# aurelienwaite/SparkNet

Hardware: AMD Instinct MI355X
Metric: images/sec AlexNet training (227x227) at 1/2/4/8 MI355X; scaling efficiency (higher is better)
Workload: dtype bf16; 1 GPU; model=caffenet (bvlc_reference_caffenet / AlexNet), global_batch=256, per_gpu_batch=256, parallelism=dp1, algorithm=local SGD, tau=50, RCCL all-reduce weight averaging, hipgraph=True, streams=3, feed_group=2, fused_input_fold=True, fp8_layers=0, fp8_wgrad=False

## Files before the change

### csrc/kernels/reduce.hip

```cpp
#include "common.h"

struct ReduceOut {
  void* out;
  long long ldo, out_gstride;
  int cols, mode, relu;
  const float* bias;
  const bf16_t* gate;
  float* extra;
  long long extra_gstride;
  int extra_col, extra_acc;
  const long long* drop_rng;
  int drop_stream;
  unsigned drop_thr;
  float drop_scale, gate_scale;
};

SN_DEV void reduce_store(const ReduceOut& o, int g, int r, int c, float4 a) {
  const float acc[4] = {a.x, a.y, a.z, a.w};
  if (o.extra && c <= o.extra_col && o.extra_col < c + 4) {
    float* e = o.extra + g * o.extra_gstride + r;
    const int q = o.extra_col - c;
    const float v = q == 0 ? a.x : (q == 1 ? a.y : (q == 2 ? a.z : a.w));
    *e = o.extra_acc ? *e + v : v;
  }
  if (o.mode == 0) {
    const long long base = g * o.out_gstride + (long long)r * o.ldo + c;
    bf16_t* p = reinterpret_cast<bf16_t*>(o.out) + base;
    float v[4];
#pragma unroll
    for (int k = 0; k < 4; ++k) {
      v[k] = acc[k] + ((o.bias && c + k < o.cols) ? o.bias[(long long)g * o.cols + c + k] : 0.f);
      if (o.relu) v[k] = fmaxf(v[k], 0.f);
      if (o.gate && c + k < o.cols) v[k] = bf2f(o.gate[base + k]) > 0.f ? v[k] * o.gate_scale : 0.f;
    }
    if (o.drop_rng) {
      if ((base & 3) == 0) {
        const uint4 u = dropout_bits4(o.drop_rng, o.drop_stream, (unsigned long long)base >> 2);
        const uint32_t b[4] = {u.x, u.y, u.z, u.w};
#pragma unroll
        for (int k = 0; k < 4; ++k) v[k] = b[k] > o.drop_thr ? v[k] * o.drop_scale : 0.f;
      } else {
#pragma unroll
        for (int k = 0; k < 4; ++k)
          v[k] = dropout_keep(o.drop_rng, o.drop_stream, o.drop_thr, base + k) ? v[k] * o.drop_scale : 0.f;
      }
    }
    if (c + 3 < o.cols && (base & 3) == 0) {
      *reinterpret_cast<uint2*>(p) = make_uint2(pack2(v[0], v[1]), pack2(v[2], v[3]));
    } else {
#pragma unroll
      for (int k = 0; k < 4; ++k)
        if (c + k < o.cols) p[k] = f2bf(v[k]);
    }
  } else {
    float* p = reinterpret_cast<float*>(o.out) + g * o.out_gstride + (long long)r * o.ldo + c;
    const int cols = o.extra ? o.extra_col : o.cols;
#pragma unroll
    for (int k = 0; k < 4; ++k)
      if (c + k < cols) p[k] = (o.mode == 2 ? p[k] : 0.f) + acc[k];
  }
}

__global__ void splitk_reduce_kernel(const float* __restrict__ ws, int splits, long long sstride, int rows,
                                     long long ldw, long long ws_gstride, ReduceOut o) {
  const int cols = o.cols, cols4 = (cols + 3) >> 2;
  const long long total = (long long)rows * cols4;
  const int g = blockIdx.y;
  const float* wsg = ws + g * ws_gstride;
  for (long long i = blockIdx.x * (long long)blockDim.x + threadIdx.x; i < total;
       i += (long long)gridDim.x * blockDim.x) {
    const int r = (int)(i / cols4), c = (int)(i - (long long)r * cols4) * 4;
    float acc[4] = {0.f, 0.f, 0.f, 0.f};
    const bool vec = (c + 3 < cols) && ((ldw & 3) == 0);
    const float* p0 = wsg + (long long)r * ldw + c;
    if (vec) {
      int s = 0;
      for (; s + 3 < splits; s += 4) {
        float4 v[4];
#pragma unroll
        for (int u = 0; u < 4; ++u) v[u] = *reinterpret_cast<const float4*>(p0 + (s + u) * sstride);
#pragma unroll
        for (int u = 0; u < 4; ++u) {
          acc[0] += v[u].x; acc[1] += v[u].y; acc[2] += v[u].z; acc[3] += v[u].w;
        }
      }
      for (; s < splits; ++s) {
        const float4 v = *reinterpret_cast<const float4*>(p0 + s * sstride);
        acc[0] += v.x; acc[1] += v.y; acc[2] += v.z; acc[3] += v.w;
      }
    } else {
      for (int s = 0; s < splits; ++s)
#pragma unroll
        for (int k = 0; k < 4; ++k)
          if (c + k < cols) acc[k] += p0[s * sstride + k];
    }
    reduce_store(o, g, r, c, make_float4(acc[0], acc[1], acc[2], acc[3]));
  }
}

__global__ void __launch_bounds__(256) splitk_reduce_wide(const float* __restrict__ ws, int splits,
                                                          long long sstride, int rows, long long ldw,
                                                          long long ws_gstride, ReduceOut o) {
  __shared__ float4 red[16][16];
  const int it = threadIdx.x & 15, sl = threadIdx.x >> 4;
  const int cols4 = (o.cols + 3) >> 2;
  const long long total = (long long)rows * cols4;
  const long long i = blockIdx.x * 16LL + it;
  const int g = blockIdx.y;
  float4 acc = make_float4(0.f, 0.f, 0.f, 0.f);
  int r = 0, c = 0;
  if (i < total) {
    r = (int)(i / cols4);
    c = (int)(i - (long long)r * cols4) * 4;
    const float* p = ws + g * ws_gstride + (long long)r * ldw + c;
    int s = sl;
    for (; s + 48 < splits; s += 64) {
      float4 v[4];
#pragma unroll
      for (int u = 0; u < 4; ++u) v[u] = *reinterpret_cast<const float4*>(p + (s + 16 * u) * sstride);
#pragma unroll
      for (int u = 0; u < 4; ++u) {
        acc.x += v[u].x; acc.y += v[u].y; acc.z += v[u].z; acc.w += v[u].w;
      }
    }
    for (; s < splits; s += 16) {
      float4 v = *reinterpret_cast<const float4*>(p + s * sstride);
      acc.x += v.x; acc.y += v.y; acc.z += v.z; acc.w += v.w;
    }
  }
  red[sl][it] = acc;
  __syncthreads();
  if (sl == 0 && i < total) {
    float a[4] = {0.f, 0.f, 0.f, 0.f};
#pragma unroll
    for (int q = 0; q < 16; ++q) {
      float4 v = red[q][it];
      a[0] += v.x; a[1] += v.y; a[2] += v.z; a[3] += v.w;
    }
    reduce_store(o, g, r, c, make_float4(a[0], a[1], a[2], a[3]));
  }
}

extern "C" int sn_splitk_reduce(const float* ws, long long splits, long long sstride, long long rows,
                                long long cols, long long ldw, void* out, long long ldo, long long mode,
                                const float* bias, long long relu, long long groups,
                                long long ws_gstride, long long out_gstride, const bf16_t* gate,
                                float* extra, long long extra_col, long long extra_acc, long long extra_gstride,
                                const long long* drop_rng, long long drop_stream, float drop_ratio,
                                float gate_scale, hipStream_t st) {
  ReduceOut o;
  o.drop_rng = drop_rng;
  o.drop_stream = (int)drop_stream;
  o.drop_thr = (uint32_t)((double)4294967295u * (double)drop_ratio);
  o.drop_scale = 1.f / (1.f - drop_ratio);
  o.gate_scale = gate_scale;
  o.out = out; o.ldo = ldo; o.out_gstride = out_gstride; o.cols = (int)cols; o.mode = (int)mode;
  o.relu = (int)relu; o.bias = bias; o.gate = gate;
  o.extra = extra; o.extra_col = (int)extra_col; o.extra_acc = (int)extra_acc; o.extra_gstride = extra_gstride;
  if (extra && (mode == 0 || extra_col != cols - 1)) return 5;
  long long total = rows * ((cols + 3) / 4);
  if (splits >= 16 && ((cols & 3) == 0 || ldw >= ((cols + 3) & ~3LL)) && (ldw & 3) == 0) {
    dim3 grid((unsigned)((total + 15) / 16), (unsigned)groups);
    hipLaunchKernelGGL(splitk_reduce_wide, grid, dim3(256), 0, st, ws, (int)splits, sstride, (int)rows, ldw,
                       ws_gstride, o);
  } else {
    dim3 grid(sn_blocks(total, 256, 4096), (unsigned)groups);
    hipLaunchKernelGGL(splitk_reduce_kernel, grid, dim3(256), 0, st, ws, (int)splits, sstride, (int)rows, ldw,
                       ws_gstride, o);
  }
  return SN_CHECK_LAUNCH();
}

__global__ void __launch_bounds__(256) colsum_pass1(const bf16_t* __restrict__ x, long long rows, int cols,
                                                    long long ld, long long rpb, int CL, float* __restrict__ part) {
  __shared__ float red[256 * 8];
  const int RL = 256 / CL;
  const int t = threadIdx.x;
  const int cc = t % CL, rr = t / CL;
  const int c = (blockIdx.y * CL + cc) * 8;
  float acc[8] = {0, 0, 0, 0, 0, 0, 0, 0};
  const long long r0 = blockIdx.x * rpb, r1 = min(rows, r0 + rpb);
  if (c < cols) {
    const bool vec = (c + 7 < cols) && ((ld & 7) == 0);
    long long r = r0 + rr;
    if (vec) {
      for (; r + 3 * RL < r1; r += 4 * RL) {
        uint4 v[4];
#pragma unroll
        for (int u = 0; u < 4; ++u) v[u] = *reinterpret_cast<const uint4*>(x + (r + u * RL) * ld + c);
#pragma unroll
        for (int u = 0; u < 4; ++u) {
          float f[8];
          unpack8(v[u], f);
#pragma unroll
          for (int k = 0; k < 8; ++k) acc[k] += f[k];
        }
      }
    }
    for (; r < r1; r += RL) {
      const bf16_t* p = x + r * ld + c;
      if (vec) {
        float f[8];
        unpack8(*reinterpret_cast<const uint4*>(p), f);
#pragma unroll
        for (int k = 0; k < 8; ++k) acc[k] += f[k];
      } else {
        for (int k = 0; k < 8; ++k)
          if (c + k < cols) acc[k] += bf2f(p[k]);
      }
    }
  }
#pragma unroll
  for (int k = 0; k < 8; ++k) red[t * 8 + k] = acc[k];
  __syncthreads();
  if (rr == 0 && c < cols) {
    for (int q = 1; q < RL; ++q)
#pragma unroll
      for (int k = 0; k < 8; ++k) acc[k] += red[(q * CL + cc) * 8 + k];
    for (int k = 0; k < 8; ++k)
      if (c + k < cols) part[blockIdx.x * (long long)cols + c + k] = acc[k];
  }
}

__global__ void __launch_bounds__(1024) colsum_pass2(const float* __restrict__ part, int nparts, int cols, float* out,
                                                     int accumulate) {
  __shared__ float red[16][64];
  const int lane = threadIdx.x & 63, w = threadIdx.x >> 6;
  const int c = blockIdx.x * 64 + lane;
  float s[8] = {0, 0, 0, 0, 0, 0, 0, 0};
  if (c < cols) {
    int p = w;
    for (; p + 7 * 16 < nparts; p += 8 * 16) {
#pragma unroll
      for (int u = 0; u < 8; ++u) s[u] += part[(long long)(p + u * 16) * cols + c];
    }
    for (; p < nparts; p += 16) s[0] += part[(long long)p * cols + c];
  }
  red[w][lane] = ((s[0] + s[1]) + (s[2] + s[3])) + ((s[4] + s[5]) + (s[6] + s[7]));
  __syncthreads();
  if (w == 0 && c < cols) {
    float tot = 0.f;
#pragma unroll
    for (int k = 0; k < 16; ++k) tot += red[k][lane];
    out[c] = (accumulate ? out[c] : 0.f) + tot;
  }
}

extern "C" int sn_colsum_bf16(const bf16_t* x, long long rows, long long cols, long long ld, float* part,
                              long long nparts, float* out, long long accumulate, hipStream_t st) {
  const int c8 = (int)((cols + 7) / 8);
  int CL = 1;
  while (CL < c8 && CL < 64) CL *= 2;
  const int cblocks = (c8 + CL - 1) / CL;
  long long rpb = (rows + nparts - 1) / nparts;
  hipLaunchKernelGGL(colsum_pass1, dim3((unsigned)nparts, (unsigned)cblocks), dim3(256), 0, st, x, rows,
                     (int)cols, ld, rpb, CL, part);
  hipLaunchKernelGGL(colsum_pass2, dim3((unsigned)((cols + 63) / 64)), dim3(1024), 0, st, part, (int)nparts,
                     (int)cols, out, (int)accumulate);
  return SN_CHECK_LAUNCH();
}

__global__ void vsum_kernel(const float* __restrict__ x, long long n, float* out, float scale, int accumulate) {
  __shared__ float red[16];
  float s = 0.f;
  for (long long i = threadIdx.x; i < n; i += blockDim.x) s += x[i];
  s = wave_sum(s);
  if ((threadIdx.x & 63) == 0) red[threadIdx.x >> 6] = s;
  __syncthreads();
  if (threadIdx.x == 0) {
    float t = 0.f;
    for (int w = 0; w < (int)(blockDim.x >> 6); ++w) t += red[w];
    out[0] = (accumulate ? out[0] : 0.f) + t * scale;
  }
}

extern "C" int sn_vsum(const float* x, long long n, float* out, float scale, long long accumulate, hipStream_t st) {
  hipLaunchKernelGGL(vsum_kernel, dim3(1), dim3(1024), 0, st, x, n, out, scale, (int)accumulate);
  return SN_CHECK_LAUNCH();
}

namespace {
__global__ void probe_tr8_kernel(unsigned* out) {
  __shared__ __attribute__((aligned(16))) unsigned char img[256];
  const int l = threadIdx.x;
  for (int e = l; e < 256; e += 64) img[e] = (unsigned char)e;
  __syncthreads();
  typedef int v2i __attribute__((ext_vector_type(2)));
  const int g = l >> 4, i = l & 15;
  const int row = 8 * (g & 1) + (i >> 1);
  typedef __attribute__((address_space(3))) v2i lds_v2i;
  const v2i v = __builtin_amdgcn_ds_read_tr8_b64_v2i32(
      (lds_v2i*)((__attribute__((address_space(3))) unsigned char*)img + row * 16 + 8 * (i & 1)));
  out[2 * l] = (unsigned)v[0];
  out[2 * l + 1] = (unsigned)v[1];
}
}

extern "C" int sn_probe_tr8(unsigned* out, hipStream_t st) {
  hipLaunchKernelGGL(probe_tr8_kernel, dim3(1), dim3(64), 0, st, out);
  return SN_CHECK_LAUNCH();
}
```

### csrc/kernels/softmax.hip

```cpp
#include "common.h"

#define FLT_MIN_ 1.175494351e-38f

__global__ void softmax_xent_fwd(const bf16_t* __restrict__ x, const float* __restrict__ labels,
                                 float* __restrict__ prob, float* __restrict__ row_loss, float* __restrict__ row_valid,
                                 int M, int C, int has_ignore, int ignore_label) {
  const int lane = threadIdx.x & 63;
  const int row = blockIdx.x * (blockDim.x >> 6) + (threadIdx.x >> 6);
  if (row >= M) return;
  const bf16_t* xr = x + (long long)row * C;
  float m = -INFINITY;
  for (int c = lane; c < C; c += 64) m = fmaxf(m, bf2f(xr[c]));
  m = wave_max(m);
  float s = 0.f;
  for (int c = lane; c < C; c += 64) s += __expf(bf2f(xr[c]) - m);
  s = wave_sum(s);
  const float inv = 1.f / s;
  float* pr = prob + (long long)row * C;
  for (int c = lane; c < C; c += 64) pr[c] = __expf(bf2f(xr[c]) - m) * inv;
  if (lane == 0) {
    int lab = (int)labels[row];
    bool valid = !(has_ignore && lab == ignore_label);
    float nll = 0.f;
    if (valid) {
      float p = __expf(bf2f(xr[min(max(lab, 0), C - 1)]) - m) * inv;
      nll = -__logf(fmaxf(p, FLT_MIN_));
    }
    row_loss[row] = nll;
    row_valid[row] = valid ? 1.f : 0.f;
  }
}

__global__ void xent_reduce(const float* __restrict__ row_loss, const float* __restrict__ row_valid, int M,
                            int normalize, float outer_num, float* __restrict__ out_loss, float* __restrict__ out_norm) {
  __shared__ float ls[16], vs[16];
  float l = 0.f, v = 0.f;
  for (int i = threadIdx.x; i < M; i += blockDim.x) {
    l += row_loss[i];
    v += row_valid[i];
  }
  l = wave_sum(l);
  v = wave_sum(v);
  if ((threadIdx.x & 63) == 0) {
    ls[threadIdx.x >> 6] = l;
    vs[threadIdx.x >> 6] = v;
  }
  __syncthreads();
  if (threadIdx.x == 0) {
    float L = 0.f, V = 0.f;
    for (int w = 0; w < (int)(blockDim.x >> 6); ++w) { L += ls[w]; V += vs[w]; }
    float norm = normalize ? V : outer_num;
    norm = fmaxf(norm, 1.f);
    out_loss[0] = L / norm;
    out_norm[0] = norm;
  }
}

extern "C" int sn_softmax_xent_fwd(const bf16_t* x, const float* labels, float* prob, float* row_loss,
                                   float* row_valid, float* out_loss, float* out_norm, long long M, long long C,
                                   long long has_ignore, long long ignore_label, long long normalize,
                                   long long outer_num, hipStream_t st) {
  const int rows_per_block = 4;
  hipLaunchKernelGGL(softmax_xent_fwd, dim3((unsigned)((M + rows_per_block - 1) / rows_per_block)), dim3(256), 0, st, x,
                     labels, prob, row_loss, row_valid, (int)M, (int)C, (int)has_ignore, (int)ignore_label);
  hipLaunchKernelGGL(xent_reduce, dim3(1), dim3(1024), 0, st, row_loss, row_valid, (int)M, (int)normalize,
                     (float)outer_num, out_loss, out_norm);
  return SN_CHECK_LAUNCH();
}

__global__ void softmax_xent_bwd(const float* __restrict__ prob, const float* __restrict__ labels,
                                 const float* __restrict__ loss_weight, const float* __restrict__ norm,
                                 bf16_t* __restrict__ dx, int M, int C, int has_ignore, int ignore_label) {
  const long long total = (long long)M * C;
  const float scale = loss_weight[0] / norm[0];
  for (long long i = blockIdx.x * (long long)blockDim.x + threadIdx.x; i < total; i += (long long)gridDim.x * blockDim.x) {
    const int row = (int)(i / C), c = (int)(i - (long long)row * C);
    const int lab = (int)labels[row];
    float g = 0.f;
    if (!(has_ignore && lab == ignore_label)) g = (prob[i] - (c == lab ? 1.f : 0.f)) * scale;
    dx[i] = f2bf(g);
  }
}

extern "C" int sn_softmax_xent_bwd(const float* prob, const float* labels, const float* loss_weight, const float* norm,
                                   bf16_t* dx, long long M, long long C, long long has_ignore, long long ignore_label,
                                   hipStream_t st) {
  hipLaunchKernelGGL(softmax_xent_bwd, dim3(sn_blocks(M * C, 256, 16384)), dim3(256), 0, st, prob, labels, loss_weight,
                     norm, dx, (int)M, (int)C, (int)has_ignore, (int)ignore_label);
  return SN_CHECK_LAUNCH();
}

__global__ void softmax_fwd(const bf16_t* __restrict__ x, bf16_t* __restrict__ y, int M, int C) {
  const int lane = threadIdx.x & 63;
  const int row = blockIdx.x * (blockDim.x >> 6) + (threadIdx.x >> 6);
  if (row >= M) return;
  const bf16_t* xr = x + (long long)row * C;
  float m = -INFINITY;
  for (int c = lane; c < C; c += 64) m = fmaxf(m, bf2f(xr[c]));
  m = wave_max(m);
  float s = 0.f;
  for (int c = lane; c < C; c += 64) s += __expf(bf2f(xr[c]) - m);
  s = wave_sum(s);
  const float inv = 1.f / s;
  for (int c = lane; c < C; c += 64) y[(long long)row * C + c] = f2bf(__expf(bf2f(xr[c]) - m) * inv);
}

__global__ void softmax_bwd(const bf16_t* __restrict__ dy, const bf16_t* __restrict__ y, bf16_t* __restrict__ dx,
                            int M, int C) {
  const int lane = threadIdx.x & 63;
  const int row = blockIdx.x * (blockDim.x >> 6) + (threadIdx.x >> 6);
  if (row >= M) return;
  const long long b = (long long)row * C;
  float d = 0.f;
  for (int c = lane; c < C; c += 64) d += bf2f(dy[b + c]) * bf2f(y[b + c]);
  d = wave_sum(d);
  for (int c = lane; c < C; c += 64) dx[b + c] = f2bf(bf2f(y[b + c]) * (bf2f(dy[b + c]) - d));
}

extern "C" int sn_softmax_fwd(const bf16_t* x, bf16_t* y, long long M, long long C, hipStream_t st) {
  hipLaunchKernelGGL(softmax_fwd, dim3((unsigned)((M + 3) / 4)), dim3(256), 0, st, x, y, (int)M, (int)C);
  return SN_CHECK_LAUNCH();
}

extern "C" int sn_softmax_bwd(const bf16_t* dy, const bf16_t* y, bf16_t* dx, long long M, long long C, hipStream_t st) {
  hipLaunchKernelGGL(softmax_bwd, dim3((unsigned)((M + 3) / 4)), dim3(256), 0, st, dy, y, dx, (int)M, (int)C);
  return SN_CHECK_LAUNCH();
}

__global__ void accuracy_rows(const bf16_t* __restrict__ x, const float* __restrict__ labels, float* __restrict__ hit,
                              float* __restrict__ valid, int M, int C, int k, int has_ignore, int ignore_label) {
  const int lane = threadIdx.x & 63;
  const int row = blockIdx.x * (blockDim.x >> 6) + (threadIdx.x >> 6);
  if (row >= M) return;
  const int lab = (int)labels[row];
  const bf16_t* xr = x + (long long)row * C;
  const int lc = min(max(lab, 0), C - 1);
  const float ls = bf2f(xr[lc]);
  float cnt = 0.f;
  for (int c = lane; c < C; c += 64) {
    const float v = bf2f(xr[c]);
    cnt += (v > ls || (!(ls > v) && c > lc)) ? 1.f : 0.f;
  }
  cnt = wave_sum(cnt);
  if (lane == 0) {
    bool v = !(has_ignore && lab == ignore_label);
    hit[row] = (v && cnt < (float)k) ? 1.f : 0.f;
    valid[row] = v ? 1.f : 0.f;
  }
}

extern "C" int sn_accuracy(const bf16_t* x, const float* labels, float* hit, float* valid, float* out_acc,
                           float* out_norm, long long M, long long C, long long k, long long has_ignore,
                           long long ignore_label, hipStream_t st) {
  hipLaunchKernelGGL(accuracy_rows, dim3((unsigned)((M + 3) / 4)), dim3(256), 0, st, x, labels, hit, valid, (int)M,
                     (int)C, (int)k, (int)has_ignore, (int)ignore_label);
  hipLaunchKernelGGL(xent_reduce, dim3(1), dim3(1024), 0, st, hit, valid, (int)M, 1, (float)M, out_acc, out_norm);
  return SN_CHECK_LAUNCH();
}
```

### csrc/kernels/solver.hip

```cpp
#include "common.h"

enum { H_LR = 0, H_MOM, H_WD, H_CLIP, H_NORM, H_DELTA, H_MOM2, H_RMS, H_CORR, H_T, H_SUMSQ = 15 };

SN_DEV void chunk_grad(const float* __restrict__ g, long long o, const long long* __restrict__ src, int cid, int i,
                       float* G) {
  const long long sp = src ? src[4 * cid] : 0;
  if (sp == 0) {
    const float4 gv = *reinterpret_cast<const float4*>(g + o);
    G[0] = gv.x; G[1] = gv.y; G[2] = gv.z; G[3] = gv.w;
    return;
  }
  const float* sl = reinterpret_cast<const float*>(sp);
  const long long ss = src[4 * cid + 1], es = src[4 * cid + 3];
  const int splits = (int)src[4 * cid + 2];
  G[0] = G[1] = G[2] = G[3] = 0.f;
  if (splits >= 16) {
    if (es == 1) {
      const float* p = sl + i;
      for (int l = 0; l < 16; ++l) {
        float P[4] = {0.f, 0.f, 0.f, 0.f};
        int s = l;
        for (; s + 48 < splits; s += 64) {
          float4 v[4];
#pragma unroll
          for (int u = 0; u < 4; ++u) v[u] = *reinterpret_cast<const float4*>(p + (s + 16 * u) * ss);
#pragma unroll
          for (int u = 0; u < 4; ++u) {
            P[0] += v[u].x; P[1] += v[u].y; P[2] += v[u].z; P[3] += v[u].w;
          }
        }
        for (; s < splits; s += 16) {
          const float4 v = *reinterpret_cast<const float4*>(p + s * ss);
          P[0] += v.x; P[1] += v.y; P[2] += v.z; P[3] += v.w;
        }
#pragma unroll
        for (int k = 0; k < 4; ++k) G[k] += P[k];
      }
    } else {
      for (int l = 0; l < 16; ++l) {
        float P[4] = {0.f, 0.f, 0.f, 0.f};
        for (int s = l; s < splits; s += 16) {
          float v[4];
#pragma unroll
          for (int k = 0; k < 4; ++k) v[k] = sl[(long long)(i + k) * es + s * ss];
#pragma unroll
          for (int k = 0; k < 4; ++k) P[k] += v[k];
        }
#pragma unroll
        for (int k = 0; k < 4; ++k) G[k] += P[k];
      }
    }
    return;
  }
  if (es == 1) {
    const float* p = sl + i;
    int s = 0;
    for (; s + 3 < splits; s += 4) {
      float4 v[4];
#pragma unroll
      for (int u = 0; u < 4; ++u) v[u] = *reinterpret_cast<const float4*>(p + (s + u) * ss);
#pragma unroll
      for (int u = 0; u < 4; ++u) {
        G[0] += v[u].x; G[1] += v[u].y; G[2] += v[u].z; G[3] += v[u].w;
      }
    }
    for (; s < splits; ++s) {
      const float4 v = *reinterpret_cast<const float4*>(p + s * ss);
      G[0] += v.x; G[1] += v.y; G[2] += v.z; G[3] += v.w;
    }
  } else {
    for (int s = 0; s < splits; ++s)
#pragma unroll
      for (int k = 0; k < 4; ++k) G[k] += sl[(long long)(i + k) * es + s * ss];
  }
}

template <int KIND, bool L1, bool CLIP, bool SHADOW>
__global__ void __launch_bounds__(256) solver_update_kernel(float* __restrict__ w, const float* __restrict__ g,
                                                            float* __restrict__ h0, float* __restrict__ h1,
                                                            bf16_t* __restrict__ shadow,
                                                            const long long* __restrict__ chunk_pos,
                                                            const float* __restrict__ chunk_mult,
                                                            const float* __restrict__ hyper, int nchunks,
                                                            const long long* __restrict__ chunk_src) {
  for (int cid = blockIdx.x; cid < nchunks; cid += gridDim.x) {
  const long long start = chunk_pos[2 * cid];
  const int count = (int)chunk_pos[2 * cid + 1];
  const float lr_mult = chunk_mult[2 * cid], decay_mult = chunk_mult[2 * cid + 1];
  const float rate = hyper[H_LR] * lr_mult;
  const float mom = hyper[H_MOM];
  const float decay = hyper[H_WD] * decay_mult;
  float gscale = hyper[H_NORM];
  if (CLIP) {
    const float clip = hyper[H_CLIP];
    const float l2 = sqrtf(hyper[H_SUMSQ]);
    if (clip > 0.f && l2 > clip) gscale *= clip / l2;
  }
  const float delta = hyper[H_DELTA], mom2 = hyper[H_MOM2], rms = hyper[H_RMS], corr = hyper[H_CORR];
  for (int i = threadIdx.x * 4; i < count; i += blockDim.x * 4) {
    const long long o = start + i;
    float4 wv = *reinterpret_cast<float4*>(w + o);
    float G[4];
    chunk_grad(g, o, chunk_src, cid, i, G);
    float4 a = *reinterpret_cast<float4*>(h0 + o);
    float4 b = make_float4(0.f, 0.f, 0.f, 0.f);
    if (KIND >= 4) b = *reinterpret_cast<float4*>(h1 + o);
    float W[4] = {wv.x, wv.y, wv.z, wv.w};
    float A[4] = {a.x, a.y, a.z, a.w}, B[4] = {b.x, b.y, b.z, b.w};
#pragma unroll
    for (int k = 0; k < 4; ++k) {
      float gg = G[k] * gscale;
      gg += decay * (L1 ? ((W[k] > 0.f) - (W[k] < 0.f)) : W[k]);
      float upd;
      if (KIND == 0) {
        A[k] = mom * A[k] + rate * gg;
        upd = A[k];
      } else if (KIND == 1) {
        float prev = A[k];
        A[k] = mom * A[k] + rate * gg;
        upd = (1.f + mom) * A[k] - mom * prev;
      } else if (KIND == 2) {
        A[k] += gg * gg;
        upd = rate * gg / (sqrtf(A[k]) + delta);
      } else if (KIND == 3) {
        A[k] = rms * A[k] + (1.f - rms) * gg * gg;
        upd = rate * gg / (sqrtf(A[k]) + delta);
      } else if (KIND == 4) {
        A[k] = mom * A[k] + (1.f - mom) * gg * gg;
        float u = gg * sqrtf((B[k] + delta) / (A[k] + delta));
        B[k] = mom * B[k] + (1.f - mom) * u * u;
        upd = rate * u;
      } else {
        A[k] = mom * A[k] + (1.f - mom) * gg;
        B[k] = mom2 * B[k] + (1.f - mom2) * gg * gg;
        upd = rate * corr * A[k] / (sqrtf(B[k]) + delta);
      }
      W[k] -= upd;
    }
    *reinterpret_cast<float4*>(w + o) = make_float4(W[0], W[1], W[2], W[3]);
    *reinterpret_cast<float4*>(h0 + o) = make_float4(A[0], A[1], A[2], A[3]);
    if (KIND >= 4) *reinterpret_cast<float4*>(h1 + o) = make_float4(B[0], B[1], B[2], B[3]);
    if (SHADOW) *reinterpret_cast<uint2*>(shadow + o) = make_uint2(pack2(W[0], W[1]), pack2(W[2], W[3]));
  }
  }
}

__global__ void sumsq_pass1(const float* __restrict__ g, long long n, float* __restrict__ part) {
  __shared__ float red[16];
  float s = 0.f;
  for (long long i = blockIdx.x * (long long)blockDim.x + threadIdx.x; i < n; i += (long long)gridDim.x * blockDim.x) {
    float v = g[i];
    s += v * v;
  }
  s = wave_sum(s);
  if ((threadIdx.x & 63) == 0) red[threadIdx.x >> 6] = s;
  __syncthreads();
  if (threadIdx.x == 0) {
    float t = 0.f;
    for (int w = 0; w < (int)(blockDim.x >> 6); ++w) t += red[w];
    part[blockIdx.x] = t;
  }
}

__global__ void sumsq_pass2(const float* __restrict__ part, int nparts, float* __restrict__ hyper) {
  __shared__ float red[16];
  float s = 0.f;
  for (int i = threadIdx.x; i < nparts; i += blockDim.x) s += part[i];
  s = wave_sum(s);
  if ((threadIdx.x & 63) == 0) red[threadIdx.x >> 6] = s;
  __syncthreads();
  if (threadIdx.x == 0) {
    float t = 0.f;
    for (int w = 0; w < (int)(blockDim.x >> 6); ++w) t += red[w];
    hyper[H_SUMSQ] = t;
  }
}

template <int KIND, bool L1, bool CLIP>
static void launch3(bool shadow, dim3 grid, hipStream_t st, float* w, const float* g, float* h0, float* h1,
                    bf16_t* sh, const long long* cp, const float* cm, const float* hyper, int n, const long long* src) {
  if (shadow)
    hipLaunchKernelGGL((solver_update_kernel<KIND, L1, CLIP, true>), grid, dim3(256), 0, st, w, g, h0, h1, sh, cp, cm,
                       hyper, n, src);
  else
    hipLaunchKernelGGL((solver_update_kernel<KIND, L1, CLIP, false>), grid, dim3(256), 0, st, w, g, h0, h1, sh, cp,
                       cm, hyper, n, src);
}

template <int KIND>
static void launch_kind(bool l1, bool clip, bool shadow, dim3 grid, hipStream_t st, float* w, const float* g,
                        float* h0, float* h1, bf16_t* sh, const long long* cp, const float* cm, const float* hyper,
                        int n, const long long* src) {
  if (l1) {
    if (clip) launch3<KIND, true, true>(shadow, grid, st, w, g, h0, h1, sh, cp, cm, hyper, n, src);
    else launch3<KIND, true, false>(shadow, grid, st, w, g, h0, h1, sh, cp, cm, hyper, n, src);
  } else {
    if (clip) launch3<KIND, false, true>(shadow, grid, st, w, g, h0, h1, sh, cp, cm, hyper, n, src);
    else launch3<KIND, false, false>(shadow, grid, st, w, g, h0, h1, sh, cp, cm, hyper, n, src);
  }
}

extern "C" int sn_solver_update(long long kind, float* w, const float* g, float* h0, float* h1, bf16_t* shadow,
                                const long long* chunk_pos, const float* chunk_mult, long long nchunks,
                                float* hyper, long long l1, long long clip, float* part, long long nparts,
                                long long total, long long grid_limit, const long long* chunk_src, hipStream_t st) {
  if (nchunks <= 0) return 0;
  if (clip && chunk_src) return 9;
  if (clip) {
    hipLaunchKernelGGL(sumsq_pass1, dim3((unsigned)nparts), dim3(256), 0, st, g, total, part);
    hipLaunchKernelGGL(sumsq_pass2, dim3(1), dim3(1024), 0, st, part, (int)nparts, hyper);
  }
  dim3 grid((unsigned)(grid_limit > 0 && grid_limit < nchunks ? grid_limit : nchunks));
  bool sh = shadow != nullptr;
  const int n = (int)nchunks;
  switch (kind) {
    case 0: launch_kind<0>(l1, clip, sh, grid, st, w, g, h0, h1, shadow, chunk_pos, chunk_mult, hyper, n, chunk_src); break;
    case 1: launch_kind<1>(l1, clip, sh, grid, st, w, g, h0, h1, shadow, chunk_pos, chunk_mult, hyper, n, chunk_src); break;
    case 2: launch_kind<2>(l1, clip, sh, grid, st, w, g, h0, h1, shadow, chunk_pos, chunk_mult, hyper, n, chunk_src); break;
    case 3: launch_kind<3>(l1, clip, sh, grid, st, w, g, h0, h1, shadow, chunk_pos, chunk_mult, hyper, n, chunk_src); break;
    case 4: launch_kind<4>(l1, clip, sh, grid, st, w, g, h0, h1, shadow, chunk_pos, chunk_mult, hyper, n, chunk_src); break;
    case 5: launch_kind<5>(l1, clip, sh, grid, st, w, g, h0, h1, shadow, chunk_pos, chunk_mult, hyper, n, chunk_src); break;
    default: return 8;
  }
  return SN_CHECK_LAUNCH();
}

__global__ void scale_shadow(float* __restrict__ w, bf16_t* __restrict__ shadow, long long n, long long n4,
                             float scale) {
  const long long stride = (long long)gridDim.x * blockDim.x;
  for (long long i = blockIdx.x * (long long)blockDim.x + threadIdx.x; i < n4; i += stride) {
    float4 v = reinterpret_cast<float4*>(w)[i];
    v.x *= scale; v.y *= scale; v.z *= scale; v.w *= scale;
    reinterpret_cast<float4*>(w)[i] = v;
    if (shadow) reinterpret_cast<uint2*>(shadow)[i] = make_uint2(pack2(v.x, v.y), pack2(v.z, v.w));
  }
  for (long long i = 4 * n4 + blockIdx.x * (long long)blockDim.x + threadIdx.x; i < n; i += stride) {
    const float v = w[i] * scale;
    w[i] = v;
    if (shadow) shadow[i] = f2bf(v);
  }
}

extern "C" int sn_scale_shadow(float* w, bf16_t* shadow, long long n, float scale, hipStream_t st) {
  if (n <= 0) return 0;
  const bool vec = (reinterpret_cast<uintptr_t>(w) & 15) == 0 && (reinterpret_cast<uintptr_t>(shadow) & 7) == 0;
  const long long n4 = vec ? n / 4 : 0;
  hipLaunchKernelGGL(scale_shadow, dim3(sn_blocks(n4 > 0 ? n4 : n, 256, 16384)), dim3(256), 0, st, w, shadow, n, n4,
                     scale);
  return SN_CHECK_LAUNCH();
}
```

### sparknet_amd/core/solver.py

```python
from __future__ import annotations

import logging
import math
import os
import time
from typing import Callable

import numpy as np
import torch

from .. import proto
from .net import Net, blob_proto_to_tensor

log = logging.getLogger("sparknet_amd.solver")

SOLVER_KINDS = {"SGD": 0, "Nesterov": 1, "AdaGrad": 2, "RMSProp": 3, "AdaDelta": 4, "Adam": 5}
_LEGACY_TYPES = {0: "SGD", 1: "Nesterov", 2: "AdaGrad", 3: "RMSProp", 4: "AdaDelta", 5: "Adam"}
N_HISTORY = {"SGD": 1, "Nesterov": 1, "AdaGrad": 1, "RMSProp": 1, "AdaDelta": 2, "Adam": 2}

H_LR, H_MOM, H_WD, H_CLIP, H_NORM, H_DELTA, H_MOM2, H_RMS, H_CORR, H_T = range(10)
N_HYPER = 16


class Solver:
    def __init__(self, param, *, device="cpu", dtype=None, seed: int | None = None,
                 train_net: Net | None = None, build_test_nets: bool = True):
        if isinstance(param, str):
            param = proto.read_solver(param)
        self.param = proto.copy(param)
        p = self.param
        self.type = p.type if p.HasField("type") else (
            _LEGACY_TYPES[int(p.solver_type)] if p.HasField("solver_type") else "SGD")
        if self.type not in SOLVER_KINDS:
            raise ValueError(f"Unknown solver type {self.type!r}")
        self.device = torch.device(device)
        if seed is None:
            seed = int(p.random_seed) if p.random_seed >= 0 else 1701
        self.seed = seed
        self.iter = 0
        self.current_step = 0
        self.callbacks: list = []
        self.action_request: Callable[[], str] | None = None
        self.requested_early_exit = False
        self.losses: list[torch.Tensor] = []
        self.smoothed_loss = 0.0
        self.net = train_net if train_net is not None else self._init_train_net(dtype)
        self.test_nets: list[Net] = []
        if build_test_nets:
            self._init_test_nets(dtype)
        self.history: list[torch.Tensor] = []
        self._init_state()

    def _net_param_source(self):
        p = self.param
        n = int(p.HasField("train_net_param")) + int(p.HasField("train_net")) + \
            int(p.HasField("net_param")) + int(p.HasField("net"))
        if n != 1:
            raise ValueError("SolverParameter must specify exactly one of train_net_param, train_net, "
                             "net_param, net")
        if p.HasField("train_net_param"):
            return proto.copy(p.train_net_param)
        if p.HasField("train_net"):
            return proto.read_net(p.train_net)
        if p.HasField("net_param"):
            return proto.copy(p.net_param)
        return proto.read_net(p.net)

    def _init_train_net(self, dtype) -> Net:
        netp = self._net_param_source()
        state = proto.NetState(phase=proto.TRAIN)
        state.MergeFrom(netp.state)
        state.MergeFrom(self.param.train_state)
        netp.state.CopyFrom(state)
        return Net(netp, device=self.device, dtype=dtype, seed=self.seed)

    def _init_test_nets(self, dtype) -> None:
        p = self.param
        sources = []
        for tp in p.test_net_param:
            sources.append(proto.copy(tp))
        for tf in p.test_net:
            sources.append(proto.read_net(tf))
        remaining = len(p.test_iter) - len(sources)
        if remaining > 0:
            if p.HasField("net_param"):
                sources += [proto.copy(p.net_param)] * remaining
            elif p.HasField("net"):
                base = proto.read_net(p.net)
                sources += [base] * remaining
        if len(p.test_state) and len(p.test_state) != len(sources):
            raise ValueError("test_state must be unspecified or specified once per test net")
        for i, netp in enumerate(sources):
            netp = proto.copy(netp)
            state = proto.NetState(phase=proto.TEST)
            state.MergeFrom(netp.state)
            if len(p.test_state):
                state.MergeFrom(p.test_state[i])
            netp.state.CopyFrom(state)
            tn = Net(netp, device=self.device, dtype=self.net.dtype, seed=self.seed, allocate=True)
            tn.share_trained_layers_with(self.net)
            self.test_nets.append(tn)

    def _init_state(self) -> None:
        n = self.net.num_param_elems
        self.history = [torch.zeros(max(n, 1), dtype=torch.float32, device=self.device)
                        for _ in range(N_HISTORY[self.type])]
        self.hyper = torch.zeros(N_HYPER, dtype=torch.float32, device=self.device)
        self._hyper_staged: list | None = None
        self._build_tables()

    def _build_tables(self) -> None:
        from .. import ops
        segs = self.net.param_segments()
        self.segments = segs
        fused = set(getattr(self, "fused_offsets", set()))
        for sink in getattr(self, "slab_sinks", ()):
            if sink.desc is not None:
                fused.update(p.offset for p in sink.params())
        self._tables = ops.solver_tables([s for s in segs if s[0] not in fused], self.net.num_param_elems,
                                         self.device)
        self.slab_tables_dirty = False

    def set_slab_sinks(self, sinks) -> None:
        self.slab_sinks = list(sinks)
        self.slab_tables_dirty = True
        if not getattr(self, "fused_offsets", None):
            self.fused_offsets = set()

    def set_fused_update(self, offsets) -> None:
        self.fused_offsets = set(offsets)
        self._build_tables()

    def get_learning_rate(self) -> float:
        p = self.param
        pol = p.lr_policy
        it = self.iter
        if pol == "fixed":
            return p.base_lr
        if pol == "step":
            self.current_step = it // p.stepsize
            return p.base_lr * math.pow(p.gamma, self.current_step)
        if pol == "exp":
            return p.base_lr * math.pow(p.gamma, it)
        if pol == "inv":
            return p.base_lr * math.pow(1.0 + p.gamma * it, -p.power)
        if pol == "multistep":
            if self.current_step < len(p.stepvalue) and it >= p.stepvalue[self.current_step]:
                self.current_step += 1
            return p.base_lr * math.pow(p.gamma, self.current_step)
        if pol == "poly":
            return p.base_lr * math.pow(1.0 - float(it) / float(p.max_iter), p.power)
        if pol == "sigmoid":
            return p.base_lr * (1.0 / (1.0 + math.exp(-p.gamma * (float(it) - float(p.stepsize)))))
        raise ValueError(f"Unknown learning rate policy: {pol!r}")

    def hyper_values(self, rate: float) -> list[float]:
        p = self.param
        h = [0.0] * N_HYPER
        h[H_LR] = rate
        h[H_MOM] = p.momentum
        h[H_WD] = p.weight_decay
        h[H_CLIP] = p.clip_gradients
        h[H_NORM] = 1.0 / max(1, p.iter_size)
        h[H_DELTA] = p.delta
        h[H_MOM2] = p.momentum2
        h[H_RMS] = p.rms_decay
        t = self.iter + 1
        if self.type == "Adam":
            h[H_CORR] = math.sqrt(1.0 - math.pow(p.momentum2, t)) / (1.0 - math.pow(p.momentum, t))
        h[H_T] = float(t)
        return h

    def stage_hyper(self, rate: float | None = None) -> float:
        rate = self.get_learning_rate() if rate is None else rate
        vals = self.hyper_values(rate)
        vals[H_T] = 0.0
        if vals == self._hyper_staged:
            return rate
        self._hyper_staged = vals
        host = torch.tensor(vals, dtype=torch.float32)
        if self.device.type == "cuda":
            host = host.pin_memory()
        self.hyper.copy_(host, non_blocking=True)
        return rate

    def apply_update(self) -> float:
        rate = self.stage_hyper()
        if self.param.display and self.iter % self.param.display == 0:
            log.info("Iteration %d, lr = %g", self.iter, rate)
        self.update_params()
        return rate

    def overlap_eligible(self) -> bool:
        return (self.device.type == "cuda" and self.param.clip_gradients <= 0 and self.param.iter_size <= 1
                and not self.callbacks)

    def overlap_plan(self, min_group: int = 1) -> tuple[dict, list]:
        net = self.net
        seg_of = {seg[0]: seg for seg in self.segments}
        final, late = {}, set()
        for li, layer in enumerate(net.layers):
            writer = getattr(layer, "fused_into", None) if layer.params else None
            wl = net.layers.index(writer) if writer is not None else li
            for i, p in enumerate(layer.params):
                if p.offset not in seg_of:
                    continue
                if not net.layer_need_backward[li] or not layer.param_grads_needed(i):
                    late.add(p.offset)
                final[p.offset] = min(final.get(p.offset, wl), wl)
        groups: dict = {}
        for off, li in final.items():
            if off not in late:
                groups.setdefault(li, []).append(seg_of[off])
        big = {li: segs for li, segs in groups.items() if sum(sg[1] for sg in segs) >= min_group}
        rest = [seg_of[o] for o in seg_of if not any(o == sg[0] for segs in big.values() for sg in segs)]
        return big, rest

    def update_params_segments(self, tables, grid_limit: int = 0) -> None:
        from .. import ops
        net = self.net
        ops.solver_update(SOLVER_KINDS[self.type], net.flat_data, net.flat_diff, self.history,
                          net.flat_compute if net.flat_compute is not net.flat_data else None,
                          tables, self.hyper, self.param.regularization_type == "L1", False, grid_limit)

    def update_params(self) -> None:
        from .. import ops
        l1 = self.param.regularization_type == "L1"
        if self.param.regularization_type not in ("L1", "L2"):
            raise ValueError(f"Unknown regularization type: {self.param.regularization_type}")
        net = self.net
        if getattr(self, "slab_tables_dirty", False):
            assert not torch.cuda.is_current_stream_capturing(), "split-K slab layout changed during capture"
            self._build_tables()
        ops.solver_update(SOLVER_KINDS[self.type], net.flat_data, net.flat_diff, self.history,
                          net.flat_compute if net.flat_compute is not net.flat_data else None,
                          self._tables, self.hyper, l1, self.param.clip_gradients > 0)

    def iteration(self):
        net = self.net
        if getattr(self, "fused_offsets", None) or getattr(self, "slab_sinks", None):
            self.stage_hyper()
        net.clear_param_diffs(lazy=True)
        for cb in self.callbacks:
            getattr(cb, "on_start", lambda: None)()
        loss = None
        for _ in range(max(1, self.param.iter_size)):
            l = net.forward_backward()
            loss = l if loss is None else loss + l
            from .. import ops
            ops.advance_rng(net.ctx.rng_state)
        net.finish_param_diffs()
        if getattr(net.ctx, "fp8", None) is not None:
            net.ctx.fp8.update()
        if self.param.iter_size > 1:
            loss = loss / self.param.iter_size
        for cb in self.callbacks:
            getattr(cb, "on_gradients_ready", lambda: None)()
        self.apply_update()
        return loss

    def step(self, iters: int) -> None:
        start_iter = self.iter
        stop_iter = self.iter + iters
        avg = max(1, self.param.average_loss)
        while self.iter < stop_iter:
            loss = self.iteration()
            self.losses.append(loss.detach())
            if len(self.losses) > avg:
                self.losses.pop(0)
            display = self.param.display and self.iter % self.param.display == 0
            self.iter += 1
            if display:
                self.smoothed_loss = float(torch.stack(self.losses).mean())
                log.info("Iteration %d, loss = %g", self.iter - 1, self.smoothed_loss)
            if self.param.snapshot and self.iter % self.param.snapshot == 0:
                self.snapshot()
            req = self.action_request() if self.action_request else "none"
            if req == "snapshot":
                self.snapshot()
            elif req == "stop":
                self.requested_early_exit = True
                break
        del start_iter

    def solve(self, resume_file: str | None = None) -> None:
        if resume_file:
            self.restore(resume_file)
        p = self.param
        self.requested_early_exit = False
        while self.iter < p.max_iter and not self.requested_early_exit:
            if p.test_interval and self.iter % p.test_interval == 0 and (self.iter > 0 or p.test_initialization):
                self.test_all()
            n = p.max_iter - self.iter
            if p.test_interval:
                n = min(n, p.test_interval - self.iter % p.test_interval)
            self.step(n)
        if p.snapshot_after_train and (not p.snapshot or self.iter % p.snapshot != 0):
            self.snapshot()
        if self.requested_early_exit:
            log.info("Optimization stopped early.")
            return
        if p.display and self.iter % p.display == 0:
            loss = self.net.forward()
            log.info("Iteration %d, loss = %g", self.iter, float(loss))
        if p.test_interval and self.iter % p.test_interval == 0:
            self.test_all()

    def test(self, test_net_id: int = 0, iters: int | None = None) -> list[float]:
        scores = self.test_and_store_result(test_net_id, iters)
        n = iters if iters is not None else self.param.test_iter[test_net_id]
        res = [s / max(n, 1) for s in scores]
        tn = self.test_nets[test_net_id]
        names = [b.name for b in tn.output_blobs]
        for name, v in zip(names, res):
            log.info("    Test net output #%s: %s = %g", test_net_id, name, v)
        return res

    def test_and_store_result(self, test_net_id: int = 0, iters: int | None = None) -> list[float]:
        tn = self.test_nets[test_net_id]
        n = iters if iters is not None else self.param.test_iter[test_net_id]
        acc = None
        for _ in range(n):
            tn.forward()
            vals = torch.stack([b.data.float().sum() for b in tn.output_blobs])
            acc = vals if acc is None else acc + vals
        return [] if acc is None else acc.cpu().tolist()

    def test_all(self) -> list[list[float]]:
        return [self.test(i) for i in range(len(self.test_nets))]

    def _prefix(self) -> str:
        return self.param.snapshot_prefix or "snapshot"

    def snapshot(self, prefix: str | None = None) -> tuple[str, str]:
        prefix = prefix or self._prefix()
        h5 = self.param.HasField("snapshot_format") and self.param.snapshot_format == 0
        ext = ".h5" if h5 else ""
        model = f"{prefix}_iter_{self.iter}.caffemodel{ext}"
        state = f"{prefix}_iter_{self.iter}.solverstate{ext}"
        d = os.path.dirname(model)
        if d:
            os.makedirs(d, exist_ok=True)
        if h5:
            self.net.to_hdf5(model, write_diff=self.param.snapshot_diff)
            self._state_to_hdf5(state, model)
        else:
            from ..utils.checkpoint import save_caffemodel
            save_caffemodel(self.net, model, write_diff=self.param.snapshot_diff)
            proto.write_binary(state, self.solver_state(model))
        log.info("Snapshotting to %s / %s", model, state)
        return model, state

    def _history_blobs(self):
        for h in self.history:
            for prm in self.net.learnable_params:
                yield prm, h[prm.offset:prm.offset + prm.count].view(prm.shape)

    def _state_to_hdf5(self, path: str, learned_net: str) -> None:
        from ..utils import hdf5
        hist = {str(i): prm.to_caffe(seg).float().cpu().numpy()
                for i, (prm, seg) in enumerate(self._history_blobs())}
        hdf5.write(path, {"iter": np.array([self.iter], np.int32), "learned_net": learned_net,
                          "current_step": np.array([self.current_step], np.int32), "history": hist})

    def solver_state(self, learned_net: str = ""):
        st = proto.SolverState(iter=self.iter, learned_net=learned_net, current_step=self.current_step)
        for prm, seg in self._history_blobs():
            bp = st.history.add()
            bp.shape.dim.extend(prm.caffe_shape)
            bp.data.extend(prm.to_caffe(seg).cpu().reshape(-1).tolist())
        return st

    def restore(self, state_file: str) -> None:
        if state_file.endswith(".h5"):
            from ..utils import hdf5
            f = hdf5.File(state_file)
            self.iter = hdf5.read_int(f["iter"])
            learned = hdf5.read_string(f["learned_net"]) if "learned_net" in f else ""
            self.current_step = hdf5.read_int(f["current_step"])
            hist = f["history"]
            blobs = [torch.from_numpy(hist[str(i)].read().astype(np.float32)) for i in range(len(hist))]
        else:
            st = proto.read_binary(state_file, proto.SolverState)
            self.iter, self.current_step, learned = st.iter, st.current_step, st.learned_net
            blobs = [blob_proto_to_tensor(b) for b in st.history]
        if learned:
            self.net.copy_trained_layers_from(learned)
        slots = list(self._history_blobs())
        if len(blobs) != len(slots):
            raise ValueError("Incorrect length of history blobs.")
        for (prm, seg), t in zip(slots, blobs):
            seg.copy_(prm.from_caffe(t).to(seg.device))
        log.info("Restored solver state from %s (iter %d)", state_file, self.iter)

    def add_callback(self, cb) -> None:
        self.callbacks.append(cb)


def create_solver(param, **kw) -> Solver:
    return Solver(param, **kw)


def timed(fn):
    def wrap(*a, **k):
        t = time.perf_counter()
        r = fn(*a, **k)
        return r, time.perf_counter() - t
    return wrap
```

### sparknet_amd/engine.py

```python
from __future__ import annotations

import gc
import logging
import os
import time

import torch

from . import ops
from .core.solver import Solver
from .utils import features
from .utils.trace import trace_range

from .ops.spec import ConvSpec

log = logging.getLogger("sparknet_amd.engine")


def fuse_relu(net) -> int:
    if net.device.type == "cuda" and net.dtype == torch.float32:
        return 0
    n = 0
    for li in range(1, len(net.layers)):
        relu = net.layers[li]
# ... 31 lines not shown
        blob = net.top_ids[li][0]
        if len(net.bottom_vecs[li][0].shape) not in (2, 4):
            continue
        if net.bottom_ids[li + 1] != [blob] or net.top_ids[li + 1] != [blob]:
            continue
        if sc.scale is None or (sc.axis, sc.k) != (1, 1) or sc.fused_into is not None:
            continue
        need = net.layer_need_backward[li]
        if net.layer_need_backward[li + 1] != need or (need and not net.bottom_need_backward[li + 1][0]):
            continue
        relu = net.layers[li + 2] if li + 2 < len(net.layers) else None
        if (relu is not None and relu.type_name == "ReLU" and getattr(relu, "slope", 1.0) == 0.0
                and net.bottom_ids[li + 2] == [blob] and net.top_ids[li + 2] == [blob] and not relu.fused
                and not relu.bwd_fused):
            if net.layer_need_backward[li + 2] != need or (need and not net.bottom_need_backward[li + 2][0]):
                continue
            relu.fused = True
            relu.bwd_fused = True
            relu.bn_fused = True
            bn.fused_relu = True
        bn.fused_scale = sc
        sc.fused_into = bn
        ex = dict(getattr(bn, "sched_extra", None) or {})
        ex["bwd_w"] = set(ex.get("bwd_w", ())) | {("p", p.offset) for p in sc.params}
        bn.sched_extra = ex
        n += 1
    net.bn_scale_fused += n
    return n


def fuse_pool_lrn(net) -> int:
    from .ops import hip
    if net.device.type != "cuda" or net.debug_info or not features.enabled("fuse_pool_lrn"):
        return 0
    outputs = set(getattr(net, "output_blob_ids", ()))
    n = 0
    for li, pool in enumerate(net.layers):
        if pool.type_name != "Pooling" or len(net.top_ids[li]) != 1 or pool.global_pooling:
            continue
        blob = net.top_ids[li][0]
        readers = [lj for lj in range(li + 1, len(net.layers)) if blob in net.bottom_ids[lj]]
        if blob in outputs or len(readers) != 1:
            continue
        lj = readers[0]
        lrn = net.layers[lj]
        if lrn.type_name != "LRN" or lrn.relu_gate or net.top_ids[lj][0] == blob:
            continue
        if net.layer_need_backward[li] != net.layer_need_backward[lj]:
            continue
        s = pool.spec(net.bottom_vecs[li][0])
        if not hip.pool_lrn_eligible(s, lrn.size, lrn.within):
            continue
        lrn.pool_fused = True
        lrn.top = net.top_vecs[lj][0]
        pool.fused_lrn = lrn
        n += 1
    return n


def fuse_lrn_pool_backward(net) -> int:
    from .ops import hip
    if net.device.type != "cuda" or net.debug_info or not features.enabled("fuse_lrn_pool_bwd"):
        return 0
    outputs = set(getattr(net, "output_blob_ids", ()))
    n = 0
    for lj, lrn in enumerate(net.layers):
        if lrn.type_name != "LRN" or lrn.pool_fused or lrn.within or len(net.top_ids[lj]) != 1:
            continue
        blob = net.top_ids[lj][0]
        if blob in outputs or blob == net.bottom_ids[lj][0]:
            continue
        readers = [li for li in range(lj + 1, len(net.layers)) if blob in net.bottom_ids[li]]
        if len(readers) != 1:
            continue
        li = readers[0]
        pool = net.layers[li]
        if (pool.type_name != "Pooling" or len(net.top_ids[li]) != 1 or pool.global_pooling
                or pool.fused_lrn is not None or pool.relu_gate or net.top_ids[li][0] == blob):
            continue
        if not (net.layer_need_backward[li] and net.layer_need_backward[lj] and net.bottom_need_backward[li][0]
                and net.bottom_need_backward[lj][0]):
            continue
        s = pool.spec(net.bottom_vecs[li][0])
        if not hip.pool_lrn_rev_eligible(s, lrn.size, lrn.within):
            continue
        pool.bwd_lrn = lrn
        lrn.bottom = net.bottom_vecs[lj][0]
        bid = net.bottom_ids[lj][0]
        ex = dict(getattr(pool, "sched_extra", None) or {})
        ex["bwd_r"] = set(ex.get("bwd_r", ())) | {("v", bid)}
        ex["bwd_w"] = set(ex.get("bwd_w", ())) | {("d", bid)}
        pool.sched_extra = ex
        n += 1
    return n


def _gating_consumers(net, blob: int, after: int):
    if blob in getattr(net, "output_blob_ids", ()):
        return None
    out = []
    for lj in range(after + 1, len(net.layers)):
        if blob not in net.bottom_ids[lj]:
            continue
        lay = net.layers[lj]
        if blob in net.top_ids[lj] or not net.layer_need_backward[lj]:
            return None
        if lay.type_name == "Split":
            for t in net.top_ids[lj]:
                sub = _gating_consumers(net, t, lj)
                if sub is None:
                    return None
                out += sub
            continue
        if lay.type_name not in _GATE_CONSUMERS or len(net.bottom_ids[lj]) != 1 or getattr(lay, "relu_gate", False):
            return None
        if lay.type_name == "Pooling" and (lay.method not in (0, 1) or len(net.top_ids[lj]) != 1):
            return None
        if lay.type_name in ("InnerProduct", "Dropout"):
            return None
        out.append(lj)
    return out


def fuse_concat(net) -> int:
    if net.device.type != "cuda" or not features.enabled("zero_copy_concat"):
        return 0
    from .layers.common import ConcatSlots
    from .ops import hip
    n = 0
    outputs = set(getattr(net, "output_blob_ids", ()))
    for lc, cat in enumerate(net.layers):
        if cat.type_name != "Concat" or len(net.bottom_ids[lc]) < 2 or cat.zero_copy is not None:
            continue
        bots = net.bottom_ids[lc]
        if len(set(bots)) != len(bots) or len(net.bottom_vecs[lc][0].shape) != 4:
            continue
        if cat.axis != 1:
            continue
        prods = []
        for bid in bots:
            writers = [lj for lj in range(lc) if bid in net.top_ids[lj]]
            readers = [lj for lj in range(len(net.layers)) if bid in net.bottom_ids[lj] and lj != lc]
            if not writers or bid in outputs:
                break
            prod = net.layers[writers[0]]
            inplace_ok = all(net.layers[lj].type_name == "ReLU" and getattr(net.layers[lj], "fused", False)
                             and net.top_ids[lj] == [bid] and net.bottom_ids[lj] == [bid] for lj in readers)
            if (not inplace_ok or set(writers[1:]) != set(readers) or prod.type_name != "Convolution"
                    or len(net.top_ids[writers[0]]) != 1 or prod.concat_slot is not None
                    or prod.fp8_slots is not None or prod.folded_input is not None):
                break
            s = prod.spec(net.bottom_vecs[writers[0]][0])
            if not hip._slice_ok(s) or hip._s2d_plan(s) is not None:
                break
            prods.append((prod, s.K))
        if len(prods) != len(bots):
            continue
        slots = ConcatSlots([k for _, k in prods])
        for part, (prod, _) in enumerate(prods):
            prod.concat_slot = (slots, part)
        cat.zero_copy = slots
        gated = _gating_consumers(net, net.top_ids[lc][0], lc)
        if gated is not None and cat.relu_gate_parts == frozenset(range(len(bots))):
            for lj in gated:
                net.layers[lj].relu_gate = True
            cat.relu_gate_parts = frozenset()
            cat.zero_copy_bwd = True
        n += 1
    return n


def fuse_dropout(net) -> int:
    if net.device.type != "cuda" or not features.enabled("fuse_dropout"):
        return 0
    n = 0
    for li in range(1, len(net.layers)):
        d = net.layers[li]
        if d.type_name != "Dropout" or d.phase != 0 or not (d.ratio > 0) or d.fused_into is not None:
            continue
        if net.bottom_ids[li] != net.top_ids[li] or not getattr(d, "relu_gate", False):
            continue
        blob = net.top_ids[li][0]
        prods = [lj for lj in range(li) if blob in net.top_ids[lj]]
        lp = next((lj for lj in reversed(prods) if net.layers[lj].type_name == "InnerProduct"), None)
        if lp is None or not getattr(net.layers[lp], "fuse_relu", False):
            continue
        between = [net.layers[lj] for lj in prods if lj > lp]
        if any(not (l.type_name == "ReLU" and getattr(l, "fused", False)) for l in between):
            continue
        consumers = [lj for lj in range(li + 1, len(net.layers)) if blob in net.bottom_ids[lj]]
        if len(consumers) != 1 or blob in getattr(net, "output_blob_ids", ()):
            continue
        lc = consumers[0]
        cons = net.layers[lc]
        if cons.type_name != "InnerProduct" or len(net.bottom_ids[lc]) != 1 or blob in net.top_ids[lc]:
            continue
        prod = net.layers[lp]
        if prod.fused_dropout is not None:
            continue
        prod.fused_dropout = d
        d.fused_into = prod
        cons.relu_gate = True
        cons.gate_scale = 1.0 / (1.0 - d.ratio)
        n += 1
    return n


def batch_weight_flips(net) -> int:
    if net.device.type != "cuda" or getattr(net, "_flip_batch", None) is not None:
        return 0
    from .ops import hip
    items = []
    for li, layer in enumerate(net.layers):
        if layer.type_name != "Convolution" or not net.layer_need_backward[li]:
            continue
        if not any(net.bottom_need_backward[li]):
            continue
        specs = [layer.spec(b) for b in net.bottom_vecs[li]]
        if not all(hip.dgrad_uses_flip(s) for s in specs):
            continue
        s = specs[0]
        wt = torch.empty((s.groups, s.Cg, s.R, s.S, s.Kg), dtype=torch.bfloat16, device=net.device)
        items.append((layer.weight.compute, wt, s.groups, s.Kg, s.R, s.S, s.Cg))
        layer.flipped_weights = wt
    if not items:
        return 0
    net._flip_batch = hip.FlipBatch(items, net.device)
    net.pre_backward_hooks.append(net._flip_batch.run)
    return len(items)


_GATE_CONSUMERS = ("Convolution", "InnerProduct", "Dropout", "Pooling", "LRN")


def fuse_relu_backward(net) -> int:
    n = 0
    for li, relu in enumerate(net.layers):
        if relu.type_name != "ReLU" or getattr(relu, "slope", 1.0) != 0.0:
            continue
        if net.bottom_ids[li] != net.top_ids[li] or getattr(relu, "bn_fused", False):
            continue
        blob = net.top_ids[li][0]
        consumers = [lj for lj in range(li + 1, len(net.layers)) if blob in net.bottom_ids[lj]]
        if not consumers:
            continue
        lc = consumers[0]
        if len(consumers) > 1 and blob not in net.top_ids[lc]:
            continue
        cons = net.layers[lc]
        if cons.type_name == "Concat" and len(net.bottom_ids[lc]) > 1 and blob not in net.top_ids[lc] \
                and blob not in getattr(net, "output_blob_ids", ()):
            pos = {i for i, b in enumerate(net.bottom_ids[lc]) if b == blob}
            cons.relu_gate_parts = frozenset(cons.relu_gate_parts | pos)
            relu.bwd_fused = True
            n += 1
            continue
        if cons.type_name not in _GATE_CONSUMERS or len(net.bottom_ids[lc]) != 1:
            continue
        if cons.type_name == "Pooling" and (cons.method != 0 or len(net.top_ids[lc]) != 1):
            continue
        if blob in getattr(net, "output_blob_ids", ()):
            continue
        cons.relu_gate = True
        relu.bwd_fused = True
        n += 1
    return n


class _FusedFCUpdate:

    def __init__(self, solver, param, flags: int):
        self.solver, self.p, self.flags = solver, param, flags

    def sgd(self) -> dict:
        p = self.p
        h = self.solver.history[0][p.offset:p.offset + p.count].view(p.data.shape)
        return {"w": p.data, "h": h, "shadow": p.compute, "hyper": self.solver.hyper, "lr_mult": p.lr_mult,
                "decay_mult": p.decay_mult, "flags": self.flags}


def fuse_fc_updates(solver) -> int:
    net = solver.net
    if net.device.type != "cuda" or not solver.overlap_eligible() or solver.type not in ("SGD", "Nesterov"):
        return 0
    if net.flat_compute is net.flat_data or solver.param.regularization_type not in ("L1", "L2"):
        return 0
    users: dict = {}
    for layer in net.layers:
        for p in layer.params:
            users[p.offset] = users.get(p.offset, 0) + 1
    flags = (1 if solver.type == "Nesterov" else 0) | (2 if solver.param.regularization_type == "L1" else 0)
    offsets = []
    for li, layer in enumerate(net.layers):
        if layer.type_name != "InnerProduct" or not net.layer_need_backward[li] or not layer.param_grads_needed(0):
            continue
        p = layer.weight
        if p.owner is not None or users.get(p.offset, 0) != 1 or layer.N % 8 or layer.Kdim % 8:
            continue
        layer.fused_update = _FusedFCUpdate(solver, p, flags)
        offsets.append(p.offset)
    if offsets:
        solver.set_fused_update(offsets)
    return len(offsets)


class _SlabGrad:

    def __init__(self, solver, layer):
        self.solver, self.layer = solver, layer
        self.buf = None
        self.desc = None
        self.got = False
        self.table = None

    def begin(self):
        self.got = False

    def end(self):
        if not self.got:
            self._set(None)

    def accepts(self, out, bias_grad) -> bool:
        ok = out.data_ptr() == self.layer.weight.diff.data_ptr()
        if ok and bias_grad is not None:
            ok = self.layer.bias is not None and bias_grad.data_ptr() == self.layer.bias.diff.data_ptr()
        return ok

    def slab(self, numel: int, device):
        if self.buf is None or self.buf.numel() < numel:
            assert not torch.cuda.is_current_stream_capturing(), "split-K slab buffer grown during capture"
            self.buf = torch.empty(numel, dtype=torch.float32, device=device)
        return self.buf[:numel]

    def record(self, d):
        self.got = True
        self._set(d)

    def _set(self, d):
        if d != self.desc:
            assert not torch.cuda.is_current_stream_capturing(), "split-K slab layout changed during capture"
            self.desc = d
            self.solver.slab_tables_dirty = True
            self.table = None
            if d is not None:
                from . import ops
                mine = {p.offset for p in self.params()}
                segs = [sg for sg in self.solver.net.param_segments() if sg[0] in mine]
                self.table = ops.solver_tables(segs, self.solver.net.num_param_elems, self.solver.device,
                                               self.chunks())

    def params(self):
        return [self.layer.weight] + ([self.layer.bias] if self.layer.bias is not None else [])

    def apply(self) -> None:
        if self.table is not None:
            self.solver.update_params_segments(self.table)

    def chunks(self) -> dict:
        d = self.desc
        if d is None:
            return {}
        M, N, ldw, G, S = d.M, d.N, d.ldw, d.groups, d.splits
        assert d.ldc == N and d.c_gstride == M * N, "weight gradient must be the dense [K][RS*Cg] layout"
        base, ss, gs = d.base, M * ldw, S * M * ldw
        wp = self.layer.weight
        out = {wp.offset: [(wp.offset + (g * M + m) * N, N, base + 4 * (g * gs + m * ldw), ss, S, 1)
                           for g in range(G) for m in range(M)]}
        bp = self.layer.bias
        if d.ones >= 0 and bp is not None:
            out[bp.offset] = [(bp.offset + g * M, M, base + 4 * (g * gs + d.ones), ss, S, ldw) for g in range(G)]
        return out


def fuse_splitk_updates(solver) -> int:
    net = solver.net
    if (net.device.type != "cuda" or not solver.overlap_eligible() or net.debug_info
            or not features.enabled("fuse_splitk")):
        return 0
    from .ops import hip
    users: dict = {}
    for layer in net.layers:
        for p in layer.params:
            users[p.offset] = users.get(p.offset, 0) + 1
    sinks = []
    for li, layer in enumerate(net.layers):
        if layer.type_name != "Convolution" or not net.layer_need_backward[li] or not layer.param_grads_needed(0):
            continue
        if len(net.bottom_vecs[li]) != 1 or getattr(layer, "folded_input", None) is not None:
            continue
        ps = [layer.weight] + ([layer.bias] if layer.bias is not None else [])
        if any(p.owner is not None or users.get(p.offset, 0) != 1 for p in ps):
            continue
        s = layer.spec(net.bottom_vecs[li][0])
        if hip.s2d_plan(s) is not None or hip._image_chunk(s) < s.N or not hip._implicit_ok(s) or s.Kg % 8:
            continue
        layer.slab_grad = _SlabGrad(solver, layer)
        sinks.append(layer.slab_grad)
    if sinks:
        solver.set_slab_sinks(sinks)
    return len(sinks)


def fuse_input_fold(net, feeder) -> bool:
    if feeder is None or feeder.device.type != "cuda" or net.dtype == torch.float32:
        return False
    from .ops import hip
    try:
        bid = net.blob_names.index(feeder.data_blob.name)
    except (AttributeError, ValueError):
        return False
    consumers = [li for li, b in enumerate(net.bottom_ids) if bid in b]
    if len(consumers) != 1:
        return False
    conv = net.layers[consumers[0]]
    if conv.type_name != "Convolution" or net.bottom_ids[consumers[0]].index(bid) != 0:
        return False
    spec = conv.spec(feeder.data_blob)
    plan = hip.s2d_plan(spec)
    if plan is None or spec.H != feeder.crop or spec.C != feeder.shape[1]:
        return False
    s2 = plan[4]
    x2 = torch.empty((spec.N, s2.H, s2.W, s2.C), dtype=torch.bfloat16, device=feeder.device)
    feeder.fold = (x2, plan, spec)
    conv.folded_input = x2
    return True


def fp8_macs_per_input(layer, bottom) -> float:
    if layer.type_name == "Convolution":
        s = layer.spec(bottom)
        return (s.K // s.groups) * s.R * s.S / float(s.sh * s.sw)
    return float(layer.N)


def fp8_dgrad_macs_per_grad(layer, bottom) -> float:
    s = layer.spec(bottom)
    return float(s.Cg * s.R * s.S)


def enable_fp8(net, min_macs_per_input: float = 1000.0, dgrad: bool = False, dgrad_format: str = "e4m3",
               wgrad: bool = False) -> int:
    if net.device.type != "cuda":
        return 0
    from .ops import hip
    chosen, chosen_dg = [], []
    for li, layer in enumerate(net.layers):
        if layer.type_name in ("Convolution", "InnerProduct") and len(net.bottom_vecs[li]) == 1:
            b = net.bottom_vecs[li][0]
            direct = layer.type_name == "Convolution" and hip.direct_fp8_ok(layer.spec(b))
            if layer.fp8_eligible(b) and (direct or fp8_macs_per_input(layer, b) >= min_macs_per_input):
                chosen.append(layer)
            if (dgrad and layer.type_name == "Convolution" and layer.fp8_dgrad_eligible(b)
                    and net.bottom_need_backward[li][0]
                    and ((direct and dgrad_format == "e4m3")
                         or fp8_dgrad_macs_per_grad(layer, b) >= min_macs_per_input)):
                chosen_dg.append(layer)
    sc = hip.Fp8Scales(2 * (len(chosen) + len(chosen_dg)), net.device)
    for i, layer in enumerate(chosen):
        layer.fp8_slots = (2 * i, 2 * i + 1)
    assert dgrad_format in ("e4m3", "e5m2"), dgrad_format
    for i, layer in enumerate(chosen_dg, start=len(chosen)):
        layer.fp8_dgrad_slots = (2 * i, 2 * i + 1)
        if dgrad_format == "e5m2":
            sc.set_e5m2(2 * i)
    n_wg = 0
    if wgrad:
        both = set(map(id, chosen)) & set(map(id, chosen_dg))
        for li, layer in enumerate(net.layers):
            if id(layer) in both and hip.fp8_wgrad_ok(layer.spec(net.bottom_vecs[li][0])):
                layer.fp8_wgrad = True
                n_wg += 1
    net.ctx.fp8 = sc if (chosen or chosen_dg) else None
    fuse_fp8_quant(net)
    return len(chosen) + len(chosen_dg) + n_wg


def fuse_fp8_quant(net) -> int:
    if getattr(net.ctx, "fp8", None) is None or not features.enabled("fuse_fp8_quant"):
        return 0
    from .ops import hip
    outputs = set(getattr(net, "output_blob_ids", ()))
    n = 0

    def sole_reader(pi):
        blob = net.top_ids[pi][0]
        readers = [lj for lj in range(pi + 1, len(net.layers))
                   if blob in net.bottom_ids[lj] and not getattr(net.layers[lj], "fused", False)]
        return readers[0] if (blob not in outputs and len(readers) == 1) else None

    for oi, pool in enumerate(net.layers):
        if (pool.type_name != "Pooling" or len(net.top_ids[oi]) != 1 or pool.fused_lrn is not None
                or pool.global_pooling):
            continue
        s = pool.spec(net.bottom_vecs[oi][0])
        lq = sole_reader(oi)
        if lq is not None and net.layers[lq].type_name == "Convolution" and net.layers[lq].fp8_slots is not None \
                and hip.pool_side_ok(s, False):
            cons = net.layers[lq]
            pool.fp8_out = (cons, cons.fp8_slots[0])
            n += 1
        bid = net.bottom_ids[oi][0]
        prods = [pj for pj in range(oi) if bid in net.top_ids[pj] and not getattr(net.layers[pj], "fused", False)]
        if prods and hip.pool_side_ok(s, True) and net.bottom_need_backward[oi][0]:
            prod = net.layers[prods[-1]]
            if (prod.type_name == "Convolution" and prod.fp8_dgrad_slots is not None
                    and net.bottom_need_backward[prods[-1]][0] and sole_reader(prods[-1]) == oi):
                pool.fp8_dx_out = (prod, prod.fp8_dgrad_slots[0])
                pool.fp8_dx_only = (features.enabled("fp8_dx_only") and not net.debug_info
                                    and hip.conv_dy_fp8_only_ok(prod, prod.spec(net.bottom_vecs[prods[-1]][0])))
                n += 1
    for pi, prod in enumerate(net.layers):
        if prod.type_name != "Convolution" or not prod.fuse_relu or len(net.top_ids[pi]) != 1:
            continue
        if prod.concat_slot is not None:
            continue
        blob = net.top_ids[pi][0]
        readers = [lj for lj in range(pi + 1, len(net.layers))
                   if blob in net.bottom_ids[lj] and not getattr(net.layers[lj], "fused", False)]
        if blob in outputs or len(readers) != 1:
            continue
        lq = readers[0]
        cons = net.layers[lq]
        if cons.type_name != "Convolution" or len(net.bottom_ids[lq]) != 1:
            continue
        if cons.fp8_slots is not None:
            prod.fp8_out = (cons, cons.fp8_slots[0])
            n += 1
        if prod.fp8_dgrad_slots is not None and net.bottom_need_backward[pi][0]:
            cons.fp8_dx_out = (prod, prod.fp8_dgrad_slots[0])
            n += 1
    return n


def fp8_step(net) -> None:
    if getattr(net.ctx, "fp8", None) is not None:
        net.ctx.fp8.update()


_DEPFREE_LRU = features.enabled("branch_depfree")


class BranchStreams:

    def __init__(self, net, n_streams: int = 4, star: bool = False):
        self.net = net
        self.n = max(1, n_streams)
        self.star = star
        self.side = None
        L = len(net.layers)
        ex = [getattr(net.layers[li], "sched_extra", None) or {} for li in range(L)]
        fwd = [(li, {("v", b) for b in net.bottom_ids[li]} | set(ex[li].get("fwd_r", ())),
                {("v", b) for b in net.top_ids[li]} | set(ex[li].get("fwd_w", ()))) for li in range(L)]
        bwd = []
        for li in range(L - 1, -1, -1):
            if not net.layer_need_backward[li]:
                continue
            reads = {("v", b) for b in list(net.bottom_ids[li]) + list(net.top_ids[li])}
            reads |= {("d", b) for b in net.top_ids[li]}
            reads |= set(ex[li].get("bwd_r", ()))
            writes = {("d", b) for b, need in zip(net.bottom_ids[li], net.bottom_need_backward[li]) if need}
            writes |= {("p", p.offset) for p in net.layers[li].params}
            writes |= set(ex[li].get("bwd_w", ()))
            bwd.append((li, reads, writes))
        self.fwd_plan = self._plan(fwd)
        self.bwd_plan = self._plan(bwd)

    def _plan(self, nodes):
        last_w, readers = {}, {}
        tail = [-1] * self.n
        seen = [[-1] * self.n for _ in range(self.n)]
        stream_of, plan = [], []
        for pos, (li, reads, writes) in enumerate(nodes):
            deps = {last_w[r] for r in reads if r in last_w}
            for w in writes:
                if w in last_w:
                    deps.add(last_w[w])
                deps |= readers.get(w, set())
            deps.discard(pos)
            follow = [stream_of[d] for d in sorted(deps, reverse=True) if tail[stream_of[d]] == d]
            if follow:
                sid = follow[0]
            elif not deps and (pos == 0 or not _DEPFREE_LRU):
                sid = 0
            else:
                sid = min(range(self.n), key=lambda s: tail[s])
            if self.star and sid != 0 and any(stream_of[d] not in (0, sid) for d in deps):
                sid = 0
            waits = [d for d in sorted(deps) if stream_of[d] != sid and d > seen[sid][stream_of[d]]]
            for d in waits:
                seen[sid][stream_of[d]] = max(seen[sid][stream_of[d]], d)
            stream_of.append(sid)
            tail[sid] = pos
            plan.append([li, sid, waits, False])
            for r in reads:
                readers.setdefault(r, set()).add(pos)
            for w in writes:
                last_w[w] = pos
                readers[w] = set()
        for _, _, waits, _ in list(plan):
            for d in waits:
                plan[d][3] = True
        return plan

    def streams_used(self, backward: bool = False) -> int:
        return len({sid for _, sid, _, _ in (self.bwd_plan if backward else self.fwd_plan)})

    def _run(self, plan, fn) -> None:
        if self.side is None:
            self.side = [torch.cuda.Stream(self.net.device) for _ in range(self.n - 1)]
            self._events = {}
            self._fork_join = (torch.cuda.Event(), [torch.cuda.Event() for _ in self.side])
        main = torch.cuda.current_stream(self.net.device)
        streams = [main] + self.side
        evs = self._events.setdefault(id(plan), {})
        fork, join = self._fork_join
        fork.record(main)
        for s in self.side:
            s.wait_event(fork)
        for pos, (li, sid, waits, record) in enumerate(plan):
            st = streams[sid]
            for d in waits:
                st.wait_event(evs[d])
            with torch.cuda.stream(st):
                fn(li)
            if record:
                if pos not in evs:
                    evs[pos] = torch.cuda.Event()
                evs[pos].record(st)
        for s, ev in zip(self.side, join):
            ev.record(s)
            main.wait_event(ev)

    def forward(self):
        net = self.net
        self._run(self.fwd_plan, lambda li: net.layers[li].forward(net.bottom_vecs[li], net.top_vecs[li]))
        return net.loss_value()

    def backward(self) -> None:
        net = self.net
        if net.backward_hooks:
            net.backward()
            return
        net.prefill_loss_diffs()
        for hook in net.pre_backward_hooks:
            hook()
        self._run(self.bwd_plan, lambda li: net.layers[li].backward(
            net.top_vecs[li], net.bottom_need_backward[li], net.bottom_vecs[li]))

    def forward_backward(self):
        loss = self.forward()
        self.backward()
        return loss


def branch_streams(net, n_streams: int = 4):
    if net.device.type != "cuda" or n_streams <= 1:
        return None
    bs = BranchStreams(net, n_streams, star=n_streams > 2)
    if bs.streams_used() <= 1 and bs.streams_used(backward=True) <= 1:
        return None
    return bs


class OverlappedUpdate:

    MIN_GROUP = 1 << 22
    GRID = 128

    def __init__(self, solver: Solver, min_group: int | None = None):
        self.solver = solver
        groups, rest = solver.overlap_plan(self.MIN_GROUP if min_group is None else min_group)
        dev = solver.device
        self.tables = {li: ops.solver_tables(segs, solver.net.num_param_elems, dev) for li, segs in groups.items()}
        self.rest = ops.solver_tables(rest, solver.net.num_param_elems, dev) if rest else None
        self.side = torch.cuda.Stream(dev)
        self.active = False

    def hook(self, li: int) -> None:
        t = self.tables.get(li)
        if t is None or not self.active:
            return
        main = torch.cuda.current_stream(self.solver.device)
        self.side.wait_stream(main)
        with torch.cuda.stream(self.side):
            self.solver.update_params_segments(t, grid_limit=self.GRID)

    def begin(self) -> None:
        self.active = True

    def end(self) -> None:
        self.active = False
        if self.rest is not None:
            self.solver.update_params_segments(self.rest)
        torch.cuda.current_stream(self.solver.device).wait_stream(self.side)


def release_activations(net) -> int:
    keep = set()
    for li in range(len(net.layers)):
        if not net.bottom_ids[li]:
            keep.update(net.top_ids[li])
    n = 0
    for bi, blob in enumerate(net.blobs):
        if bi in keep:
            continue
        blob._data = None
        blob._diff = None
        n += 1
    from .ops.hip import ConvScratch
    for layer in net.layers:
        ws = getattr(layer, "_ws", None)
        for d in ws if isinstance(ws, list) else ():
            if isinstance(d, ConvScratch):
                d.release()
    gc.collect()
    torch.cuda.empty_cache()
    return n


GRAPH_RELEASE = None


def _release_before_capture(dev) -> bool:
    if GRAPH_RELEASE is not None:
        return bool(GRAPH_RELEASE)
    if dev.type != "cuda":
        return False
    total = torch.cuda.get_device_properties(dev).total_memory
    return torch.cuda.memory_reserved(dev) > 0.45 * total


class GraphStep:

    def __init__(self, solver: Solver, warmup: int = 2, pre=None, overlap: bool = True, fuse_fc: bool = True,
                 streams: int = 2, comm=None):
        self.solver = solver
        self.pre = pre
        self.comm = comm
        self.graph = None
        self.loss = None
        self.warmup = warmup
        self.overlap = None
        if overlap and solver.overlap_eligible():
            self.overlap = OverlappedUpdate(solver)
            solver.net.backward_hooks.append(self.overlap.hook)
        elif fuse_fc:
            fuse_fc_updates(solver)
            fuse_splitk_updates(solver)
        self.n_streams = streams if not solver.net.debug_info else 1
        self.branches = None
        self._use_branches = False

    def _body(self):
        s = self.solver
        net = s.net
        net.clear_param_diffs(lazy=True)
        for cb in s.callbacks:
            getattr(cb, "on_start", lambda: None)()
        if self.overlap is not None:
            self.overlap.begin()
        if self._use_branches and self.branches is None:
            self.branches = branch_streams(net, self.n_streams) or False
        loss = (self.branches.forward_backward() if self._use_branches and self.branches
                else net.forward_backward())
        net.finish_param_diffs()
        fp8_step(net)
        for cb in s.callbacks:
            getattr(cb, "on_gradients_ready", lambda: None)()
        ops.advance_rng(net.ctx.rng_state)
        if self.overlap is not None:
            self.overlap.end()
        else:
            s.update_params()
        return loss

    def capture(self) -> None:
        s = self.solver
        dev = s.device
        side = torch.cuda.Stream(dev)
        side.wait_stream(torch.cuda.current_stream(dev))
        with torch.cuda.stream(side):
            for w in range(self.warmup):
                self._use_branches = w > 0
                if self.pre:
                    self.pre()
                s.stage_hyper()
                self._body()
                s.iter += 1
        torch.cuda.current_stream(dev).wait_stream(side)
        torch.cuda.synchronize(dev)
        if self.comm is not None:
            from .ops import gemm as _gemm
            _gemm.sync_tuned(self.comm)
        if _release_before_capture(dev):
            release_activations(s.net)
        self.graph = torch.cuda.CUDAGraph()
        self._use_branches = True
        if self.pre:
            self.pre()
        s.stage_hyper()
        with torch.cuda.graph(self.graph):
            self.loss = self._body()
        self.graph.replay()
        s.iter += 1
        gc.collect()
        gc.freeze()

    max_ahead = int(os.environ.get("SN_MAX_AHEAD", "2"))

    def step(self):
        s = self.solver
        if self.graph is None:
            self.capture()
            return self.loss
        d = self.max_ahead
        if d > 0:
            ring = self.__dict__.setdefault("_ahead", [None] * d)
            k = self.__dict__.get("_ahead_k", 0)
            if ring[k % d] is not None:
                ring[k % d].synchronize()
        if self.pre:
            self.pre()
        s.stage_hyper()
        self.graph.replay()
        s.iter += 1
        if d > 0:
            ev = ring[k % d] or torch.cuda.Event()
            ev.record()
            ring[k % d] = ev
            self._ahead_k = k + 1
        return self.loss


class LocalSGDTrainer:

    def __init__(self, solver: Solver, comm=None, tau: int = 50, feeder=None, use_graph: bool = True,
                 log_every: int = 0, overlap_update: bool = False, fuse_fc: bool = True, streams: int = 2):
        self.solver = solver
        self.comm = comm
        self.tau = tau
        self.feeder = feeder
        self.round = 0
        self.use_graph = use_graph and solver.device.type == "cuda"
        self.step_fn = (GraphStep(solver, pre=self._pre, overlap=overlap_update, fuse_fc=fuse_fc, streams=streams,
                                  comm=comm)
                        if self.use_graph else None)
        self.log_every = log_every
        self.times = {"compute": 0.0, "allreduce": 0.0}

    def _pre(self):
        if self.feeder is not None:
            with trace_range("data"):
                self.feeder.stage()
                self.feeder.prefetch()

    def broadcast_initial(self) -> None:
        if self.comm is not None and getattr(self.comm, "active", self.comm.world_size > 1):
            self.comm.broadcast_params(self.solver.net)

    def local_step(self):
        with trace_range("compute"):
            if self.use_graph:
                return self.step_fn.step()
            self._pre()
            loss = self.solver.iteration()
            self.solver.iter += 1
            return loss

    def average(self) -> None:
        if self.comm is not None and getattr(self.comm, "active", self.comm.world_size > 1):
            with trace_range("allreduce"):
                self.comm.average_params(self.solver.net)

    def run_round(self):
        loss = None
        for _ in range(self.tau):
            loss = self.local_step()
        self.average()
        self.round += 1
        return loss

    def train(self, rounds: int, on_round=None):
        for r in range(rounds):
            t = time.perf_counter()
            loss = self.run_round()
            if on_round:
                on_round(r, loss, time.perf_counter() - t)
        return self.round
```

### sparknet_amd/layers/loss.py

```python
from __future__ import annotations

import torch

from .. import ops
from ..core.layer import Layer, register


def _prod(dims) -> int:
    n = 1
    for d in dims:
        n *= int(d)
    return n


def rows_view(blob, axis, diff=False):
    t = blob.diff if diff else blob.data
    axis = blob.canonical_axis(axis)
    if blob.is_image:
        if axis == 1:
            return t.reshape(-1, blob.shape[1])
        t = _lh().nhwc_to_nchw(t) if t.is_cuda else t.permute(0, 3, 1, 2)
    elif axis == len(blob.shape) - 1 or blob.count_range(axis + 1) == 1:
        return t.reshape(-1, blob.shape[axis])
    outer, A, inner = _prod(blob.shape[:axis]), blob.shape[axis], _prod(blob.shape[axis + 1:])
    if inner == 1:
        return t.reshape(-1, A)
    if t.is_cuda:
        return _lh().transpose(t.contiguous(), outer, A, inner).reshape(-1, A)
    return t.reshape(outer, A, inner).permute(0, 2, 1).reshape(-1, A)


def rows_view_back(rows, blob, axis):
    axis = blob.canonical_axis(axis)
    if (blob.is_image and axis == 1) or (not blob.is_image and (
            axis == len(blob.shape) - 1 or blob.count_range(axis + 1) == 1)):
        return rows.reshape(blob.data.shape)
    outer, A, inner = _prod(blob.shape[:axis]), blob.shape[axis], _prod(blob.shape[axis + 1:])
    if inner == 1:
        t = rows
    elif rows.is_cuda:
        t = _lh().transpose(rows.contiguous().reshape(outer, inner, A), outer, inner, A)
    else:
        t = rows.reshape(outer, inner, A).permute(0, 2, 1)
    if not blob.is_image:
        return t.reshape(blob.data.shape)
    N, C_, H, W = blob.shape
    if rows.is_cuda:
        return _lh().nchw_to_nhwc(t.contiguous().reshape(N, C_, H * W), N, C_, H, W)
    return t.reshape(N, C_, H, W).permute(0, 2, 3, 1).contiguous()


def _lh():
    from ..ops import layers_hip
    return layers_hip


def _sample_rows(blob, diff=False):
    t = blob.diff if diff else blob.data
    N = blob.shape[0] if blob.shape else 1
    if blob.is_image and blob.shape[2] * blob.shape[3] > 1:
        t = _lh().nhwc_to_nchw(t)
    return t.reshape(N, -1)


def _sample_rows_back(g, blob):
    if blob.is_image and blob.shape[2] * blob.shape[3] > 1:
        N, C_, H, W = blob.shape
        return _lh().nchw_to_nhwc(g.reshape(N, C_, H * W), N, C_, H, W)
    return g.reshape(blob.data.shape)


class _RowLossGPU:

    kind = ""

    def _gpu_label(self, bottoms):
        return bottoms[1].data.reshape(-1).float() if len(bottoms) > 1 else None

    def gpu_forward(self, x, t, label, H=None, margin=0.0, legacy=False):
        lh = _lh()
        M = x.shape[0]
        self._ws = lh.loss_rows_fwd(self.kind, x, t, label, H, M, x.shape[1], margin, legacy)
        return lh.loss_sum(self._ws, M, 1.0 / M)

    def gpu_backward(self, x, t, label, lw, H=None, margin=0.0, legacy=False):
        M = x.shape[0]
        return _lh().loss_rows_bwd(self.kind, x, t, label, H, M, x.shape[1], lw, 1.0 / M, 1.0, self._ws, margin,
                                   legacy)


class LossLayer(Layer):
    is_loss = True
    auto_top_blobs = True
    min_bottoms = 2
    exact_tops = -1
    min_tops = 1

    def reshape(self, bottoms, tops):
        tops[0].reshape((), torch.float32)

    def allow_force_backward(self, bottom_id: int) -> bool:
        return bottom_id != 1


@register("SoftmaxWithLoss")
class SoftmaxWithLossLayer(LossLayer):
    exact_bottoms = 2
    max_tops = 2

    def layer_setup(self, bottoms, tops):
        lp = self.lp.loss_param
        self.ignore_label = lp.ignore_label if lp.HasField("ignore_label") else None
        self.normalize = lp.normalize
        self.axis = bottoms[0].canonical_axis(self.lp.softmax_param.axis)

    def reshape(self, bottoms, tops):
        tops[0].reshape((), torch.float32)
        b = bottoms[0]
        outer = b.count_range(0, self.axis)
        inner = b.count_range(self.axis + 1)
        if outer * inner != bottoms[1].count:
            raise ValueError("Number of labels must match number of predictions")
        self.outer = outer
        if len(tops) > 1:
            tops[1].reshape(b.shape, self.dtype)

    def forward(self, bottoms, tops):
        x2 = rows_view(bottoms[0], self.axis)
        loss, prob, norm = ops.softmax_loss_forward(x2, bottoms[1].data, self.ignore_label,
                                                    self.normalize, self.outer)
        self.prob, self.norm = prob, norm
        tops[0].data = loss.reshape(())
        if len(tops) > 1:
            tops[1].data = rows_view_back(prob, bottoms[0], self.axis).to(self.dtype)

    def backward(self, tops, propagate_down, bottoms):
        if len(propagate_down) > 1 and propagate_down[1]:
            raise ValueError("SoftmaxWithLoss cannot backpropagate to label inputs")
        if propagate_down[0]:
            g = ops.softmax_loss_backward(self.prob, bottoms[1].data, tops[0].diff, self.norm,
                                          self.ignore_label, bottoms[0].dtype)
            bottoms[0].diff = rows_view_back(g, bottoms[0], self.axis).to(bottoms[0].dtype)


@register("Softmax")
class SoftmaxLayer(Layer):
    exact_bottoms = 1
    exact_tops = 1

    def layer_setup(self, bottoms, tops):
        self.axis = bottoms[0].canonical_axis(self.lp.softmax_param.axis)

    def reshape(self, bottoms, tops):
        tops[0].reshape(bottoms[0].shape, self.dtype)

    def forward(self, bottoms, tops):
        b = bottoms[0]
        tops[0].data = rows_view_back(ops.softmax_forward(rows_view(b, self.axis)), b, self.axis).to(self.dtype)

    def backward(self, tops, propagate_down, bottoms):
        if not propagate_down[0]:
            return
        t, b = tops[0], bottoms[0]
        g = ops.softmax_backward(rows_view(t, self.axis, diff=True), rows_view(t, self.axis))
        b.diff = rows_view_back(g, b, self.axis).to(b.dtype)


@register("Accuracy")
class AccuracyLayer(Layer):
    exact_bottoms = 2
    exact_tops = 1

    def layer_setup(self, bottoms, tops):
        p = self.lp.accuracy_param
        self.top_k = int(p.top_k)
        self.axis = bottoms[0].canonical_axis(p.axis)
        self.ignore_label = p.ignore_label if p.HasField("ignore_label") else None

    def reshape(self, bottoms, tops):
        tops[0].reshape((), torch.float32)

    def forward(self, bottoms, tops):
        x2 = rows_view(bottoms[0], self.axis)
        tops[0].data = ops.accuracy(x2, bottoms[1].data, self.top_k, self.ignore_label).reshape(())

    def backward(self, tops, propagate_down, bottoms):
        if any(propagate_down):
            raise NotImplementedError("Accuracy has no backward")


@register("EuclideanLoss")
class EuclideanLossLayer(LossLayer, _RowLossGPU):
    exact_bottoms = 2
    kind = "Euclidean"

    def forward(self, bottoms, tops):
        if bottoms[0].data.is_cuda:
            a, b = bottoms[0].data.reshape(bottoms[0].shape[0], -1), bottoms[1].data.reshape(bottoms[0].shape[0], -1)
            tops[0].data = self.gpu_forward(a, b, None).reshape(())
            return
        self.d = bottoms[0].data.float() - bottoms[1].data.float()
        n = bottoms[0].shape[0]
        tops[0].data = ((self.d * self.d).sum() / n / 2.0).reshape(())

    def backward(self, tops, propagate_down, bottoms):
        n = bottoms[0].shape[0]
        if tops[0].diff.is_cuda:
            rows = [bottoms[i].data.reshape(n, -1) for i in range(2)]
            for i in range(2):
                if propagate_down[i]:
                    g = self.gpu_backward(rows[i], rows[1 - i], None, tops[0].diff)
                    bottoms[i].diff = g.reshape(bottoms[i].data.shape)
            return
        lw = tops[0].diff.float()
        for i in range(2):
            if propagate_down[i]:
                sign = 1.0 if i == 0 else -1.0
                bottoms[i].diff = (self.d * (sign * lw / n)).to(bottoms[i].dtype)


@register("SigmoidCrossEntropyLoss")
class SigmoidCrossEntropyLossLayer(LossLayer, _RowLossGPU):
    exact_bottoms = 2
    kind = "SigmoidXent"

    def forward(self, bottoms, tops):
        if bottoms[0].data.is_cuda:
            x, t = _sample_rows(bottoms[0]), _sample_rows(bottoms[1])
            tops[0].data = self.gpu_forward(x, t.reshape(x.shape), None).reshape(())
            return
        x = bottoms[0].data.float()
        t = bottoms[1].data.float().reshape(x.shape)
        self.sig = torch.sigmoid(x)
        loss = -(x * (t - (x >= 0).float()) - torch.log1p(torch.exp(x - 2 * x * (x >= 0).float())))
        tops[0].data = (loss.sum() / bottoms[0].shape[0]).reshape(())

    def backward(self, tops, propagate_down, bottoms):
        if len(propagate_down) > 1 and propagate_down[1]:
            raise ValueError("SigmoidCrossEntropyLoss cannot backpropagate to label inputs")
        if propagate_down[0] and tops[0].diff.is_cuda:
            x, t = _sample_rows(bottoms[0]), _sample_rows(bottoms[1])
            g = self.gpu_backward(x, t.reshape(x.shape), None, tops[0].diff)
            bottoms[0].diff = _sample_rows_back(g, bottoms[0])
            return
        if propagate_down[0]:
            t = bottoms[1].data.float().reshape(self.sig.shape)
            g = (self.sig - t) * (tops[0].diff.float() / bottoms[0].shape[0])
            bottoms[0].diff = g.to(bottoms[0].dtype)


@register("HingeLoss")
class HingeLossLayer(LossLayer, _RowLossGPU):
    exact_bottoms = 2

    def forward(self, bottoms, tops):
        if bottoms[0].data.is_cuda:
            self.kind = "HingeL2" if int(self.lp.hinge_loss_param.norm) == 2 else "HingeL1"
            tops[0].data = self.gpu_forward(_sample_rows(bottoms[0]), None, self._gpu_label(bottoms)).reshape(())
            return
        x = rows_view(bottoms[0], 1).float()
        lab = bottoms[1].data.reshape(-1).long()
        sign = -torch.ones_like(x)
        sign.scatter_(1, lab[:, None], 1.0)
        self.m = torch.clamp(1 - sign * x, min=0)
        self.sign = sign
        l2 = int(self.lp.hinge_loss_param.norm) == 2
        self.l2 = l2
        v = (self.m * self.m).sum() if l2 else self.m.sum()
        tops[0].data = (v / x.shape[0]).reshape(())

    def backward(self, tops, propagate_down, bottoms):
        if propagate_down[0] and tops[0].diff.is_cuda:
            g = self.gpu_backward(_sample_rows(bottoms[0]), None, self._gpu_label(bottoms), tops[0].diff)
            bottoms[0].diff = _sample_rows_back(g, bottoms[0])
            return
        if propagate_down[0]:
            n = self.m.shape[0]
            g = -self.sign * ((2 * self.m) if self.l2 else (self.m > 0).float())
            g = g * (tops[0].diff.float() / n)
            bottoms[0].diff = g.reshape(bottoms[0].data.shape).to(bottoms[0].dtype)


@register("MultinomialLogisticLoss")
class MultinomialLogisticLossLayer(LossLayer, _RowLossGPU):
    exact_bottoms = 2
    kind = "Multinomial"

    def forward(self, bottoms, tops):
        if bottoms[0].data.is_cuda:
            tops[0].data = self.gpu_forward(_sample_rows(bottoms[0]), None, self._gpu_label(bottoms)).reshape(())
            return
        p = rows_view(bottoms[0], 1).float()
        lab = bottoms[1].data.reshape(-1).long()
        self.pl = p.gather(1, lab[:, None]).clamp_min(1e-20)
        tops[0].data = (-torch.log(self.pl).sum() / p.shape[0]).reshape(())

    def backward(self, tops, propagate_down, bottoms):
        if propagate_down[0] and tops[0].diff.is_cuda:
            g = self.gpu_backward(_sample_rows(bottoms[0]), None, self._gpu_label(bottoms), tops[0].diff)
            bottoms[0].diff = _sample_rows_back(g, bottoms[0])
            return
        if propagate_down[0]:
            p = rows_view(bottoms[0], 1).float()
            lab = bottoms[1].data.reshape(-1).long()
            g = torch.zeros_like(p)
            g.scatter_(1, lab[:, None], -1.0 / self.pl)
            g = g * (tops[0].diff.float() / p.shape[0])
            bottoms[0].diff = g.reshape(bottoms[0].data.shape).to(bottoms[0].dtype)


@register("InfogainLoss")
class InfogainLossLayer(LossLayer, _RowLossGPU):
    min_bottoms = 2
    max_bottoms = 3
    kind = "Infogain"

    def _gpu_H(self, bottoms, dim):
        H = self.H if self.H is not None else bottoms[2].data
        return H.reshape(dim, -1).float().contiguous()

    def layer_setup(self, bottoms, tops):
        self.H = None
        if len(bottoms) < 3:
            from ..core.net import blob_proto_to_tensor
            from .. import proto
            src = self.lp.infogain_loss_param.source
            self.H = blob_proto_to_tensor(proto.read_binary(src, proto.BlobProto)).reshape(
                bottoms[0].shape[1], -1).to(self.device)

    def forward(self, bottoms, tops):
        if bottoms[0].data.is_cuda:
            x = _sample_rows(bottoms[0])
            self._Hg = self._gpu_H(bottoms, x.shape[1])
            tops[0].data = self.gpu_forward(x, None, self._gpu_label(bottoms), self._Hg).reshape(())
            return
        p = rows_view(bottoms[0], 1).float()
        H = self.H if self.H is not None else bottoms[2].data.float().reshape(p.shape[1], -1)
        lab = bottoms[1].data.reshape(-1).long()
        self.Hl = H[lab]
        self.p = p.clamp_min(1e-20)
        tops[0].data = (-(self.Hl * torch.log(self.p)).sum() / p.shape[0]).reshape(())

    def backward(self, tops, propagate_down, bottoms):
        if propagate_down[0] and tops[0].diff.is_cuda:
            g = self.gpu_backward(_sample_rows(bottoms[0]), None, self._gpu_label(bottoms), tops[0].diff, self._Hg)
            bottoms[0].diff = _sample_rows_back(g, bottoms[0])
            return
        if propagate_down[0]:
            g = -self.Hl / self.p * (tops[0].diff.float() / self.p.shape[0])
            bottoms[0].diff = g.reshape(bottoms[0].data.shape).to(bottoms[0].dtype)


@register("ContrastiveLoss")
class ContrastiveLossLayer(LossLayer, _RowLossGPU):
    exact_bottoms = 3
    kind = "Contrastive"

    def forward(self, bottoms, tops):
        p = self.lp.contrastive_loss_param
        if bottoms[0].data.is_cuda:
            n = bottoms[0].shape[0]
            a, b = bottoms[0].data.reshape(n, -1), bottoms[1].data.reshape(n, -1)
            self._y = bottoms[2].data.reshape(-1).float()
            tops[0].data = self.gpu_forward(a, b, self._y, None, p.margin, p.legacy_version).reshape(())
            return
        a = bottoms[0].data.float().reshape(bottoms[0].shape[0], -1)
        b = bottoms[1].data.float().reshape(a.shape)
        y = bottoms[2].data.float().reshape(-1)
        self.diff = a - b
        self.d2 = (self.diff * self.diff).sum(1)
        self.margin, self.legacy = p.margin, p.legacy_version
        if self.legacy:
            neg = torch.clamp(self.margin - self.d2, min=0)
        else:
            neg = torch.clamp(self.margin - torch.sqrt(self.d2), min=0) ** 2
        self.y = y
        loss = torch.where(y > 0, self.d2, neg).sum() / a.shape[0] / 2.0
        tops[0].data = loss.reshape(())

    def backward(self, tops, propagate_down, bottoms):
        if tops[0].diff.is_cuda:
            p = self.lp.contrastive_loss_param
            n = bottoms[0].shape[0]
            rows = [bottoms[i].data.reshape(n, -1) for i in range(2)]
            for i in range(2):
                if propagate_down[i]:
                    g = self.gpu_backward(rows[i], rows[1 - i], self._y, tops[0].diff, None, p.margin,
                                          p.legacy_version)
                    bottoms[i].diff = g.reshape(bottoms[i].data.shape)
            return
        n = self.diff.shape[0]
        lw = tops[0].diff.float() / n
        if self.legacy:
            negc = -(self.margin - self.d2 > 0).float()
        else:
            dist = torch.sqrt(self.d2)
            mdist = self.margin - dist
            negc = -(mdist > 0).float() * mdist / (dist + 1e-4)
        coef = torch.where(self.y > 0, torch.ones_like(self.d2), negc)[:, None]
        for i, sign in ((0, 1.0), (1, -1.0)):
            if propagate_down[i]:
                g = sign * lw * coef * self.diff
                bottoms[i].diff = g.reshape(bottoms[i].data.shape).to(bottoms[i].dtype)
```

### sparknet_amd/layers/vision.py

```python
from __future__ import annotations

import torch

from .. import ops, proto
from ..core.layer import Layer, register
from ..ops.spec import POOL_AVE, POOL_MAX, POOL_STOCHASTIC, ConvSpec, PoolSpec


def _conv_hw(cp, name, rep_name, h_name, w_name, default):
    if cp.HasField(h_name) or cp.HasField(w_name):
        return int(getattr(cp, h_name)), int(getattr(cp, w_name))
    rep = list(getattr(cp, rep_name))
    if len(rep) == 0:
        return default, default
    if len(rep) == 1:
        return int(rep[0]), int(rep[0])
    return int(rep[0]), int(rep[1])


def conv_geometry(cp):
    if cp.HasField("kernel_h") or cp.HasField("kernel_w"):
        kh, kw = cp.kernel_h, cp.kernel_w
    else:
        ks = list(cp.kernel_size)
# ... 344 lines not shown
                dx = ops.conv_backward(t.diff, b.data, w, s, bool(propagate_down[i]), dw, db, gate, ws,
                                       dw_acc=dw_acc, db_acc=db_acc)
            side, ws.fp8_dx_side_out = ws.fp8_dx_side_out, None
            if side is not None:
                self.fp8_dx_out[0]._fp8_dy_side = side
            if propagate_down[i]:
                b.diff = dx


@register("Deconvolution")
class DeconvolutionLayer(Layer):
    min_bottoms = 1
    min_tops = 1

    def layer_setup(self, bottoms, tops):
        cp = self.lp.convolution_param
        if conv_nd_mode(cp, bottoms[0]):
            self.__class__ = DeconvolutionNdLayer
            return self.layer_setup(bottoms, tops)
        self.R, self.S, self.sh, self.sw, self.ph, self.pw = conv_geometry(cp)
        self.K = int(cp.num_output)
        self.groups = int(cp.group)
        C = bottoms[0].shape[1]
        self.C = C
        Kg = self.K // self.groups
        self.weight = self.add_param((C, Kg, self.R, self.S), (C, self.R, self.S, Kg),
                                     to_caffe=lambda t: t.permute(0, 3, 1, 2),
                                     from_caffe=lambda t: t.permute(0, 2, 3, 1),
                                     filler=cp.weight_filler if cp.HasField("weight_filler") else None)
        self.bias = None
        if cp.bias_term:
            self.bias = self.add_param((self.K,), filler=cp.bias_filler if cp.HasField("bias_filler") else None)

    def out_hw(self, H, W):
        return ((H - 1) * self.sh + self.R - 2 * self.ph, (W - 1) * self.sw + self.S - 2 * self.pw)

    def fwd_spec(self, b):
        N, C, H, W = b.shape
        Ho, Wo = self.out_hw(H, W)
        return ConvSpec(N, Ho, Wo, self.K, C, self.R, self.S, self.sh, self.sw, self.ph, self.pw,
                        1, 1, self.groups)

    def reshape(self, bottoms, tops):
        for b, t in zip(bottoms, tops):
            N, C, H, W = b.shape
            Ho, Wo = self.out_hw(H, W)
            t.reshape((N, self.K, Ho, Wo), self.dtype)

    def _w_as_conv(self):
        return self.weight.compute

    def forward(self, bottoms, tops):
        for b, t in zip(bottoms, tops):
            s = self.fwd_spec(b)
            zeros = torch.zeros(t.data.shape, dtype=t.dtype, device=t.device)
            y = ops.conv_backward(b.data, zeros, self._w_as_conv(), s, True, None, None)
            if self.bias is not None:
                y = (y.float() + self.bias.data.float()).to(t.dtype)
            t.data = y

    def backward(self, tops, propagate_down, bottoms):
        dw = self.weight.diff if self.param_grads_needed(0) else None
        for i, (t, b) in enumerate(zip(tops, bottoms)):
            s = self.fwd_spec(b)
            if self.bias is not None and self.param_grads_needed(1):
                self.bias.diff += t.diff.float().reshape(-1, self.K).sum(0)
            if dw is not None:
                ops.conv_backward(b.data, t.diff, self._w_as_conv(), s, False, dw, None)
            if propagate_down[i]:
                b.diff = ops.conv_forward(t.diff, self._w_as_conv(), None, s)


@register("Pooling")
class PoolingLayer(Layer):
    exact_bottoms = 1
    min_tops = 1
    max_tops = 2

    def layer_setup(self, bottoms, tops):
        pp = self.lp.pooling_param
        self.global_pooling = pp.global_pooling
        if pp.HasField("kernel_h") or pp.HasField("kernel_w"):
            self.kh, self.kw = pp.kernel_h, pp.kernel_w
        else:
            self.kh = self.kw = pp.kernel_size
        if pp.HasField("pad_h") or pp.HasField("pad_w"):
            self.ph, self.pw = pp.pad_h, pp.pad_w
        else:
            self.ph = self.pw = pp.pad
        if pp.HasField("stride_h") or pp.HasField("stride_w"):
            self.sh, self.sw = pp.stride_h, pp.stride_w
        else:
            self.sh = self.sw = pp.stride
        self.method = int(pp.pool)
        if self.global_pooling:
            self.ph = self.pw = 0
            self.sh = self.sw = 1
        elif not self.kh or not self.kw:
            raise ValueError("Pooling: kernel size is required")
        self.aux = None

    relu_gate = False
    fused_lrn = None
    bwd_lrn = None
    fp8_out = None
    fp8_dx_out = None

    def _fp8_side(self, pair, shape, key, dev):
        sc = getattr(self.ctx, "fp8", None)
        if pair is None or sc is None or sc.updates == 0:
            return None
        from ..ops import gemm as _gemm
        parts = self.__dict__.setdefault("_fp8_parts", {})
        if key not in parts:
            parts[key] = _gemm.new_side_part(dev)
        i = pair[1]
        return _gemm.Fp8Side(torch.empty(shape, dtype=torch.bfloat16, device=dev), sc.slot(i), sc.is_e5m2(i),
                             parts[key])

    def spec(self, b) -> PoolSpec:
        N, C, H, W = b.shape
        kh, kw = (H, W) if self.global_pooling else (self.kh, self.kw)
        return PoolSpec(N, H, W, C, kh, kw, self.sh, self.sw, self.ph, self.pw, self.method)

    def reshape(self, bottoms, tops):
        s = self.spec(bottoms[0])
        tops[0].reshape((s.N, s.C, s.P, s.Q), self.dtype)
        if len(tops) > 1:
            tops[1].reshape((s.N, s.C, s.P, s.Q), self.dtype)

    def forward(self, bottoms, tops):
        s = self.spec(bottoms[0])
        x = bottoms[0].data
        if self.method == POOL_STOCHASTIC and x.is_cuda:
            from ..ops import layers_hip
            if getattr(self, "stream", None) is None:
                self.stream = self.ctx.next_stream_id()
            train = self.phase == proto.TRAIN
            tops[0].data, self.aux = layers_hip.stopool(x, s, self.ctx.rng_state, self.stream, train)
            return
        if self.method == POOL_STOCHASTIC:
            if self.phase == proto.TRAIN:
                wins = ops.ref._pool_windows(x.float(), s, 0.0)
                u = torch.rand(wins.shape[:4], generator=self.ctx.gen).to(wins.device)
                csum = wins.cumsum(-1)
                self.aux = (csum >= (u * csum[..., -1])[..., None]).to(torch.uint8).argmax(-1, keepdim=True)
                tops[0].data = ops.ref.nhwc(wins.gather(-1, self.aux).squeeze(-1)).to(x.dtype)
            else:
                tops[0].data = _stochastic_test(x.float().clamp_min(0), s).to(x.dtype)
            return
        f = self.fused_lrn
        if f is not None and x.is_cuda:
            from ..ops import hip
            tops[0].data, self.aux, f.top.data = hip.pool_lrn_forward(x, s, self.relu_gate, f.size, f.alpha, f.beta,
                                                                      f.k)
            return
        side = self._fp8_side(self.fp8_out, (s.N, s.P, s.Q, s.C), "fwd", x.device) if x.is_cuda else None
        if side is not None:
            from ..ops import hip
            y, self.aux = hip.pool_forward_mask(x, s, self.relu_gate, side=side)
            self.fp8_out[0]._fp8_x_side = side
        else:
            y, self.aux = ops.pool_forward_aux(x, s, self.relu_gate)
        tops[0].data = y
        if len(tops) > 1:
            tops[1].data = (self.aux.to(tops[1].dtype) if self.aux is not None
                            else torch.zeros_like(y))

    def backward(self, tops, propagate_down, bottoms):
        if not propagate_down[0]:
            return
        s = self.spec(bottoms[0])
        if self.method == POOL_STOCHASTIC and tops[0].diff.is_cuda:
            import dataclasses
            sm = dataclasses.replace(s, method=0)
            bottoms[0].diff = ops.pool_backward(tops[0].diff, bottoms[0].data, sm, self.aux)
            return
        if self.method == POOL_STOCHASTIC:
            xl = bottoms[0].data.float().requires_grad_(True)
            with torch.enable_grad():
                y = ops.ref._pool_windows(xl, s, 0.0).gather(-1, self.aux).squeeze(-1)
                g, = torch.autograd.grad(y, xl, ops.ref.nchw(tops[0].diff.float()))
            bottoms[0].diff = g.to(bottoms[0].dtype)
            return
        f = self.fused_lrn
        if f is not None and bottoms[0].data.is_cuda:
            from ..ops import hip
            bottoms[0].diff = hip.lrn_pool_backward(f.top.diff, tops[0].data, self.aux, s, f.size, f.alpha, f.beta,
                                                    f.k)
            return
        f = self.bwd_lrn
        if f is not None and self.aux is not None and self.fp8_dx_out is None and bottoms[0].data.is_cuda:
            from ..ops import hip
            f.bottom.diff = hip.pool_lrn_backward_rev(tops[0].diff, self.aux, f.bottom.data, s, f.size, f.alpha,
                                                      f.beta, f.k, f.relu_gate)
            f.bwd_done = True
            return
        side = (self._fp8_side(self.fp8_dx_out, (s.N, s.H, s.W, s.C), "bwd", bottoms[0].data.device)
                if bottoms[0].data.is_cuda else None)
        if side is not None:
            from ..ops import hip
            bottoms[0].diff = hip.pool_backward(tops[0].diff, bottoms[0].data, s, self.aux, tops[0].data,
                                                self.relu_gate, side=side, side_only=self.fp8_dx_only)
            self.fp8_dx_out[0]._fp8_dy_side = side
            return
        bottoms[0].diff = ops.pool_backward(tops[0].diff, bottoms[0].data, s, self.aux, tops[0].data,
                                            self.relu_gate)


def _stochastic_test(xf, s: PoolSpec):
    sq = ops.ref._pool_windows(xf * xf, s, 0.0).sum(-1)
    lin = ops.ref._pool_windows(xf, s, 0.0).sum(-1)
    out = torch.where(lin > 0, sq / lin.clamp_min(1e-30), torch.zeros_like(lin))
    return ops.ref.nhwc(out)


@register("LRN")
class LRNLayer(Layer):
    exact_bottoms = 1
    exact_tops = 1

    def layer_setup(self, bottoms, tops):
        p = self.lp.lrn_param
        self.size = int(p.local_size)
        if self.size % 2 == 0:
            raise ValueError("LRN only supports odd values for local_size")
        self.alpha, self.beta, self.k = float(p.alpha), float(p.beta), float(p.k)
        self.within = int(p.norm_region) == 1

    def reshape(self, bottoms, tops):
        tops[0].reshape(bottoms[0].shape, self.dtype)

    def forward(self, bottoms, tops):
        if self.pool_fused and bottoms[0].data.is_cuda:
            return
        tops[0].data = ops.lrn_forward(bottoms[0].data, self.size, self.alpha, self.beta, self.k, self.within)

    relu_gate = False
    pool_fused = False
    top = None
    bottom = None
    bwd_done = False

    def backward(self, tops, propagate_down, bottoms):
        if self.bwd_done:
            self.bwd_done = False
            return
        if not propagate_down[0] or (self.pool_fused and bottoms[0].data.is_cuda):
            return
        x = bottoms[0].data
        if self.relu_gate and x.is_cuda:
            from ..ops import hip
            bottoms[0].diff = hip.lrn_backward(tops[0].diff, x, self.size, self.alpha, self.beta, self.k,
                                               self.within, gate=True)
            return
        dx = ops.lrn_backward(tops[0].diff, x, self.size, self.alpha, self.beta, self.k, self.within, tops[0].data)
        bottoms[0].diff = ops.relu_backward(dx, x) if self.relu_gate else dx


@register("InnerProduct")
class InnerProductLayer(Layer):
    exact_bottoms = 1
    exact_tops = 1
    fuse_relu = False
    relu_gate = False
    supports_grad_overwrite = True

    def layer_setup(self, bottoms, tops):
        p = self.lp.inner_product_param
        self.N = int(p.num_output)
        b = bottoms[0]
        self.axis = b.canonical_axis(p.axis)
        self.Kdim = b.count_range(self.axis)
        self.perm = None
        if b.is_image and self.axis == 1 and b.shape[2] * b.shape[3] > 1:
            _, C, H, W = b.shape
            self.perm = (C, H, W)
        N, K = self.N, self.Kdim
        if self.perm is not None:
            C, H, W = self.perm
            to_caffe = lambda t: t.reshape(N, H, W, C).permute(0, 3, 1, 2).reshape(N, K)
            from_caffe = lambda t: t.reshape(N, C, H, W).permute(0, 2, 3, 1).reshape(N, K)
        else:
            to_caffe = from_caffe = None
        self.weight = self.add_param((N, K), (N, K), to_caffe, from_caffe,
                                     filler=p.weight_filler if p.HasField("weight_filler") else None)
        self.bias = None
        if p.bias_term:
            self.bias = self.add_param((N,), filler=p.bias_filler if p.HasField("bias_filler") else None)

    def reshape(self, bottoms, tops):
        b = bottoms[0]
        if b.count_range(self.axis) != self.Kdim:
            raise ValueError(f"{self.name}: input size incompatible with inner product parameters")
        tops[0].reshape(tuple(b.shape[:self.axis]) + (self.N,), self.dtype)

    def forward(self, bottoms, tops):
        b = bottoms[0]
        M = b.count_range(0, self.axis)
        x2 = b.data.reshape(M, self.Kdim)
        bias = self.bias.data if self.bias is not None else None
        d = self.fused_dropout
        drop = (d.ctx.rng_state, d.stream, d.ratio) if d is not None and x2.is_cuda and d.phase == 0 else None
        if self.fp8_slots is not None and x2.is_cuda:
            from ..ops import hip
            sc = self.ctx.fp8
            ix, iw = self.fp8_slots
            xq = hip.quant_fp8(x2, sc.slot(ix))
            wq = hip.quant_fp8(self.weight.compute, sc.slot(iw))
            y = hip.linear_forward_fp8(xq, wq, bias, sc.deq(ix), sc.deq(iw), relu=self.fuse_relu, dropout=drop)
        else:
            if drop is not None:
                from ..ops import hip
                y = hip.linear_forward(x2, self.weight.compute, bias, self.fuse_relu, dropout=drop)
            else:
                y = ops.linear_forward(x2, self.weight.compute, bias, self.fuse_relu)
        tops[0].data = y.reshape(tops[0].data.shape)

    fp8_slots = None
    fused_update = None
    fused_dropout = None
    gate_scale = 1.0

    def fp8_eligible(self, b) -> bool:
        return self.Kdim % 16 == 0

    def backward(self, tops, propagate_down, bottoms):
        b = bottoms[0]
        M = b.count_range(0, self.axis)
        dy2 = tops[0].diff.reshape(M, self.N)
        x2 = b.data.reshape(M, self.Kdim)
        dw = self.weight.diff if self.param_grads_needed(0) else None
        db = self.bias.diff if (self.bias is not None and self.param_grads_needed(1)) else None
        gate = b.data if self.relu_gate else None
        dw_acc = not (dw is not None and self.grad_overwrite(0))
        db_acc = not (db is not None and self.grad_overwrite(1))
        if self.fused_update is not None and dw is not None and x2.is_cuda:
            from ..ops import hip
            dx = hip.linear_backward_sgd(dy2, x2, self.weight.compute, bool(propagate_down[0]),
                                         self.fused_update.sgd(), db, gate, db_acc=db_acc, gate_scale=self.gate_scale)
        elif self.gate_scale != 1.0:
            from ..ops import hip
            dx = hip.linear_backward(dy2, x2, self.weight.compute, bool(propagate_down[0]), dw, db, gate,
                                     dw_acc=dw_acc, db_acc=db_acc, gate_scale=self.gate_scale)
        else:
            dx = ops.linear_backward(dy2, x2, self.weight.compute, bool(propagate_down[0]), dw, db, gate,
                                     dw_acc=dw_acc, db_acc=db_acc)
        if propagate_down[0]:
            b.diff = dx.reshape(b.data.shape)


@register("Im2col")
class Im2colLayer(Layer):
    exact_bottoms = 1
    exact_tops = 1

    def layer_setup(self, bottoms, tops):
        cp = self.lp.convolution_param
        if conv_nd_mode(cp, bottoms[0]):
            self.__class__ = Im2colNdLayer
            return self.layer_setup(bottoms, tops)
        self.R, self.S, self.sh, self.sw, self.ph, self.pw = conv_geometry(cp)

    def reshape(self, bottoms, tops):
        N, C, H, W = bottoms[0].shape
        P = (H + 2 * self.ph - self.R) // self.sh + 1
        Q = (W + 2 * self.pw - self.S) // self.sw + 1
        tops[0].reshape((N, C * self.R * self.S, P, Q), self.dtype)

    def _geom(self, b, t):
        N, C_, H, W = b.shape
        return (N, H, W, C_, t.shape[2], t.shape[3], self.R, self.S, self.sh, self.sw, self.ph, self.pw, 1, 1)

    def forward(self, bottoms, tops):
        if bottoms[0].data.is_cuda:
            from ..ops import layers_hip
            b, t = bottoms[0], tops[0]
            t.data = layers_hip.im2col_caffe(b.data, self._geom(b, t), t.data.shape)
            return
        xn = bottoms[0].nchw().float()
        cols = torch.nn.functional.unfold(xn, (self.R, self.S), padding=(self.ph, self.pw),
                                          stride=(self.sh, self.sw))
        N, CK, L = cols.shape
        t = tops[0]
        t.data = cols.reshape(N, CK, t.shape[2], t.shape[3]).permute(0, 2, 3, 1).contiguous().to(t.dtype)

    def backward(self, tops, propagate_down, bottoms):
        if not propagate_down[0]:
            return
        t, b = tops[0], bottoms[0]
        if t.diff.is_cuda:
            from ..ops import layers_hip
            b.diff = layers_hip.col2im_caffe(t.diff, self._geom(b, t), b.data.shape)
            return
        d = t.nchw(diff=True).float().reshape(t.shape[0], t.shape[1], -1)
        x = torch.nn.functional.fold(d, b.shape[2:], (self.R, self.S), padding=(self.ph, self.pw),
                                     stride=(self.sh, self.sw))
        b.diff = x.permute(0, 2, 3, 1).contiguous().to(b.dtype)


class Im2colNdLayer(_NdGeometry, Layer):
    type_name = "Im2colND"
    exact_bottoms = 1
    exact_tops = 1

    def layer_setup(self, bottoms, tops):
        self.nd_setup(self.lp.convolution_param, bottoms[0])

    def spec(self, b) -> ops.ConvNdSpec:
        num, C, ins = self.nd_split(b.shape)
        return ops.ConvNdSpec(num, C, 1, ins, self.ks, self.st, self.pd, 1)

    def reshape(self, bottoms, tops):
        b = bottoms[0]
        s = self.spec(b)
        tops[0].reshape(tuple(b.shape[:self.axis]) + (s.C * s.T,) + s.outs, self.dtype)

    def forward(self, bottoms, tops):
        b = bottoms[0]
        s = self.spec(b)
        x = _logical(b).reshape((s.num, s.C) + s.ins)
        CT = s.C * s.T
        if x.is_cuda:
            from ..ops import hip, layers_hip
            x = x.contiguous()
            col = torch.empty((s.num * s.P, CT), dtype=x.dtype, device=x.device)
            hip.call("im2col_nd", x, col, s.nd, s.num, s.C, s.C, 0, CT, hip._nd_dims(s), hip._nd_dt(x),
                     hip._nd_dt(col))
            y = layers_hip.transpose(col, s.num, s.P, CT)
        else:
            y = ops.ref.im2col_nd(x.float(), s).reshape(s.num, s.P, CT).transpose(1, 2)
        _store_logical(tops[0], y)

    def backward(self, tops, propagate_down, bottoms):
        if not propagate_down[0]:
            return
        b, t = bottoms[0], tops[0]
        s = self.spec(b)
        CT = s.C * s.T
        dy = _logical(t, diff=True).reshape(s.num, CT, s.P)
        if dy.is_cuda:
            from ..ops import hip, layers_hip
            dcol = layers_hip.transpose(dy.contiguous(), s.num, CT, s.P)
            dx = torch.empty((s.num, s.C) + s.ins, dtype=dy.dtype, device=dy.device)
            hip.call("col2im_nd", dcol, dx, s.nd, s.num, s.C, s.C, 0, CT, hip._nd_dims(s), hip._nd_dt(dcol),
                     hip._nd_dt(dx), 0)
        else:
            x = _logical(b).reshape((s.num, s.C) + s.ins).float().detach().requires_grad_(True)
            col = ops.ref.im2col_nd(x, s).reshape(s.num, s.P, CT).transpose(1, 2)
            dx, = torch.autograd.grad(col, x, dy.float())
        _store_logical(b, dx, diff=True)


__all__ = ["ConvolutionLayer", "DeconvolutionLayer", "PoolingLayer", "LRNLayer", "InnerProductLayer",
           "Im2colLayer", "POOL_MAX", "POOL_AVE"]
```

### sparknet_amd/ops/__init__.py

```python
from __future__ import annotations

import contextlib
import threading

import torch

from . import ref
from .spec import POOL_AVE, POOL_MAX, POOL_STOCHASTIC, ConvNdSpec, ConvSpec, PoolSpec

_hip = None
_state = threading.local()


def _hipmod():
    global _hip
    if _hip is None:
        from . import hip as _h
        _hip = _h
    return _hip


def f32_active() -> bool:
    return getattr(_state, "f32", False)


@contextlib.contextmanager
def precision(dtype):
    prev = f32_active()
    _state.f32 = dtype == torch.float32
    try:
        yield
    finally:
        _state.f32 = prev


def _gpu(t: torch.Tensor) -> bool:
    return t.is_cuda and not f32_active()


def _impl(t: torch.Tensor):
    if not t.is_cuda:
        return ref
    if f32_active():
        from . import f32dev
        return f32dev
    return _hipmod()


def _dispatch(name):
    def fn(first, *args, **kwargs):
        return getattr(_impl(first), name)(first, *args, **kwargs)
    fn.__name__ = name
    return fn


conv_forward = _dispatch("conv_forward")
conv_backward = _dispatch("conv_backward")
conv_nd_forward = _dispatch("conv_nd_forward")
conv_nd_backward = _dispatch("conv_nd_backward")
linear_forward = _dispatch("linear_forward")
linear_backward = _dispatch("linear_backward")
pool_forward = _dispatch("pool_forward")
lrn_forward = _dispatch("lrn_forward")
lrn_backward = _dispatch("lrn_backward")
relu_forward = _dispatch("relu_forward")
relu_backward = _dispatch("relu_backward")
softmax_forward = _dispatch("softmax_forward")
softmax_backward = _dispatch("softmax_backward")
accuracy = _dispatch("accuracy")


def pool_backward(dy, x, s, aux=None, y=None, gate=False):
    if _gpu(dy):
        return _hipmod().pool_backward(dy, x, s, aux, y, gate)
    if dy.is_cuda:
        from . import f32dev
        return f32dev.pool_backward(dy, x, s, aux, y, gate)
    return ref.pool_backward(dy, x, s, gate)


def pool_forward_aux(x, s, gate=False):
    if _gpu(x):
        return _hipmod().pool_forward_mask(x, s, gate)
    if x.is_cuda:
        from . import f32dev
        return f32dev.pool_forward_aux(x, s, gate)
    return ref.pool_forward(x, s), None


def dropout_forward(x, ratio, rng_state, stream):
    if _gpu(x):
        return _hipmod().dropout_forward(x, ratio, rng_state, stream)
    if x.is_cuda:
        from . import f32dev
        return f32dev.dropout_forward(x, ratio, rng_state, stream)
    seed, counter = (int(v) for v in rng_state.tolist())
    return ref.dropout_forward(x, ratio, seed, counter, stream)


def dropout_backward(dy, ratio, rng_state, stream, gate=None):
    if _gpu(dy):
        return _hipmod().dropout_backward(dy, ratio, rng_state, stream, gate)
    if dy.is_cuda:
        from . import f32dev
        return f32dev.dropout_backward(dy, ratio, rng_state, stream, gate)
    seed, counter = (int(v) for v in rng_state.tolist())
    return ref.dropout_backward(dy, ratio, seed, counter, stream, gate)


def softmax_loss_forward(x2, labels, ignore_label=None, normalize=True, outer_num=None):
    return _impl(x2).softmax_loss_forward(x2, labels, ignore_label, normalize, outer_num)


def softmax_loss_backward(prob, labels, loss_weight, norm, ignore_label=None, dtype=torch.float32):
    return _impl(prob).softmax_loss_backward(prob, labels, loss_weight, norm, ignore_label, dtype)


def sum_bf16(tensors):
    return _hipmod().sum_bf16([t.contiguous() for t in tensors])


def cast_f32_to_bf16(src: torch.Tensor, dst: torch.Tensor) -> None:
    if src.is_cuda:
        _hipmod().cast_f32_to_bf16(src, dst)
    else:
        dst.copy_(src)


def advance_rng(rng_state: torch.Tensor) -> None:
    if rng_state.is_cuda:
        _hipmod().advance_rng(rng_state)
    else:
        rng_state[1] += 1


def solver_tables(segments, total: int, device, slab_chunks=None) -> dict:
    device = torch.device(device)
    if device.type == "cuda":
        return _hipmod().solver_tables(segments, total, device, slab_chunks)
    assert not slab_chunks
    lr = torch.zeros(max(total, 1))
    dc = torch.zeros(max(total, 1))
    for off, cnt, lm, dm in segments:
        lr[off:off + cnt] = lm
        dc[off:off + cnt] = dm
    return {"lr": lr, "decay": dc}


def solver_update(kind, data, diff, history, compute, tables, hyper, l1: bool, clip: bool,
                  grid_limit: int = 0) -> None:
    if data.is_cuda:
        _hipmod().solver_update(kind, data, diff, history, compute, tables, hyper, l1, clip, grid_limit)
        return
    h = hyper.tolist()
    ref.solver_update_ref(kind, data, diff, history, tables["lr"], tables["decay"], h, l1, clip)
    if compute is not None and compute is not data:
        compute.copy_(data)
```

### sparknet_amd/ops/gemm.py

```python
from __future__ import annotations

import ast
import contextlib
import ctypes as C
import json
import os
from dataclasses import dataclass, field, replace

import torch

from . import _lib
from ..utils import features

OP_DENSE, OP_IM2COL, OP_FLIPW = 0, 1, 2
EPI_BF16, EPI_F32, EPI_F32_ACC, EPI_SGD, EPI_BF16_DROP = 0, 1, 2, 3, 4
BM = BN = 128
BK = 64


@dataclass
class Dense:
    t: torch.Tensor
    ld: int
    kcontig: bool
    gstride: int = 0


@dataclass
class ConvGeom:
    N: int
    H: int
    W: int
    C: int
    P: int
    Q: int
    R: int
    S: int
    sh: int = 1
    sw: int = 1
    ph: int = 0
    pw: int = 0
    dh: int = 1
    dw: int = 1
    Cg: int = 0

    def c_struct(self) -> _lib.SnConvGeom:
        return _lib.SnConvGeom(self.N, self.H, self.W, self.C, self.P, self.Q, self.R, self.S,
                               self.sh, self.sw, self.ph, self.pw, self.dh, self.dw, self.Cg)


@dataclass
class Im2col:
    x: torch.Tensor
    geom: ConvGeom
    kcontig: bool
    gstride: int = 0


@dataclass
class FlipW:
    w: torch.Tensor
    Kg: int
    R: int
    S: int
    Cg: int


FP8 = torch.uint8


@dataclass
class Operand:
    s: _lib.SnOperand
    mc: int
    mode: int


def _operand(op, fp8: bool = False) -> Operand:
    elt = FP8 if fp8 else torch.bfloat16
    if isinstance(op, FlipW):
        assert op.w.dtype == torch.bfloat16 and op.w.is_contiguous() and op.Cg % 8 == 0
        g = _lib.SnConvGeom(0, 0, 0, op.Kg, 1, 1, op.R, op.S, 1, 1, 0, 0, 1, 1, op.Cg)
        s = _lib.SnOperand(op.w.data_ptr(), 0, op.Kg * op.R * op.S * op.Cg, g)
        return Operand(s, 1, OP_FLIPW)
    if isinstance(op, Dense):
        assert op.t.dtype == elt, (op.t.dtype, elt)
        assert op.t.data_ptr() % 16 == 0 and (op.ld * op.t.element_size()) % 16 == 0, \
            "dense operand must be 16-B aligned"
        s = _lib.SnOperand(op.t.data_ptr(), op.ld, op.gstride, _lib.SnConvGeom())
        return Operand(s, 0 if op.kcontig else 1, OP_DENSE)
    g = op.geom
    assert op.x.dtype == elt and (op.x.is_contiguous() or (
        op.x.dim() == 4 and op.x.stride(-1) == 1 and op.x.stride(2) == g.C and op.x.shape[-1] <= g.C)), \
        "implicit conv operand must be NHWC (contiguous or a channel slice with pixel stride C)"
    cm = 16 if fp8 else 8
    assert g.Cg % cm == 0 and g.C % cm == 0, f"implicit conv needs channels % {cm} == 0"
    assert g.N * g.P * g.Q < (1 << 24) and g.N * g.H * g.W < (1 << 24), "conv too large for one launch"
    assert g.N * g.H * g.W * g.C < (1 << 31), "implicit conv uses 32-bit element offsets"
    assert op.x.data_ptr() % 16 == 0, "implicit conv operand must be 16-B aligned"
    s = _lib.SnOperand(op.x.data_ptr(), 0, op.gstride, g.c_struct())
    return Operand(s, 0 if op.kcontig else 1, OP_IM2COL)


TILES = {0: (128, 128), 1: (256, 64), 2: (256, 128), 3: (128, 256), 4: (128, 96), 5: (256, 48),
         6: (256, 256), 7: (256, 128), 10: (128, 64),
         11: (256, 256), 12: (256, 128), 13: (256, 128), 14: (256, 192), 15: (128, 192), 16: (192, 128),
         17: (192, 96), 18: (192, 64), 19: (128, 128), 20: (128, 64), 21: (64, 256), 22: (64, 128)}
_SLOTS = {6: 256, 7: 256, 10: 768, 11: 256, 12: 256, 13: 256, 14: 256, 19: 256, 20: 512, 21: 512, 22: 768}
_KTILE_US = {6: 2.0, 7: 1.1, 11: 2.0, 12: 1.1, 13: 1.1, 14: 1.55}
_FORCE_TILE = int(os.environ.get("SN_GEMM_TILE", "-1"))


def choose_tile(M: int, N: int, b_kcontig: bool = False) -> int:
    if N <= 64 and M >= 256:
        return 5 if N % 48 == 0 and N % 64 != 0 else 1
    if b_kcontig and N % 96 == 0 and N % 128 != 0 and M >= 128:
        return 4
    return 0


SLOTS = 512
KTILE_US = 1.25
BLOCK_OVERHEAD = 4
REDUCE_BW = 5e12


def _cost(tiles: int, ktiles: int, s: int, out_elems: int, tile: int = 0) -> float:
    kt = -(-ktiles // s)
    t = -(-tiles * s // _SLOTS.get(tile, SLOTS)) * (kt + BLOCK_OVERHEAD) * _KTILE_US.get(tile, KTILE_US)
    if s > 1:
        t += (out_elems * 4.0 * (s + 1)) / REDUCE_BW * 1e6 + 3.0
    return t


def choose_splits(M: int, N: int, K: int, groups: int = 1, tile: int = 0) -> tuple[int, int]:
    bm, bn = TILES[tile]
    tiles = -(-M // bm) * -(-N // bn) * groups
    ktiles = -(-K // BK)
    ws_cap = max(1, (256 << 20) // max(1, 4 * M * N * groups))
    smax = max(1, min(256, ktiles // 4, ws_cap))
    best, best_t = 1, _cost(tiles, ktiles, 1, M * N * groups, tile)
    for s in range(2, smax + 1):
        t = _cost(tiles, ktiles, s, M * N * groups, tile)
        if t < best_t * 0.98:
            best, best_t = s, t
    kchunk = -(-K // best)
    kchunk = -(-kchunk // BK) * BK
    splits = -(-K // kchunk)
    return splits, kchunk


@dataclass
class GemmCall:
    M: int
    N: int
    K: int
    groups: int
    a: Operand
    b: Operand
    epi: int
    out: torch.Tensor
    ldc: int
    c_gstride: int = 0
    bias: torch.Tensor | None = None
    relu: bool = False
    gate: torch.Tensor | None = None
    gate_scale: float = 1.0
    bias_grad: torch.Tensor | None = None
    bias_acc: bool = True
    ones: int = -1
    sgd: dict | None = None
    dropout: tuple | None = None
    deq_a: torch.Tensor | None = None
    deq_b: torch.Tensor | None = None
    fp8_format: int = 0

    @property
    def fp8(self) -> bool:
        return self.fp8_format != 0

    @property
    def bk(self) -> int:
        return 128 if self.fp8_format else BK

    @property
    def b_kc_dense(self) -> bool:
        return self.b.mc == 0 and self.b.mode == OP_DENSE

    @property
    def key(self) -> tuple:
        a, b, f8 = self.a, self.b, self.fp8_format
        return (self.M, self.N, self.K, self.groups, a.mc, a.mode, b.mc, b.mode, self.epi, self.gate is not None,
                self.bias_grad is not None, self.dropout is not None, _geom_key(a.s), _geom_key(b.s),
                *(("fp8",) if f8 == 1 else ("fp8", f8) if f8 else ()), self.out.dtype)


@dataclass
class SplitSlabs:
    ws: torch.Tensor = field(compare=False)
    base: int
    splits: int
    M: int
    N: int
    ldw: int
    groups: int
    ones: int
    ldc: int
    c_gstride: int


def gemm(M: int, N: int, K: int, A, B, out: torch.Tensor, ldc: int, *, epi: int,
         groups: int = 1, c_gstride: int = 0, bias: torch.Tensor | None = None, relu: bool = False,
         splits: int | None = None, gate: torch.Tensor | None = None,
         deq: tuple[torch.Tensor, torch.Tensor] | None = None,
         bias_grad: torch.Tensor | None = None, bias_acc: bool = True, sgd: dict | None = None,
         dropout: tuple | None = None, gate_scale: float = 1.0) -> None:
    if M == 0 or N == 0:
        return
    if epi == EPI_SGD:
        assert sgd is not None and groups == 1 and deq is None
        splits = 1
    deq_a, deq_b, fp8 = (*deq, 1)[:3] if deq is not None else (None, None, 0)
    a, b = _operand(A, bool(fp8)), _operand(B, bool(fp8))
    ones = -1
    if bias_grad is not None:
        assert epi in (EPI_F32, EPI_F32_ACC, EPI_SGD) and b.mc == 1 and b.mode != OP_FLIPW and N % 8 == 0
        assert not fp8 or (a.mc == 1 and N % 16 == 0)
        assert bias_grad.dtype == torch.float32 and bias_grad.is_contiguous() and bias_grad.numel() == groups * M
        ones, N = N, N + 1
    assert bias is None or (bias.dtype == torch.float32 and bias.is_contiguous())
    assert gate is None or (epi == EPI_BF16 and gate.dtype == torch.bfloat16)
    assert dropout is None or epi == EPI_BF16
    call =GemmCall(M, N, K, groups, a, b, epi, out, ldc, c_gstride, bias, relu, gate, float(gate_scale),
                    bias_grad, bias_acc, ones, sgd if epi == EPI_SGD else None, dropout, deq_a, deq_b, fp8)
    if splits is not None or _FORCE_TILE >= 0:
        tile, model_splits, kchunk = _model_config(call, _FORCE_TILE)
        if splits is None:
            splits = model_splits
        else:
            kchunk = _kchunk(K, splits, call.bk)
    else:
        tile, splits, kchunk = _tuned_config(call)
    _launch(call, tile, splits, kchunk)


def _kchunk(K: int, splits: int, bk: int) -> int:
    return -(-(-(-K // splits)) // bk) * bk


def _model_config(c: GemmCall, force: int = -1) -> tuple[int, int, int]:
    if c.fp8:
        tile = force if (force in _FP8_TILES and not (c.a.mc or c.b.mc)) else 0
    else:
        tile = force if force >= 0 else choose_tile(c.M, c.N, c.b_kc_dense)
    if c.epi == EPI_SGD and tile not in (0, 1, 2, 3):
        tile = 0
    _, kchunk = choose_splits(c.M, c.N, c.K * BK // c.bk, c.groups, tile)
    kchunk = kchunk * c.bk // BK
    return tile, -(-c.K // kchunk), kchunk


_LDS_EPI = True
_LDS_EPI_TILES = frozenset((0, 1, 4, 5, 10, 12, 13, 14, 15, 16, 17, 18, 19, 20))


def _ptr(t) -> int:
    return t.data_ptr() if t is not None else 0


def _gemm_args(c: GemmCall, tile: int, **fields) -> _lib.SnGemmArgs:
    bm, bn = TILES[tile]
    tm, tn = -(-c.M // bm), -(-c.N // bn)
    args = _lib.SnGemmArgs(M=c.M, N=c.N, K=c.K, groups=c.groups, a_mc=c.a.mc, a_mode=c.a.mode, b_mc=c.b.mc,
                           b_mode=c.b.mode, A=c.a.s, B=c.b.s, tile=tile, fp8=c.fp8_format, deq_a=_ptr(c.deq_a),
                           deq_b=_ptr(c.deq_b), raster_n=int(1 < tn <= 8 and tm >= 8 * tn), ones_col=c.ones,
                           **fields)
    if c.sgd is not None:
        s = c.sgd
        args.sgd_w, args.sgd_h, args.sgd_shadow, args.sgd_hyper = (s[k].data_ptr() for k in ("w", "h", "shadow", "hyper"))
        args.sgd_lr_mult, args.sgd_decay_mult, args.sgd_flags = float(s["lr_mult"]), float(s["decay_mult"]), int(s["flags"])
    return args


def _launch(c: GemmCall, tile: int, splits: int, kchunk: int) -> None:
    M, N, out = c.M, c.N, c.out
    splits = max(1, -(-c.K // kchunk))
    rng, dstream, ratio = c.dropout or (None, 0, 0.0)
    dstream, ratio = int(dstream), float(ratio)
    if splits == 1:
        e = EPI_BF16_DROP if rng is not None else c.epi
        lds = int(_LDS_EPI and c.epi == EPI_BF16 and tile in _LDS_EPI_TILES and c.ldc % 8 == 0 and c.c_gstride % 8 == 0
                  and out.data_ptr() % 16 == 0)
        thr, scale = (int(4294967295 * ratio) & 0xffffffff, 1.0 / (1.0 - ratio)) if rng is not None else (0, 1.0)
        args = _gemm_args(c, tile, splits=1, kchunk=max(kchunk, c.bk), epi=e, C=out.data_ptr(), ldc=c.ldc,
                          c_gstride=c.c_gstride, bias=_ptr(c.bias), relu=int(c.relu), gate=_ptr(c.gate),
                          gate_scale=c.gate_scale, bias_out=_ptr(c.bias_grad), bias_acc=int(c.bias_acc),
                          drop_rng=_ptr(rng), drop_stream=dstream, drop_thr=thr, drop_scale=scale, lds_store=lds)
        side = _SIDE
        if side is not None and side.covers(out):
            q = _side_fields(side, c, tile, e, lds)
            if q is not None:
                args.q_out, args.q_ld, args.q_gstride, args.q_slot, args.q_e5m2, args.q_part = q
        _lib.check(_lib.kernels().sn_gemm(C.byref(args), C.c_void_p(_lib.stream_ptr())), "gemm")
        if _lib.DEBUG_SYNC:
            _lib.debug_sync("gemm")
        return
    if _SIDE is not None and _SIDE.covers(out):
        _SIDE.ok = False
    ldw = -(-N // 4) * 4
    sink = _DEFER_SINK
    deferred = (sink is not None and c.epi == EPI_F32 and not c.fp8 and (c.bias_grad is None or not c.bias_acc)
                and sink.accepts(out, c.bias_grad))
    ws = (sink.slab(c.groups * splits * M * ldw, out.device).view(c.groups, splits, M, ldw) if deferred
          else torch.empty((c.groups, splits, M, ldw), dtype=torch.float32, device=out.device))
    args = _gemm_args(c, tile, splits=splits, kchunk=kchunk, epi=EPI_F32, C=ws.data_ptr(), ldc=ldw,
                      c_gstride=splits * M * ldw, c_split_stride=M * ldw, drop_scale=1.0, gate_scale=1.0)
    _lib.check(_lib.kernels().sn_gemm(C.byref(args), C.c_void_p(_lib.stream_ptr())), "gemm")
    if deferred:
        sink.record(SplitSlabs(ws, ws.data_ptr(), splits, M, N - (1 if c.ones >= 0 else 0), ldw, c.groups, c.ones,
                               c.ldc, c.c_gstride))
        return
    mode = {EPI_BF16: 0, EPI_F32: 1, EPI_F32_ACC: 2}[c.epi]
    _lib.call("splitk_reduce", ws, splits, M * ldw, M, N, ldw, out, c.ldc, mode, c.bias, int(c.relu),
              c.groups, splits * M * ldw, c.c_gstride, c.gate, c.bias_grad, c.ones, int(c.bias_acc), M,
              C.c_void_p(_ptr(rng)), dstream, ratio, c.gate_scale)




class Fp8Side:
    def __init__(self, base: torch.Tensor, slot: torch.Tensor, e5m2: bool = False, part: torch.Tensor | None = None):
        assert base.is_contiguous() and base.dtype == torch.bfloat16
        self.base = base
        self.q = torch.empty(base.shape, dtype=torch.uint8, device=base.device)
        self.slot = slot
        self.e5m2 = bool(e5m2)
        self.ok = True
        self.only = False
        self.launches = 0
        self.part = part if part is not None else new_side_part(base.device)

    def finish(self) -> None:
        if self.launches:
            _lib.call("fp8_fold_amax", self.part, self.slot)

    def covers(self, out: torch.Tensor) -> bool:
        b = self.base.data_ptr()
        return out.dtype == torch.bfloat16 and b <= out.data_ptr() < b + 2 * self.base.numel()

    @property
    def complete(self) -> bool:
        return self.ok and self.launches > 0

    def matches(self, x: torch.Tensor) -> bool:
        return self.complete and x.data_ptr() == self.base.data_ptr() and x.numel() == self.base.numel()


def new_side_part(device) -> torch.Tensor:
    return torch.zeros(256 * 32, dtype=torch.float32, device=device)


_SIDE = None
_SIDE_FRAG = features.enabled("fp8_side_frag")
SIDE_STATS = {"used": 0, "missed": 0}


def side_bytes(side, x: torch.Tensor, e5m2: bool = False):
    if side is None:
        return None
    if side.matches(x) and side.e5m2 == bool(e5m2):
        SIDE_STATS["used"] += 1
        return side.q
    SIDE_STATS["missed"] += 1
    return None


@contextlib.contextmanager
def fp8_side_output(side):
    global _SIDE
    prev, _SIDE = _SIDE, side
    try:
        yield side
    finally:
        _SIDE = prev
    side.finish()


def _side_fields(side, c, tile, epi, lds):
    off = (c.out.data_ptr() - side.base.data_ptr()) // 2
    qp = side.q.data_ptr() + off
    if ((not lds and not _SIDE_FRAG) or epi not in (EPI_BF16, EPI_BF16_DROP) or tile in (6, 7)
            or c.N % 8 or c.ldc % 8 or c.c_gstride % 8 or qp % 8):
        side.ok = False
        return None
    side.launches += 1
    return (qp, c.ldc, c.c_gstride, side.slot.data_ptr(), int(side.e5m2), side.part.data_ptr())


_DEFER_SINK = None


class defer_reduce:
    def __init__(self, sink):
        self.sink = sink

    def __enter__(self):
        global _DEFER_SINK
        self.prev, _DEFER_SINK = _DEFER_SINK, self.sink
        self.sink.begin()
        return self.sink

    def __exit__(self, *exc):
        global _DEFER_SINK
        _DEFER_SINK = self.prev
        self.sink.end()
        return False


_AUTOTUNE = os.environ.get("SN_GEMM_AUTOTUNE", "0") == "1"
_TUNED: dict = {}
_MISSES: set = set()
_TUNE_LOG = os.environ.get("SN_GEMM_TUNE_LOG", "0") == "1"
_TUNE_PASSES = 3
_THIN = True
_DB_PATH = os.environ.get("SN_GEMM_TUNE_DB", os.path.join(os.path.dirname(os.path.abspath(__file__)),
                                                          "gemm_tuned.json"))


def _key_to_str(key) -> str:
    return repr(key[:-1] + (str(key[-1]).replace("torch.", ""),))


def _key_from_str(s: str):
    k = ast.literal_eval(s)
    return k[:-1] + (getattr(torch, k[-1]),)


def load_tune_db(path: str | None = None) -> int:
    path = path or _DB_PATH
    if not path or path == "0" or not os.path.exists(path):
        return 0
    with open(path) as f:
        db = json.load(f)
    for k, v in db.items():
        _TUNED[_key_from_str(k)] = tuple(int(x) for x in v)
    return len(db)


def save_tune_db(path: str) -> int:
    db = {}
    if os.path.exists(path):
        with open(path) as f:
            db = json.load(f)
    db.update({_key_to_str(k): list(v) for k, v in _TUNED.items()})
    with open(path, "w") as f:
        json.dump(dict(sorted(db.items())), f, indent=0)
    return len(db)


load_tune_db()


def _geom_key(s) -> tuple:
    return (s.ld, s.gstride) + tuple(getattr(s.g, f) for f, _ in s.g._fields_)


def _candidates(c: GemmCall) -> list:
    M, N, K, groups, b_kc_dense, epi = c.M, c.N, c.K, c.groups, c.b_kc_dense, c.epi
    tiles = [0, 1, 2]
    if N >= 256:
        tiles.append(3)
    if epi != EPI_SGD and M >= 256:
        tiles.append(7)
        if N > 128:
            tiles.append(6)
    if epi != EPI_SGD and M >= 256 and N > 64:
        tiles += [12, 13]
        if N > 128:
            tiles.append(11)
        if N > 128 and (b_kc_dense or N % 192 == 0):
            tiles.append(14)
    if epi != EPI_SGD and N > 64:
        tiles.append(16)
        if b_kc_dense and N > 128:
            tiles.append(15)
    if epi != EPI_SGD and M >= 192:
        tiles.append(18)
        if b_kc_dense and N % 96 == 0:
            tiles.append(17)
    if epi != EPI_SGD and N >= 64:
        tiles.append(20)
    if _THIN and (M <= 64 or -(-M // 64) * 64 < -(-M // 128) * 128):
        tiles += [21, 22]
    if epi != EPI_SGD:
        tiles.append(10)
        if b_kc_dense and N % 96 == 0:
            tiles.append(4)
        if N % 48 == 0 and N <= 96 and M >= 256:
            tiles.append(5)
    out = []
    for t in tiles:
        s, kc = choose_splits(M, N, K, groups, t)
        out.append((t, s, kc))
        if epi == EPI_SGD:
            continue
        for s2 in {1, 2 * s} - {s}:
            kc2 = _kchunk(K, s2, BK)
            s2 = max(1, -(-K // kc2))
            if s2 * M * N * groups * 4 <= (256 << 20):
                out.append((t, s2, kc2))
    return list(dict.fromkeys(out))


_FP8_TILES = (0, 11, 16)


def _candidates_fp8(c: GemmCall) -> list:
    M, N, K, groups = c.M, c.N, c.K, c.groups
    out = []
    for t in ((0,) if (c.a.mc or c.b.mc) else _FP8_TILES):
        if t != 0 and (c.dropout is not None or c.epi not in (EPI_BF16, EPI_F32)):
            continue
        s, kc = choose_splits(M, N, K // 2, groups, t)
        for s2 in dict.fromkeys((s, 1)):
            kc2 = _kchunk(K, s2, 128)
            s2 = max(1, -(-K // kc2))
            if s2 == 1 or s2 * M * N * groups * 4 <= (256 << 20):
                out.append((t, s2, kc2))
    return list(dict.fromkeys(out))


def _tuned_config(c: GemmCall) -> tuple[int, int, int]:
    M, N, K, groups, epi, out = c.M, c.N, c.K, c.groups, c.epi, c.out
    key = c.key
    hit = _TUNED.get(key)
    if hit is None and not _AUTOTUNE and epi != EPI_SGD:
        _MISSES.add(key)
    if hit is not None:
        return hit
    default = tile, splits, _ = _model_config(c)
    extent = (groups - 1) * c.c_gstride + (M - 1) * c.ldc + (N - (1 if c.ones >= 0 else 0))
    if (not _AUTOTUNE or epi == EPI_SGD or not out.is_cuda or torch.cuda.is_current_stream_capturing()
            or (out.is_contiguous() and extent > out.numel())):
        return default
    scratch = torch.empty_like(out) if out.is_contiguous() else torch.empty(extent, dtype=out.dtype, device=out.device)
    trial = replace(c, out=scratch, bias_grad=torch.zeros_like(c.bias_grad) if c.bias_grad is not None else None)
    times = {}
    for cand in (_candidates_fp8(c) if c.fp8 else _candidates(c)):
        try:
            _launch(trial, *cand)
        except RuntimeError as e:
            if _TUNE_LOG:
                print(f"[gemm-tune] candidate {cand} skipped: {e}", flush=True)
            continue
        times[cand] = float("inf")
    torch.cuda.synchronize(out.device)
    est = _cost(-(-M // TILES[tile][0]) * -(-N // TILES[tile][1]) * groups, -(-K // BK), splits, M * N * groups, tile)
    reps = max(4, min(32, int(150.0 / max(est, 1.0))))
    for _ in range(_TUNE_PASSES):
        for cand in times:
            torch.cuda._sleep(1 << 19)
            e0, e1 = torch.cuda.Event(enable_timing=True), torch.cuda.Event(enable_timing=True)
            e0.record()
            for _ in range(reps):
                _launch(trial, *cand)
            e1.record()
            e1.synchronize()
            times[cand] = min(times[cand], e0.elapsed_time(e1))
    best = min(times, key=times.get) if times else default
    if default in times and times[best] > 0.97 * times[default]:
        best = default
    if _TUNE_LOG:
        print(f"[gemm-tune] M={M} N={N} K={K} g={groups} modes={(c.a.mc, c.a.mode)}/{(c.b.mc, c.b.mode)} epi={epi} "
              f"default={default} best={best} " +
              " ".join(f"{k[0]}/{k[1]}:{v * 1000 / reps:.1f}" for k, v in sorted(times.items())), flush=True)
    _TUNED[key] = best
    return best


def set_autotune(on: bool) -> None:
    global _AUTOTUNE
    _AUTOTUNE = bool(on)


def tune_misses() -> list:
    return sorted(_MISSES, key=repr)


def sync_tuned(comm) -> int:
    import torch.distributed as dist
    if (comm is None or not getattr(comm, "active", False) or comm.world_size <= 1
            or not (dist.is_available() and dist.is_initialized())):
        return 0
    payload = [{_key_to_str(k): list(v) for k, v in _TUNED.items()} if comm.rank == 0 else None]
    dist.broadcast_object_list(payload, src=0)
    for ks, v in payload[0].items():
        _TUNED[_key_from_str(ks)] = tuple(v)
    return len(payload[0])



def _pad8(t: torch.Tensor, dim: int) -> torch.Tensor:
    n = t.shape[dim]
    if n % 8 == 0 and t.is_contiguous() and t.data_ptr() % 16 == 0:
        return t
    pad = (-n) % 8
    shape = list(t.shape)
    shape[dim] = n + pad
    out = torch.zeros(shape, dtype=t.dtype, device=t.device)
    out.narrow(dim, 0, n).copy_(t)
    return out


def linear_fwd(x: torch.Tensor, w: torch.Tensor, bias: torch.Tensor | None = None,
               relu: bool = False, out: torch.Tensor | None = None, dropout: tuple | None = None) -> torch.Tensor:
    M, K = x.shape
    N = w.shape[0]
    xp, wp = _pad8(x, 1), _pad8(w, 1)
    Kp = xp.shape[1]
    if out is None:
        out = torch.empty((M, N), dtype=torch.bfloat16, device=x.device)
    if dropout is not None:
        assert out.is_contiguous()
    gemm(M, N, Kp, Dense(xp, Kp, True), Dense(wp, Kp, True), out, out.stride(0), epi=EPI_BF16,
         bias=bias, relu=relu, dropout=dropout)
    return out


def linear_dgrad(dy: torch.Tensor, w: torch.Tensor, out: torch.Tensor | None = None,
                 gate: torch.Tensor | None = None, gate_scale: float = 1.0) -> torch.Tensor:
    M, N = dy.shape
    K = w.shape[1]
    dyp = _pad8(dy, 1)
    Np = dyp.shape[1]
    wp = w
    if Np != N or K % 8 or not w.is_contiguous():
        wp = torch.zeros((Np, -(-K // 8) * 8), dtype=w.dtype, device=w.device)
        wp[:N, :K].copy_(w)
    Kp = wp.shape[1]
    o = out if out is not None and Kp == K else torch.empty((M, Kp), dtype=torch.bfloat16, device=dy.device)
    fused = gate is None or (Kp == K and gate.is_contiguous())
    gemm(M, Kp, Np, Dense(dyp, Np, True), Dense(wp, Kp, False), o, o.stride(0), epi=EPI_BF16,
         gate=gate if fused else None, gate_scale=gate_scale if fused else 1.0)
    if not fused:
        o = o[:, :K] * (gate > 0).to(o.dtype) * gate_scale
    elif o is not out:
        o = o[:, :K]
    if out is not None and o is not out:
        out.copy_(o)
        return out
    return o


def linear_wgrad(dy: torch.Tensor, x: torch.Tensor, dw: torch.Tensor, accumulate: bool = True,
                 db: torch.Tensor | None = None, db_acc: bool = True) -> bool:
    M, N = dy.shape
    K = x.shape[1]
    dyp, xp = _pad8(dy, 1), _pad8(x, 1)
    Np, Kp = dyp.shape[1], xp.shape[1]
    if Np == N and Kp == K and dw.is_contiguous():
        fuse = db is not None and db.is_contiguous() and db.dtype == torch.float32
        gemm(N, K, M, Dense(dyp, Np, False), Dense(xp, Kp, False), dw, K,
             epi=EPI_F32_ACC if accumulate else EPI_F32, bias_grad=db if fuse else None, bias_acc=db_acc)
        return fuse
    tmp = torch.zeros((Np, Kp), dtype=torch.float32, device=dw.device)
    gemm(Np, Kp, M, Dense(dyp, Np, False), Dense(xp, Kp, False), tmp, Kp, epi=EPI_F32)
    if accumulate:
        dw.add_(tmp[:N, :K])
    else:
        dw.copy_(tmp[:N, :K])
    return False


def linear_wgrad_sgd(dy: torch.Tensor, x: torch.Tensor, sgd: dict, db: torch.Tensor | None = None,
                     db_acc: bool = True) -> bool:
    M, N = dy.shape
    K = x.shape[1]
    assert N % 8 == 0 and K % 8 == 0 and dy.is_contiguous() and x.is_contiguous()
    fuse = db is not None and db.is_contiguous() and db.dtype == torch.float32
    w = sgd["w"]
    gemm(N, K, M, Dense(dy, N, False), Dense(x, K, False), w, K, epi=EPI_SGD, sgd=sgd,
         bias_grad=db if fuse else None, bias_acc=db_acc)
    return fuse


def colsum(x: torch.Tensor, out: torch.Tensor, accumulate: bool = True) -> None:
    M, N = x.shape
    c8 = -(-N // 8)
    cl = 1
    while cl < c8 and cl < 64:
        cl *= 2
    cblocks = -(-c8 // cl)
    rl = 256 // cl
    nparts = max(1, min(max(1, 1024 // cblocks), -(-M // (2 * rl))))
    part = torch.empty((nparts, N), dtype=torch.float32, device=x.device)
    _lib.call("colsum_bf16", x, M, N, x.stride(0), part, nparts, out, int(accumulate))
```

### sparknet_amd/ops/hip.py

```python
from __future__ import annotations

import contextlib
import ctypes as C
import dataclasses
import os
from typing import NamedTuple

import torch

from . import _lib
from ..utils import features
from .gemm import (EPI_BF16, EPI_F32, EPI_F32_ACC, ConvGeom, Dense, FlipW, Fp8Side, Im2col, colsum, fp8_side_output,
                   gemm, linear_dgrad, linear_fwd, linear_wgrad, side_bytes)
from .spec import POOL_MAX, ConvNdSpec, ConvSpec, PoolSpec

call = _lib.call
BF16 = torch.bfloat16
DGRAD_INPLACE_WEIGHTS = False


def _c(t: torch.Tensor) -> torch.Tensor:
    return t if t.is_contiguous() else t.contiguous()


# ... 640 lines not shown
    lh.axis_copy(t, tmp, s.num, chans, per, s.P, g * per, 0, per)
    return lh.transpose(tmp, s.num, per, s.P).view(s.num * s.P, per)


def conv_nd_forward(x, w, b, s: ConvNdSpec):
    from . import layers_hip as lh
    x = _c(x)
    CT = s.Cg * s.T
    y = torch.empty((s.num, s.K, s.P), dtype=BF16, device=x.device)
    for g in range(s.groups):
        col = _nd_col(x, s, g)
        wg = torch.zeros((s.Kg, col.shape[1]), dtype=BF16, device=x.device)
        wg[:, :CT] = w[g * s.Kg:(g + 1) * s.Kg].reshape(s.Kg, CT)
        bg = b[g * s.Kg:(g + 1) * s.Kg].float().contiguous() if b is not None else None
        yc = linear_fwd(col, wg, bg)
        if s.groups == 1:
            y = lh.transpose(yc, s.num, s.P, s.Kg, out_shape=(s.num, s.K, s.P))
        else:
            lh.axis_copy(lh.transpose(yc, s.num, s.P, s.Kg), y, s.num, s.Kg, s.K, s.P, 0, g * s.Kg, s.Kg)
    return y.view((s.num, s.K) + s.outs)


def conv_nd_backward(dy, x, w, s: ConvNdSpec, need_dx: bool, dw=None, db=None):
    dy = _c(dy).to(BF16)
    if x is not None:
        x = _c(x)
    assert x is not None or dw is None, "the weight gradient needs the input"
    CT = s.Cg * s.T
    dx = torch.empty((s.num, s.C) + s.ins, dtype=dy.dtype, device=dy.device) if need_dx else None
    for g in range(s.groups):
        dyc = _nd_chan_cl(dy, s, s.K, g, s.Kg)
        if dw is not None:
            col = _nd_col(x, s, g)
            dwg = dw.view(s.K, CT)[g * s.Kg:(g + 1) * s.Kg]
            dbg = db[g * s.Kg:(g + 1) * s.Kg] if db is not None else None
            if not linear_wgrad(dyc, col[:, :CT], dwg, accumulate=True, db=dbg, db_acc=True) and dbg is not None:
                colsum(dyc, dbg, accumulate=True)
        elif db is not None:
            colsum(dyc, db[g * s.Kg:(g + 1) * s.Kg], accumulate=True)
        if need_dx:
            wg = w[g * s.Kg:(g + 1) * s.Kg].reshape(s.Kg, CT).contiguous()
            dcol = linear_dgrad(dyc, wg)
            call("col2im_nd", dcol, dx, s.nd, s.num, s.C, s.Cg, g * s.Cg, dcol.stride(0), _nd_dims(s), 0,
                 _nd_dt(dx), 0)
    return dx



def _pool_args(s: PoolSpec):
    return (s.N, s.H, s.W, s.C, s.P, s.Q, s.kh, s.kw, s.sh, s.sw, s.ph, s.pw, s.method)


_MAX_ELEMS = 1 << 31


def _pool_images(s: PoolSpec) -> int:
    per = s.H * s.W * s.C
    return s.N if s.N * per < _MAX_ELEMS else max(1, (_MAX_ELEMS - 1) // per)


def pool_side_ok(s: PoolSpec, backward: bool) -> bool:
    if s.C % 8:
        return False
    if not backward:
        return s.method == POOL_MAX and s.kh == s.kw and s.kh in (2, 3)
    nh, nw = -(-s.kh // s.sh), -(-s.kw // s.sw)
    return not (s.kh == 3 and s.kw == 3 and s.sh == 2 and s.sw == 2) and nh == nw and 1 <= nh <= 3


def _side_args(side, t, n0, n1):
    if side is None:
        return (None, None, None, 0)
    return (side.q[n0:n1], side.slot, side.part, int(side.e5m2))


def pool_forward_mask(x, s: PoolSpec, gate: bool = False, side=None):
    x = _c(x)
    if side is not None:
        assert pool_side_ok(s, False) and tuple(side.base.shape) == (s.N, s.P, s.Q, s.C)
        y = side.base
    else:
        y = torch.empty((s.N, s.P, s.Q, s.C), dtype=BF16, device=x.device)
    mask = torch.empty((s.N, s.P, s.Q, s.C), dtype=torch.uint8, device=x.device) if s.method == POOL_MAX else None
    nb = _pool_images(s)
    for n0 in range(0, s.N, nb):
        n1 = min(s.N, n0 + nb)
        call("pool_fwd", x[n0:n1], y[n0:n1], mask[n0:n1] if mask is not None else None,
             *_pool_args(dataclasses.replace(s, N=n1 - n0)), int(gate and s.method == POOL_MAX),
             *_side_args(side, y, n0, n1))
    if side is not None:
        side.launches += 1
        side.finish()
    return y, mask


def pool_forward(x, s: PoolSpec):
    return pool_forward_mask(x, s)[0]


def pool_backward(dy, x, s: PoolSpec, mask=None, y=None, gate=False, side=None, side_only=False):
    if side_only:
        assert side is not None and s.method == POOL_MAX
        side.only = True
    if side is not None:
        assert pool_side_ok(s, True) and not (gate and s.method != POOL_MAX)
        assert tuple(side.base.shape) == (s.N, s.H, s.W, s.C)
        dx = side.base
    else:
        dx = torch.empty((s.N, s.H, s.W, s.C), dtype=BF16, device=dy.device)
    if s.method == POOL_MAX and mask is None:
        _, mask = pool_forward_mask(x, s, gate)
    dy = _c(dy)
    nb = _pool_images(s)
    for n0 in range(0, s.N, nb):
        n1 = min(s.N, n0 + nb)
        call("pool_bwd", dy[n0:n1], mask[n0:n1] if mask is not None else None, None if side_only else dx[n0:n1],
             *_pool_args(dataclasses.replace(s, N=n1 - n0)), *_side_args(side, dx, n0, n1))
    if side is not None:
        side.launches += 1
        side.finish()
    if gate and s.method != POOL_MAX:
        dx = relu_backward(dx, x)
    return dx


def pool_lrn_eligible(s: PoolSpec, size: int, within: bool) -> bool:
    if s.method != POOL_MAX or within or (s.kh, s.kw, s.sh, s.sw) != (3, 3, 2, 2) or s.C % 8 or size not in (3, 5, 7, 9):
        return False
    if s.ph >= 3 or s.pw >= 3 or s.N * s.H * s.W * s.C >= 1 << 32:
        return False
    fn = _lib.kernels().sn_pool_lrn_supported
    fn.restype = C.c_int
    return bool(fn(*(C.c_longlong(v) for v in (s.N, s.H, s.W, s.C, s.P, s.Q, s.ph, s.pw, size))))


def pool_lrn_forward(x, s: PoolSpec, gate: bool, size: int, alpha: float, beta: float, k: float):
    x = _c(x)
    pooled = torch.empty((s.N, s.P, s.Q, s.C), dtype=BF16, device=x.device)
    mask = torch.empty((s.N, s.P, s.Q, s.C), dtype=torch.uint8, device=x.device)
    y = torch.empty_like(pooled)
    call("pool_lrn_fwd", x, pooled, mask, y, s.N, s.H, s.W, s.C, s.P, s.Q, s.ph, s.pw, int(gate), int(size),
         float(alpha), float(beta), float(k))
    return pooled, mask, y


def lrn_pool_backward(dy, pooled, mask, s: PoolSpec, size: int, alpha: float, beta: float, k: float):
    dx = torch.empty((s.N, s.H, s.W, s.C), dtype=BF16, device=dy.device)
    call("lrn_pool_bwd", _c(pooled), _c(dy), mask, dx, s.N, s.H, s.W, s.C, s.P, s.Q, s.ph, s.pw, int(size),
         float(alpha), float(beta), float(k))
    return dx


def pool_lrn_rev_eligible(s: PoolSpec, size: int, within: bool) -> bool:
    if s.method != POOL_MAX or within or (s.kh, s.kw, s.sh, s.sw) != (3, 3, 2, 2) or s.C % 8 or size not in (3, 5, 7, 9):
        return False
    if s.ph >= 3 or s.pw >= 3 or s.N * s.H * s.W * s.C >= 1 << 32 or s.C > 8192:
        return False
    if 2 * (s.P - 1) - s.ph >= s.H or 2 * (s.Q - 1) - s.pw >= s.W:
        return False
    return (s.H + s.ph + 1) // 2 <= s.P + 1 and (s.W + s.pw + 1) // 2 <= s.Q + 1


def pool_lrn_backward_rev(dy, mask, x, s: PoolSpec, size: int, alpha: float, beta: float, k: float,
                          gate: bool = False):
    x = _c(x)
    assert tuple(x.shape) == (s.N, s.H, s.W, s.C) and tuple(mask.shape) == (s.N, s.P, s.Q, s.C)
    dx = torch.empty_like(x)
    call("pool_lrn_bwd_rev", _c(dy), _c(mask), x, dx, s.N, s.H, s.W, s.C, s.P, s.Q, s.ph, s.pw, int(size),
         float(alpha), float(beta), float(k), int(gate))
    return dx


def lrn_forward(x, size, alpha, beta, k, within=False):
    x = _c(x)
    N, H, W, Cc = x.shape
    y = torch.empty_like(x)
    if within:
        call("lrn_within_fwd", x, y, None, N, H, W, Cc, size, float(alpha), float(beta))
    else:
        call("lrn_across_fwd", x, y, N, H, W, Cc, size, float(alpha), float(beta), float(k))
    return y


def lrn_backward(dy, x, size, alpha, beta, k, within=False, y=None, gate=False):
    x, dy = _c(x), _c(dy)
    N, H, W, Cc = x.shape
    dx = torch.empty_like(x)
    if within:
        sbuf = torch.empty(x.shape, dtype=torch.float32, device=x.device)
        u = torch.empty(x.shape, dtype=torch.float32, device=x.device)
        call("lrn_within_bwd", x, dy, sbuf, u, dx, N, H, W, Cc, size, float(alpha), float(beta))
        if gate:
            dx = relu_backward(dx, x)
    else:
        call("lrn_across_bwd", x, dy, dx, N, H, W, Cc, size, float(alpha), float(beta), float(k), int(gate))
    return dx



def relu_forward(x, slope=0.0):
    x = as_bf16(x)
    y = torch.empty_like(x)
    call("relu_fwd", x, y, x.numel(), float(slope))
    return y


def relu_backward(dy, x, slope=0.0):
    dy, x = as_bf16(dy), as_bf16(x)
    dx = torch.empty_like(dy)
    call("relu_bwd", dy, x, dx, x.numel(), float(slope))
    return dx


def _dropout(x, ratio, rng_state, stream, gate=None):
    x = as_bf16(x)
    y = torch.empty_like(x)
    call("dropout", x, y, x.numel(), rng_state, int(stream), float(ratio), as_bf16(gate))
    return y


def dropout_forward(x, ratio, rng_state, stream):
    return _dropout(x, ratio, rng_state, stream)


def dropout_backward(dy, ratio, rng_state, stream, gate=None):
    return _dropout(dy, ratio, rng_state, stream, gate)


def cast_f32_to_bf16(src, dst):
    call("cast_f32_bf16", src, dst, src.numel())


def advance_rng(rng_state):
    call("advance_rng", rng_state)


def concat_channels(parts, out):
    pix = out.numel() // out.shape[-1]
    parts = [_c(t) for t in parts]
    assert sum(t.shape[-1] for t in parts) == out.shape[-1] and all(t.numel() // t.shape[-1] == pix for t in parts)
    _concat(parts, None, [t.shape[-1] for t in parts], out, pix, 0)
    return out


def concat_channels_bwd(dy, diffs, gates, chans):
    dy = _c(dy)
    pix = dy.numel() // dy.shape[-1]
    assert sum(chans) == dy.shape[-1]
    for d, g, c in zip(diffs, gates, chans):
        assert d is None or (d.is_contiguous() and d.shape[-1] == c and d.numel() // c == pix)
        assert g is None or (g.is_contiguous() and d is not None and g.shape == d.shape)
    _concat(diffs, gates, chans, dy, pix, 1)


def _concat(parts, gates, chans, top, pix, bwd):
    n = len(parts)
    P = (C.c_void_p * 8)(*[(t.data_ptr() if t is not None else 0) for t in parts] + [0] * (8 - n))
    G = (C.c_void_p * 8)(*[(g.data_ptr() if g is not None else 0) for g in (gates or [None] * n)] + [0] * (8 - n))
    Ch = (C.c_longlong * 8)(*list(chans) + [0] * (8 - n))
    _lib.check(_lib.kernels().sn_concat_nhwc(P, G, Ch, C.c_longlong(n), C.c_void_p(top.data_ptr()),
                                             C.c_longlong(pix), C.c_longlong(bwd), C.c_void_p(_lib.stream_ptr())),
               "concat_nhwc")
    if _lib.DEBUG_SYNC:
        _lib.debug_sync("concat_nhwc")


def sum_bf16(tensors, out=None):
    out = torch.empty_like(tensors[0]) if out is None else out
    n = out.numel()
    for i in range(0, len(tensors), 8):
        chunk = [_c(t) for t in tensors[i:i + 8]]
        if i:
            chunk = [out] + chunk[:7]
        arr = (C.c_void_p * 8)(*[t.data_ptr() for t in chunk] + [0] * (8 - len(chunk)))
        _lib.check(_lib.kernels().sn_sum_bf16(arr, C.c_longlong(len(chunk)), C.c_void_p(out.data_ptr()),
                                              C.c_longlong(n), C.c_void_p(_lib.stream_ptr())), "sum_bf16")
    return out



def softmax_loss_forward(x2, labels, ignore_label=None, normalize=True, outer_num=None):
    x2 = as_bf16(x2)
    M, Cn = x2.shape
    dev = x2.device
    prob = torch.empty((M, Cn), dtype=torch.float32, device=dev)
    rows = torch.empty((2, M), dtype=torch.float32, device=dev)
    out = torch.empty(2, dtype=torch.float32, device=dev)
    lab = _c(labels.reshape(-1).float())
    call("softmax_xent_fwd", x2, lab, prob, rows[0], rows[1], out[0:1], out[1:2], M, Cn,
         int(ignore_label is not None), int(ignore_label or 0), int(normalize),
         int(outer_num if outer_num is not None else M))
    return out[0], prob, out[1:2]


def softmax_loss_backward(prob, labels, loss_weight, norm, ignore_label=None, dtype=BF16):
    M, Cn = prob.shape
    dx = torch.empty((M, Cn), dtype=BF16, device=prob.device)
    lw = loss_weight.reshape(-1).float()
    call("softmax_xent_bwd", prob, _c(labels.reshape(-1).float()), lw, norm, dx, M, Cn,
         int(ignore_label is not None), int(ignore_label or 0))
    return dx if dtype == BF16 else dx.to(dtype)


def softmax_forward(x2):
    x2 = as_bf16(x2)
    y = torch.empty_like(x2)
    call("softmax_fwd", x2, y, x2.shape[0], x2.shape[1])
    return y


def softmax_backward(dy2, y2):
    dy2, y2 = as_bf16(dy2), as_bf16(y2)
    dx = torch.empty_like(y2)
    call("softmax_bwd", dy2, y2, dx, y2.shape[0], y2.shape[1])
    return dx


def accuracy(x2, labels, top_k=1, ignore_label=None):
    x2 = as_bf16(x2)
    M, Cn = x2.shape
    rows = torch.empty((2, M), dtype=torch.float32, device=x2.device)
    out = torch.empty(2, dtype=torch.float32, device=x2.device)
    call("accuracy", x2, _c(labels.reshape(-1).float()), rows[0], rows[1], out[0:1], out[1:2], M, Cn,
         int(top_k), int(ignore_label is not None), int(ignore_label or 0))
    return out[0]



CHUNK = 8192


def solver_tables(segments, total: int, device, slab_chunks=None) -> dict:
    pos, mult, src = [], [], []
    slab_chunks = slab_chunks or {}
    for off, cnt, lm, dm in segments:
        if off in slab_chunks:
            for start, n, ptr, ss, splits, es in slab_chunks[off]:
                for s in range(0, n, CHUNK):
                    pos.append((start + s, min(CHUNK, n - s)))
                    mult.append((lm, dm))
                    src.append((ptr + 4 * s * es, ss, splits, es))
            continue
        padded = -(-cnt // 64) * 64
        for s in range(0, padded, CHUNK):
            pos.append((off + s, min(CHUNK, padded - s)))
            mult.append((lm, dm))
            src.append((0, 0, 0, 0))
    nparts = max(1, min(1024, -(-total // (256 * 16))))
    return {
        "pos": torch.tensor(pos or [(0, 0)], dtype=torch.int64, device=device),
        "mult": torch.tensor(mult or [(0.0, 0.0)], dtype=torch.float32, device=device),
        "src": (torch.tensor(src, dtype=torch.int64, device=device) if slab_chunks and src else None),
        "n": len(pos),
        "part": torch.empty(nparts, dtype=torch.float32, device=device),
        "total": total,
    }


def solver_update(kind, data, diff, history, compute, tables, hyper, l1, clip, grid_limit=0):
    h0 = history[0]
    h1 = history[1] if len(history) > 1 else history[0]
    call("solver_update", int(kind), data, diff, h0, h1, compute, tables["pos"], tables["mult"], tables["n"],
         hyper, int(l1), int(clip), tables["part"], tables["part"].numel(), tables["total"], int(grid_limit),
         tables.get("src"))


def scale_shadow(flat, shadow, scale: float):
    call("scale_shadow", flat, shadow, flat.numel(), float(scale))



def s2d_plan(s: ConvSpec):
    return _s2d_plan(s)


def _labels(labels, label_out):
    if labels is None:
        return None, None
    assert labels.dtype == torch.int32 and label_out.dtype == torch.float32 and label_out.numel() == labels.numel()
    return _c(labels), label_out


def augment_s2d(src_u8, x2, crop, plan, s: ConvSpec, mean=None, mean_mode=0, scale=1.0, rng_state=None,
                train=True, mirror=False, labels=None, label_out=None):
    N, Cc, Hs, Ws = src_u8.shape
    f, cp, rf, sf, s2 = plan
    assert tuple(x2.shape) == (N, s2.H, s2.W, s2.C) and x2.dtype == BF16 and x2.is_contiguous()
    assert s.C == Cc and s.H == crop and s.W == crop
    assert labels is None or labels.numel() == N
    call("augment_s2d", _c(src_u8), x2, N, Cc, Hs, Ws, crop, crop, mean, int(mean_mode), float(scale), rng_state,
         int(train), int(mirror), s2.H, s2.W, f, cp, s.ph, s.pw, *_labels(labels, label_out))
    return x2


def augment(src_u8, dst, crop, mean=None, mean_mode=0, scale=1.0, rng_state=None, train=True, mirror=False,
            offs_out=None, labels=None, label_out=None):
    N, Cc, Hs, Ws = src_u8.shape
    assert labels is None or labels.numel() == N
    call("augment_f32" if dst.dtype == torch.float32 else "augment", _c(src_u8), dst, N, Cc, Hs, Ws, crop, crop,
         mean, int(mean_mode), float(scale), rng_state, int(train), int(mirror), offs_out,
         *_labels(labels, label_out))
    return dst



FP8_MARGIN = float(os.environ.get("SN_FP8_MARGIN", "1.0"))
FP8_HISTORY = int(os.environ.get("SN_FP8_HISTORY", "16"))


E4M3_MAX, E5M2_MAX = 448.0, 57344.0


class Fp8Scales:

    def __init__(self, n: int, device):
        self.updates = 0
        self.slots = torch.zeros((max(n, 1), 8), dtype=torch.float32, device=device)
        self.slots[:, 0] = 1.0
        self.slots[:, 2] = 1.0
        self.slots[:, 4] = E4M3_MAX
        self.n = n
        self._e5m2 = set()
        self.history = FP8_HISTORY
        self.hist = torch.zeros((max(n, 1), max(1, self.history)), dtype=torch.float32, device=device)

    def set_e5m2(self, i: int) -> None:
        self.slots[i, 4] = E5M2_MAX
        self._e5m2.add(i)

    def is_e5m2(self, i: int) -> bool:
        return i in self._e5m2

    def slot(self, i: int) -> torch.Tensor:
        return self.slots[i]

    def deq(self, i: int) -> torch.Tensor:
        return self.slots[i, 2:3]

    def update(self) -> None:
        call("fp8_update_scales", self.slots, self.hist, int(self.history), self.n, float(FP8_MARGIN))
        self.updates += 1


def quant_fp8(x: torch.Tensor, slot: torch.Tensor, out: torch.Tensor | None = None,
              e5m2: bool = False) -> torch.Tensor:
    x = _c(x)
    q = torch.empty(x.shape, dtype=torch.uint8, device=x.device) if out is None else out
    call("quant_fp8", x, q, x.numel(), slot, bool(e5m2))
    return q


def conv_forward_fp8(xq, wq, b, s: ConvSpec, deq_x, deq_w, relu=False, out=None):
    assert s.Cg % 16 == 0 and s.C % 16 == 0 and xq.dtype == torch.uint8 and wq.dtype == torch.uint8
    nb = _image_chunk(s)
    if nb < s.N:
        y = out if out is not None else torch.empty((s.N, s.P, s.Q, s.K), dtype=BF16, device=xq.device)
        for n0 in range(0, s.N, nb):
            n1 = min(s.N, n0 + nb)
            conv_forward_fp8(xq[n0:n1], wq, b, s.with_batch(n1 - n0), deq_x, deq_w, relu, out=y[n0:n1])
        return y
    M = s.N * s.P * s.Q
    kred = s.R * s.S * s.Cg
    y = out if out is not None else torch.empty((s.N, s.P, s.Q, s.K), dtype=BF16, device=xq.device)
    assert y.is_contiguous()
    if direct_fp8_ok(s) and not _side_covers(y):
        call("conv3x3_fp8", _c(xq), _c(wq), deq_x, deq_w, b, None, y, s.N, s.H, s.W, int(relu))
        return y
    A = Im2col(xq, _geom(s), kcontig=True, gstride=s.Cg)
    B = Dense(wq.view(s.K, kred), kred, True, gstride=s.Kg * kred)
    gemm(M, s.Kg, kred, A, B, y, s.K, epi=EPI_BF16, groups=s.groups, c_gstride=s.Kg, bias=b, relu=relu,
         deq=(deq_x, deq_w))
    return y


def linear_forward_fp8(xq, wq, b, deq_x, deq_w, relu=False, dropout=None):
    M, K = xq.shape
    N = wq.shape[0]
    assert K % 16 == 0
    y = torch.empty((M, N), dtype=BF16, device=xq.device)
    gemm(M, N, K, Dense(xq, K, True), Dense(wq, K, True), y, N, epi=EPI_BF16, bias=b, relu=relu,
         deq=(deq_x, deq_w), dropout=dropout)
    return y
```

### sparknet_amd/utils/features.py

```python
from __future__ import annotations

import os

DEFAULTS = {
    "fuse_pool_lrn": True,
    "fuse_lrn_pool_bwd": True,
    "zero_copy_concat": True,
    "fuse_dropout": True,
    "fuse_fp8_quant": True,
    "fuse_bn_scale": True,
    "branch_depfree": True,
    "fuse_splitk": False,
    "conv_direct_c64": True,
    "conv_direct_k96": True,
    "conv_direct96": True,
    "conv_packed": True,
    "conv_packed44": True,
    "conv_packed11": False,
    "conv_packed_k64": True,
    "conv_direct_fp8": True,
    "conv_depthwise": True,
    "fp8_wgrad_bias": True,
    "fp8_side_frag": True,
    "fp8_dx_only": True,
}

_cache: tuple[str, dict] = ("", {})


def _parsed() -> dict:
    global _cache
    raw = os.environ.get("SN_FEATURES", "")
    if raw != _cache[0]:
        out = {}
        for item in filter(None, (p.strip() for p in raw.split(","))):
            name, _, val = item.partition("=")
            if name not in DEFAULTS:
                raise ValueError(f"SN_FEATURES: unknown switch {name!r} (known: {', '.join(sorted(DEFAULTS))})")
            out[name] = val.strip().lower() not in ("0", "false", "off", "no")
        _cache = (raw, out)
    return _cache[1]


def enabled(name: str) -> bool:
    if name not in DEFAULTS:
        raise KeyError(name)
    return _parsed().get(name, DEFAULTS[name])
```

Measured before the change: 120,100 images/sec.

## Fuse final FC split-K reduce with softmax-xent head and fold loss reduce into solver

Adds a fused kernel that takes the last inner-product layer's split-K workspace, reduces it with bias, writes logits, and computes softmax, per-row loss and the loss gradient in one launch per row. It also folds the cross-entropy loss reduction and the RNG advance into an extra block of the solver update kernel. Both are enabled by default through new feature switches. The aim is to remove several small kernel launches and the round trips of logits and probabilities through global memory at the network head, at the cost of more complex control flow and one block per row with 1024 threads.

```diff
diff --git a/csrc/kernels/reduce.hip b/csrc/kernels/reduce.hip
--- a/csrc/kernels/reduce.hip
+++ b/csrc/kernels/reduce.hip
@@ -1,4 +1,5 @@
 #include "common.h"
+#include "reduce_order.h"
 
 struct ReduceOut {
   void* out;
@@ -70,31 +71,9 @@
   for (long long i = blockIdx.x * (long long)blockDim.x + threadIdx.x; i < total;
        i += (long long)gridDim.x * blockDim.x) {
     const int r = (int)(i / cols4), c = (int)(i - (long long)r * cols4) * 4;
-    float acc[4] = {0.f, 0.f, 0.f, 0.f};
     const bool vec = (c + 3 < cols) && ((ldw & 3) == 0);
     const float* p0 = wsg + (long long)r * ldw + c;
-    if (vec) {
-      int s = 0;
-      for (; s + 3 < splits; s += 4) {
-        float4 v[4];
-#pragma unroll
-        for (int u = 0; u < 4; ++u) v[u] = *reinterpret_cast<const float4*>(p0 + (s + u) * sstride);
-#pragma unroll
-        for (int u = 0; u < 4; ++u) {
-          acc[0] += v[u].x; acc[1] += v[u].y; acc[2] += v[u].z; acc[3] += v[u].w;
-        }
-      }
-      for (; s < splits; ++s) {
-        const float4 v = *reinterpret_cast<const float4*>(p0 + s * sstride);
-        acc[0] += v.x; acc[1] += v.y; acc[2] += v.z; acc[3] += v.w;
-      }
-    } else {
-      for (int s = 0; s < splits; ++s)
-#pragma unroll
-        for (int k = 0; k < 4; ++k)
-          if (c + k < cols) acc[k] += p0[s * sstride + k];
-    }
-    reduce_store(o, g, r, c, make_float4(acc[0], acc[1], acc[2], acc[3]));
+    reduce_store(o, g, r, c, splitk_sum_serial(p0, splits, sstride, vec, cols - c));
   }
 }
 
@@ -113,31 +92,12 @@
     r = (int)(i / cols4);
     c = (int)(i - (long long)r * cols4) * 4;
     const float* p = ws + g * ws_gstride + (long long)r * ldw + c;
-    int s = sl;
-    for (; s + 48 < splits; s += 64) {
-      float4 v[4];
-#pragma unroll
-      for (int u = 0; u < 4; ++u) v[u] = *reinterpret_cast<const float4*>(p + (s + 16 * u) * sstride);
-#pragma unroll
-      for (int u = 0; u < 4; ++u) {
-        acc.x += v[u].x; acc.y += v[u].y; acc.z += v[u].z; acc.w += v[u].w;
-      }
-    }
-    for (; s < splits; s += 16) {
-      float4 v = *reinterpret_cast<const float4*>(p + s * sstride);
-      acc.x += v.x; acc.y += v.y; acc.z += v.z; acc.w += v.w;
-    }
+    acc = splitk_lane_partial(p, acc, sl, splits, sstride);
   }
   red[sl][it] = acc;
   __syncthreads();
   if (sl == 0 && i < total) {
-    float a[4] = {0.f, 0.f, 0.f, 0.f};
-#pragma unroll
-    for (int q = 0; q < 16; ++q) {
-      float4 v = red[q][it];
-      a[0] += v.x; a[1] += v.y; a[2] += v.z; a[3] += v.w;
-    }
-    reduce_store(o, g, r, c, make_float4(a[0], a[1], a[2], a[3]));
+    reduce_store(o, g, r, c, splitk_lane_combine(&red[0][it], 16));
   }
 }
 
@@ -159,7 +119,7 @@
   o.extra = extra; o.extra_col = (int)extra_col; o.extra_acc = (int)extra_acc; o.extra_gstride = extra_gstride;
   if (extra && (mode == 0 || extra_col != cols - 1)) return 5;
   long long total = rows * ((cols + 3) / 4);
-  if (splits >= 16 && ((cols & 3) == 0 || ldw >= ((cols + 3) & ~3LL)) && (ldw & 3) == 0) {
+  if (splitk_wide_order(splits, cols, ldw)) {
     dim3 grid((unsigned)((total + 15) / 16), (unsigned)groups);
     hipLaunchKernelGGL(splitk_reduce_wide, grid, dim3(256), 0, st, ws, (int)splits, sstride, (int)rows, ldw,
                        ws_gstride, o);
diff --git a/csrc/kernels/reduce_order.h b/csrc/kernels/reduce_order.h
--- /dev/null
+++ b/csrc/kernels/reduce_order.h
@@ -0,0 +1,87 @@
+#pragma once
+#include "common.h"
+
+static inline bool splitk_wide_order(long long splits, long long cols, long long ldw) {
+  return splits >= 16 && ((cols & 3) == 0 || ldw >= ((cols + 3) & ~3LL)) && (ldw & 3) == 0;
+}
+
+SN_DEV float4 splitk_sum_serial(const float* __restrict__ p0, int splits, long long sstride, bool vec, int nvalid) {
+  float acc[4] = {0.f, 0.f, 0.f, 0.f};
+  if (vec) {
+    int s = 0;
+    for (; s + 3 < splits; s += 4) {
+      float4 v[4];
+#pragma unroll
+      for (int u = 0; u < 4; ++u) v[u] = *reinterpret_cast<const float4*>(p0 + (s + u) * sstride);
+#pragma unroll
+      for (int u = 0; u < 4; ++u) {
+        acc[0] += v[u].x; acc[1] += v[u].y; acc[2] += v[u].z; acc[3] += v[u].w;
+      }
+    }
+    for (; s < splits; ++s) {
+      const float4 v = *reinterpret_cast<const float4*>(p0 + s * sstride);
+      acc[0] += v.x; acc[1] += v.y; acc[2] += v.z; acc[3] += v.w;
+    }
+  } else {
+    for (int s = 0; s < splits; ++s)
+#pragma unroll
+      for (int k = 0; k < 4; ++k)
+        if (k < nvalid) acc[k] += p0[s * sstride + k];
+  }
+  return make_float4(acc[0], acc[1], acc[2], acc[3]);
+}
+
+SN_DEV float4 splitk_lane_partial(const float* __restrict__ p, float4 acc, int s, int splits, long long sstride) {
+  for (; s + 48 < splits; s += 64) {
+    float4 v[4];
+#pragma unroll
+    for (int u = 0; u < 4; ++u) v[u] = *reinterpret_cast<const float4*>(p + (s + 16 * u) * sstride);
+#pragma unroll
+    for (int u = 0; u < 4; ++u) {
+      acc.x += v[u].x; acc.y += v[u].y; acc.z += v[u].z; acc.w += v[u].w;
+    }
+  }
+  for (; s < splits; s += 16) {
+    float4 v = *reinterpret_cast<const float4*>(p + s * sstride);
+    acc.x += v.x; acc.y += v.y; acc.z += v.z; acc.w += v.w;
+  }
+  return acc;
+}
+
+SN_DEV float4 splitk_lane_combine(const float4* red, int stride) {
+  float a[4] = {0.f, 0.f, 0.f, 0.f};
+#pragma unroll
+  for (int q = 0; q < 16; ++q) {
+    float4 v = red[q * stride];
+    a[0] += v.x; a[1] += v.y; a[2] += v.z; a[3] += v.w;
+  }
+  return make_float4(a[0], a[1], a[2], a[3]);
+}
+
+SN_DEV void xent_reduce_block(const float* __restrict__ row_loss, const float* __restrict__ row_valid, int M,
+                              int normalize, float outer_num, float* __restrict__ out_loss,
+                              float* __restrict__ out_norm, float* ls, float* vs) {
+  const int lane = threadIdx.x & 63;
+  for (int w = threadIdx.x >> 6; w < 16; w += blockDim.x >> 6) {
+    float l = 0.f, v = 0.f;
+    for (int i = w * 64 + lane; i < M; i += 1024) {
+      l += row_loss[i];
+      v += row_valid[i];
+    }
+    l = wave_sum(l);
+    v = wave_sum(v);
+    if (lane == 0) {
+      ls[w] = l;
+      vs[w] = v;
+    }
+  }
+  __syncthreads();
+  if (threadIdx.x == 0) {
+    float L = 0.f, V = 0.f;
+    for (int w = 0; w < 16; ++w) { L += ls[w]; V += vs[w]; }
+    float norm = normalize ? V : outer_num;
+    norm = fmaxf(norm, 1.f);
+    out_loss[0] = L / norm;
+    out_norm[0] = norm;
+  }
+}
diff --git a/csrc/kernels/softmax.hip b/csrc/kernels/softmax.hip
--- a/csrc/kernels/softmax.hip
+++ b/csrc/kernels/softmax.hip
@@ -1,4 +1,5 @@
 #include "common.h"
+#include "reduce_order.h"
 
 #define FLT_MIN_ 1.175494351e-38f
 
@@ -34,26 +35,7 @@
 __global__ void xent_reduce(const float* __restrict__ row_loss, const float* __restrict__ row_valid, int M,
                             int normalize, float outer_num, float* __restrict__ out_loss, float* __restrict__ out_norm) {
   __shared__ float ls[16], vs[16];
-  float l = 0.f, v = 0.f;
-  for (int i = threadIdx.x; i < M; i += blockDim.x) {
-    l += row_loss[i];
-    v += row_valid[i];
-  }
-  l = wave_sum(l);
-  v = wave_sum(v);
-  if ((threadIdx.x & 63) == 0) {
-    ls[threadIdx.x >> 6] = l;
-    vs[threadIdx.x >> 6] = v;
-  }
-  __syncthreads();
-  if (threadIdx.x == 0) {
-    float L = 0.f, V = 0.f;
-    for (int w = 0; w < (int)(blockDim.x >> 6); ++w) { L += ls[w]; V += vs[w]; }
-    float norm = normalize ? V : outer_num;
-    norm = fmaxf(norm, 1.f);
-    out_loss[0] = L / norm;
-    out_norm[0] = norm;
-  }
+  xent_reduce_block(row_loss, row_valid, M, normalize, outer_num, out_loss, out_norm, ls, vs);
 }
 
 extern "C" int sn_softmax_xent_fwd(const bf16_t* x, const float* labels, float* prob, float* row_loss,
@@ -90,6 +72,139 @@
   return SN_CHECK_LAUNCH();
 }
 
+struct HeadArgs {
+  const float* ws;
+  long long sstride, ldw;
+  const float* bias;
+  bf16_t* x;
+  long long ldx;
+  const float* labels;
+  float *prob, *row_loss, *row_valid;
+  bf16_t* dx;
+  int splits, C, wide;
+  float loss_weight, norm;
+};
+
+#define HEAD_LDS_C 4096
+
+SN_DEV void head_store_logits(const HeadArgs& a, bf16_t* xr, bf16_t* lx, int c, float4 s) {
+  const float acc[4] = {s.x, s.y, s.z, s.w};
+  float v[4];
+#pragma unroll
+  for (int k = 0; k < 4; ++k) v[k] = acc[k] + ((a.bias && c + k < a.C) ? a.bias[c + k] : 0.f);
+  if (a.C <= HEAD_LDS_C) {
+#pragma unroll
+    for (int k = 0; k < 4; ++k)
+      if (c + k < a.C) lx[c + k] = f2bf(v[k]);
+  }
+  if (c + 3 < a.C && (reinterpret_cast<uintptr_t>(xr + c) & 7) == 0) {
+    *reinterpret_cast<uint2*>(xr + c) = make_uint2(pack2(v[0], v[1]), pack2(v[2], v[3]));
+  } else {
+#pragma unroll
+    for (int k = 0; k < 4; ++k)
+      if (c + k < a.C) xr[c + k] = f2bf(v[k]);
+  }
+}
+
+__global__ void __launch_bounds__(1024) ip_softmax_xent(HeadArgs a) {
+  __shared__ float4 red[16][128];
+  __shared__ float stat[2];
+  __shared__ bf16_t lx[HEAD_LDS_C];
+  const int t = threadIdx.x, row = blockIdx.x, C = a.C;
+  bf16_t* xr = a.x + (long long)row * a.ldx;
+  const bf16_t* xs = C <= HEAD_LDS_C ? lx : xr;
+  if (!a.ws && C <= HEAD_LDS_C) {
+    for (int c = t; c < C; c += 1024) lx[c] = xr[c];
+    __syncthreads();
+  }
+  if (a.ws) {
+    const int cols4 = (C + 3) >> 2;
+    const float* wr = a.ws + (long long)row * a.ldw;
+    if (a.wide) {
+      const int it = t & 63, sl = t >> 6;
+      for (int base = 0; base < cols4; base += 128) {
+        float4 acc[2];
+#pragma unroll
+        for (int u = 0; u < 2; ++u) {
+          const int i = base + u * 64 + it;
+          acc[u] = make_float4(0.f, 0.f, 0.f, 0.f);
+          if (i < cols4) {
+            const float4 v = *reinterpret_cast<const float4*>(wr + i * 4 + sl * a.sstride);
+            acc[u].x += v.x; acc[u].y += v.y; acc[u].z += v.z; acc[u].w += v.w;
+          }
+        }
+#pragma unroll
+        for (int u = 0; u < 2; ++u) {
+          const int i = base + u * 64 + it;
+          if (i < cols4) acc[u] = splitk_lane_partial(wr + i * 4, acc[u], sl + 16, a.splits, a.sstride);
+          red[sl][u * 64 + it] = acc[u];
+        }
+        __syncthreads();
+        if (t < 128 && base + t < cols4) head_store_logits(a, xr, lx, (base + t) * 4, splitk_lane_combine(&red[0][t], 128));
+        __syncthreads();
+      }
+    } else {
+      for (int i = t; i < cols4; i += 1024) {
+        const int c = i * 4;
+        const bool vec = (c + 3 < C) && ((a.ldw & 3) == 0);
+        head_store_logits(a, xr, lx, c, splitk_sum_serial(wr + c, a.splits, a.sstride, vec, C - c));
+      }
+    }
+    __syncthreads();
+  }
+  const int lab = (int)a.labels[row];
+  if (t < 64) {
+    const int lane = t;
+    float m = -INFINITY;
+    for (int c = lane; c < C; c += 64) m = fmaxf(m, bf2f(xs[c]));
+    m = wave_max(m);
+    float s = 0.f;
+    for (int c = lane; c < C; c += 64) s += __expf(bf2f(xs[c]) - m);
+    s = wave_sum(s);
+    const float inv = 1.f / s;
+    if (lane == 0) {
+      float p = __expf(bf2f(xs[min(max(lab, 0), C - 1)]) - m) * inv;
+      a.row_loss[row] = -__logf(fmaxf(p, FLT_MIN_));
+      a.row_valid[row] = 1.f;
+      stat[0] = m;
+      stat[1] = inv;
+    }
+  }
+  __syncthreads();
+  const float m = stat[0], inv = stat[1];
+  const float scale = a.loss_weight / a.norm;
+  float* pr = a.prob + (long long)row * C;
+  bf16_t* dr = a.dx + (long long)row * C;
+  for (int c = t; c < C; c += 1024) {
+    const float p = __fmul_rn(__expf(bf2f(xs[c]) - m), inv);
+    pr[c] = p;
+    dr[c] = f2bf((p - (c == lab ? 1.f : 0.f)) * scale);
+  }
+}
+
+extern "C" int sn_ip_softmax_xent(const float* ws, long long splits, long long sstride, long long ldw,
+                                  const float* bias, bf16_t* x, long long ldx, const float* labels, float* prob,
+                                  float* row_loss, float* row_valid, bf16_t* dx, long long M, long long C,
+                                  float loss_weight, long long normalize, long long outer_num, hipStream_t st) {
+  if (M <= 0 || C <= 0) return 0;
+  if (ws && splits < 1) return 5;
+  HeadArgs a;
+  a.ws = ws; a.sstride = sstride; a.ldw = ldw; a.bias = bias; a.x = x; a.ldx = ldx; a.labels = labels;
+  a.prob = prob; a.row_loss = row_loss; a.row_valid = row_valid; a.dx = dx;
+  a.splits = (int)splits; a.C = (int)C; a.wide = ws && splitk_wide_order(splits, C, ldw);
+  a.loss_weight = loss_weight;
+  a.norm = fmaxf(normalize ? (float)M : (float)outer_num, 1.f);
+  hipLaunchKernelGGL(ip_softmax_xent, dim3((unsigned)M), dim3(1024), 0, st, a);
+  return SN_CHECK_LAUNCH();
+}
+
+extern "C" int sn_xent_reduce(const float* row_loss, const float* row_valid, float* out_loss, float* out_norm,
+                              long long M, long long normalize, long long outer_num, hipStream_t st) {
+  hipLaunchKernelGGL(xent_reduce, dim3(1), dim3(1024), 0, st, row_loss, row_valid, (int)M, (int)normalize,
+                     (float)outer_num, out_loss, out_norm);
+  return SN_CHECK_LAUNCH();
+}
+
 __global__ void softmax_fwd(const bf16_t* __restrict__ x, bf16_t* __restrict__ y, int M, int C) {
   const int lane = threadIdx.x & 63;
   const int row = blockIdx.x * (blockDim.x >> 6) + (threadIdx.x >> 6);
diff --git a/csrc/kernels/solver.hip b/csrc/kernels/solver.hip
--- a/csrc/kernels/solver.hip
+++ b/csrc/kernels/solver.hip
@@ -1,4 +1,5 @@
 #include "common.h"
+#include "reduce_order.h"
 
 enum { H_LR = 0, H_MOM, H_WD, H_CLIP, H_NORM, H_DELTA, H_MOM2, H_RMS, H_CORR, H_T, H_SUMSQ = 15 };
 
@@ -75,6 +76,14 @@
   }
 }
 
+struct StepTail {
+  const float *row_loss, *row_valid;
+  float *out_loss, *out_norm;
+  long long* rng;
+  int M, normalize, on;
+  float outer_num;
+};
+
 template <int KIND, bool L1, bool CLIP, bool SHADOW>
 __global__ void __launch_bounds__(256) solver_update_kernel(float* __restrict__ w, const float* __restrict__ g,
                                                             float* __restrict__ h0, float* __restrict__ h1,
@@ -82,8 +91,17 @@
                                                             const long long* __restrict__ chunk_pos,
                                                             const float* __restrict__ chunk_mult,
                                                             const float* __restrict__ hyper, int nchunks,
-                                                            const long long* __restrict__ chunk_src) {
-  for (int cid = blockIdx.x; cid < nchunks; cid += gridDim.x) {
+                                                            const long long* __restrict__ chunk_src, StepTail tail) {
+  const int nblk = gridDim.x - tail.on;
+  if (tail.on && blockIdx.x == 0) {
+    __shared__ float ls[16], vs[16];
+    if (tail.row_loss)
+      xent_reduce_block(tail.row_loss, tail.row_valid, tail.M, tail.normalize, tail.outer_num, tail.out_loss,
+                        tail.out_norm, ls, vs);
+    if (tail.rng && threadIdx.x == 0) tail.rng[1] += 1;
+    return;
+  }
+  for (int cid = blockIdx.x - tail.on; cid < nchunks; cid += nblk) {
   const long long start = chunk_pos[2 * cid];
   const int count = (int)chunk_pos[2 * cid + 1];
   const float lr_mult = chunk_mult[2 * cid], decay_mult = chunk_mult[2 * cid + 1];
@@ -178,51 +196,76 @@
 
 template <int KIND, bool L1, bool CLIP>
 static void launch3(bool shadow, dim3 grid, hipStream_t st, float* w, const float* g, float* h0, float* h1,
-                    bf16_t* sh, const long long* cp, const float* cm, const float* hyper, int n, const long long* src) {
+                    bf16_t* sh, const long long* cp, const float* cm, const float* hyper, int n, const long long* src, const StepTail& tail) {
   if (shadow)
     hipLaunchKernelGGL((solver_update_kernel<KIND, L1, CLIP, true>), grid, dim3(256), 0, st, w, g, h0, h1, sh, cp, cm,
-                       hyper, n, src);
+                       hyper, n, src, tail);
   else
     hipLaunchKernelGGL((solver_update_kernel<KIND, L1, CLIP, false>), grid, dim3(256), 0, st, w, g, h0, h1, sh, cp,
-                       cm, hyper, n, src);
+                       cm, hyper, n, src, tail);
 }
 
 template <int KIND>
 static void launch_kind(bool l1, bool clip, bool shadow, dim3 grid, hipStream_t st, float* w, const float* g,
                         float* h0, float* h1, bf16_t* sh, const long long* cp, const float* cm, const float* hyper,
-                        int n, const long long* src) {
+                        int n, const long long* src, const StepTail& tail) {
   if (l1) {
-    if (clip) launch3<KIND, true, true>(shadow, grid, st, w, g, h0, h1, sh, cp, cm, hyper, n, src);
-    else launch3<KIND, true, false>(shadow, grid, st, w, g, h0, h1, sh, cp, cm, hyper, n, src);
+    if (clip) launch3<KIND, true, true>(shadow, grid, st, w, g, h0, h1, sh, cp, cm, hyper, n, src, tail);
+    else launch3<KIND, true, false>(shadow, grid, st, w, g, h0, h1, sh, cp, cm, hyper, n, src, tail);
   } else {
-    if (clip) launch3<KIND, false, true>(shadow, grid, st, w, g, h0, h1, sh, cp, cm, hyper, n, src);
-    else launch3<KIND, false, false>(shadow, grid, st, w, g, h0, h1, sh, cp, cm, hyper, n, src);
-  }
+    if (clip) launch3<KIND, false, true>(shadow, grid, st, w, g, h0, h1, sh, cp, cm, hyper, n, src, tail);
+    else launch3<KIND, false, false>(shadow, grid, st, w, g, h0, h1, sh, cp, cm, hyper, n, src, tail);
+  }
+}
+
+static int solver_update_launch(long long kind, float* w, const float* g, float* h0, float* h1, bf16_t* shadow,
+                                const long long* chunk_pos, const float* chunk_mult, long long nchunks,
+                                float* hyper, long long l1, long long clip, float* part, long long nparts,
+                                long long total, long long grid_limit, const long long* chunk_src,
+                                const StepTail& tail, hipStream_t st) {
+  if (nchunks <= 0) return tail.on ? 9 : 0;
+  if (clip && chunk_src) return 9;
+  if (clip) {
+    hipLaunchKernelGGL(sumsq_pass1, dim3((unsigned)nparts), dim3(256), 0, st, g, total, part);
+    hipLaunchKernelGGL(sumsq_pass2, dim3(1), dim3(1024), 0, st, part, (int)nparts, hyper);
+  }
+  dim3 grid((unsigned)(grid_limit > 0 && grid_limit < nchunks ? grid_limit : nchunks) + tail.on);
+  bool sh = shadow != nullptr;
+  const int n = (int)nchunks;
+  switch (kind) {
+    case 0: launch_kind<0>(l1, clip, sh, grid, st, w, g, h0, h1, shadow, chunk_pos, chunk_mult, hyper, n, chunk_src, tail); break;
+    case 1: launch_kind<1>(l1, clip, sh, grid, st, w, g, h0, h1, shadow, chunk_pos, chunk_mult, hyper, n, chunk_src, tail); break;
+    case 2: launch_kind<2>(l1, clip, sh, grid, st, w, g, h0, h1, shadow, chunk_pos, chunk_mult, hyper, n, chunk_src, tail); break;
+    case 3: launch_kind<3>(l1, clip, sh, grid, st, w, g, h0, h1, shadow, chunk_pos, chunk_mult, hyper, n, chunk_src, tail); break;
+    case 4: launch_kind<4>(l1, clip, sh, grid, st, w, g, h0, h1, shadow, chunk_pos, chunk_mult, hyper, n, chunk_src, tail); break;
+    case 5: launch_kind<5>(l1, clip, sh, grid, st, w, g, h0, h1, shadow, chunk_pos, chunk_mult, hyper, n, chunk_src, tail); break;
+    default: return 8;
+  }
+  return SN_CHECK_LAUNCH();
 }
 
 extern "C" int sn_solver_update(long long kind, float* w, const float* g, float* h0, float* h1, bf16_t* shadow,
                                 const long long* chunk_pos, const float* chunk_mult, long long nchunks,
                                 float* hyper, long long l1, long long clip, float* part, long long nparts,
                                 long long total, long long grid_limit, const long long* chunk_src, hipStream_t st) {
-  if (nchunks <= 0) return 0;
-  if (clip && chunk_src) return 9;
-  if (clip) {
-    hipLaunchKernelGGL(sumsq_pass1, dim3((unsigned)nparts), dim3(256), 0, st, g, total, part);
-    hipLaunchKernelGGL(sumsq_pass2, dim3(1), dim3(1024), 0, st, part, (int)nparts, hyper);
-  }
-  dim3 grid((unsigned)(grid_limit > 0 && grid_limit < nchunks ? grid_limit : nchunks));
-  bool sh = shadow != nullptr;
-  const int n = (int)nchunks;
-  switch (kind) {
-    case 0: launch_kind<0>(l1, clip, sh, grid, st, w, g, h0, h1, shadow, chunk_pos, chunk_mult, hyper, n, chunk_src); break;
-    case 1: launch_kind<1>(l1, clip, sh, grid, st, w, g, h0, h1, shadow, chunk_pos, chunk_mult, hyper, n, chunk_src); break;
-    case 2: launch_kind<2>(l1, clip, sh, grid, st, w, g, h0, h1, shadow, chunk_pos, chunk_mult, hyper, n, chunk_src); break;
-    case 3: launch_kind<3>(l1, clip, sh, grid, st, w, g, h0, h1, shadow, chunk_pos, chunk_mult, hyper, n, chunk_src); break;
-    case 4: launch_kind<4>(l1, clip, sh, grid, st, w, g, h0, h1, shadow, chunk_pos, chunk_mult, hyper, n, chunk_src); break;
-    case 5: launch_kind<5>(l1, clip, sh, grid, st, w, g, h0, h1, shadow, chunk_pos, chunk_mult, hyper, n, chunk_src); break;
-    default: return 8;
-  }
-  return SN_CHECK_LAUNCH();
+  StepTail tail = {};
+  return solver_update_launch(kind, w, g, h0, h1, shadow, chunk_pos, chunk_mult, nchunks, hyper, l1, clip, part,
+                              nparts, total, grid_limit, chunk_src, tail, st);
+}
+
+extern "C" int sn_solver_update_tail(long long kind, float* w, const float* g, float* h0, float* h1, bf16_t* shadow,
+                                     const long long* chunk_pos, const float* chunk_mult, long long nchunks,
+                                     float* hyper, long long l1, long long clip, float* part, long long nparts,
+                                     long long total, long long grid_limit, const long long* chunk_src,
+                                     const float* row_loss, const float* row_valid, float* out_loss,
+                                     float* out_norm, long long M, long long normalize, long long outer_num,
+                                     long long* rng, hipStream_t st) {
+  StepTail tail = {};
+  tail.row_loss = row_loss; tail.row_valid = row_valid; tail.out_loss = out_loss; tail.out_norm = out_norm;
+  tail.rng = rng; tail.M = (int)M; tail.normalize = (int)normalize; tail.outer_num = (float)outer_num;
+  tail.on = (row_loss || rng) ? 1 : 0;
+  return solver_update_launch(kind, w, g, h0, h1, shadow, chunk_pos, chunk_mult, nchunks, hyper, l1, clip, part,
+                              nparts, total, grid_limit, chunk_src, tail, st);
 }
 
 __global__ void scale_shadow(float* __restrict__ w, bf16_t* __restrict__ shadow, long long n, long long n4,
diff --git a/sparknet_amd/core/solver.py b/sparknet_amd/core/solver.py
--- a/sparknet_amd/core/solver.py
+++ b/sparknet_amd/core/solver.py
@@ -223,7 +223,7 @@
                           net.flat_compute if net.flat_compute is not net.flat_data else None,
                           tables, self.hyper, self.param.regularization_type == "L1", False, grid_limit)
 
-    def update_params(self) -> None:
+    def update_params(self, tail=None) -> None:
         from .. import ops
         l1 = self.param.regularization_type == "L1"
         if self.param.regularization_type not in ("L1", "L2"):
@@ -232,9 +232,13 @@
         if getattr(self, "slab_tables_dirty", False):
             assert not torch.cuda.is_current_stream_capturing(), "split-K slab layout changed during capture"
             self._build_tables()
+        if tail is not None and not self._tables["n"]:
+            tail.separate()
+            tail = None
         ops.solver_update(SOLVER_KINDS[self.type], net.flat_data, net.flat_diff, self.history,
                           net.flat_compute if net.flat_compute is not net.flat_data else None,
-                          self._tables, self.hyper, l1, self.param.clip_gradients > 0)
+                          self._tables, self.hyper, l1, self.param.clip_gradients > 0,
+                          **({"tail": tail.args()} if tail is not None else {}))
 
     def iteration(self):
         net = self.net
diff --git a/sparknet_amd/engine.py b/sparknet_amd/engine.py
--- a/sparknet_amd/engine.py
+++ b/sparknet_amd/engine.py
@@ -357,6 +357,93 @@
     if offsets:
         solver.set_fused_update(offsets)
     return len(offsets)
+
+
+class _LossHead:
+
+    def __init__(self, ip, loss, loss_weight: float):
+        self.ip, self.loss, self.loss_weight = ip, loss, float(loss_weight)
+        self.armed = False
+        self.tail = None
+        self.slabs = None
+        self.bias = None
+
+    def begin(self, bias):
+        self.slabs, self.bias = None, bias
+        return self
+
+    def accepts(self, c) -> bool:
+        from .ops import gemm
+        return (c.epi == gemm.EPI_BF16 and c.groups == 1 and not c.relu and c.gate is None and c.dropout is None
+                and c.bias_grad is None and c.out.is_contiguous() and tuple(c.out.shape) == (c.M, c.N)
+                and gemm._ptr(c.bias) == gemm._ptr(self.bias))
+
+    def record(self, ws, splits, ldw):
+        self.slabs = (ws, splits, ldw)
+
+    def take(self):
+        slabs, self.slabs = self.slabs, None
+        return slabs, self.bias
+
+
+def fuse_loss_head(net) -> list:
+    if (net.device.type != "cuda" or net.dtype != torch.bfloat16 or net.debug_info
+            or not features.enabled("fuse_loss_head")):
+        return []
+    weights = {id(t): w for t, w in net._loss_tops}
+    heads = []
+    for li, loss in enumerate(net.layers):
+        if loss.type_name != "SoftmaxWithLoss" or getattr(loss, "fused_head", None) is not None:
+            continue
+        if (loss.ignore_label is not None or len(net.top_ids[li]) != 1 or not net.layer_need_backward[li]
+                or not net.bottom_need_backward[li][0] or id(net.top_vecs[li][0]) not in weights):
+            continue
+        bid = net.bottom_ids[li][0]
+        blob = net.blobs[bid]
+        readers = [lj for lj, b in enumerate(net.bottom_ids) if bid in b]
+        writers = [lj for lj, t in enumerate(net.top_ids) if bid in t]
+        if readers != [li] or len(writers) != 1 or bid in net.output_blob_ids:
+            continue
+        ip = net.layers[writers[0]]
+        if (ip.type_name != "InnerProduct" or ip.fuse_relu or ip.fused_dropout is not None
+                or getattr(ip, "loss_head", None) is not None or len(blob.shape) != 2 or loss.axis != 1
+                or blob.dtype != torch.bfloat16 or blob.shape[0] >= 1 << 24):
+            continue
+        head = _LossHead(ip, loss, weights[id(net.top_vecs[li][0])])
+        ip.loss_head = loss.fused_head = head
+        heads.append(head)
+    return heads
+
+
+class StepTail:
+
+    def __init__(self, net, head):
+        self.net = net
+        self.head = head
+        self.armed = False
+        self.rows = None
+        self.out = torch.zeros(2, dtype=torch.float32, device=net.device)
+        if head is not None:
+            head.tail = self
+
+    def args(self):
+        loss = self.head.loss if self.rows is not None else None
+        return (self.rows, self.out, bool(loss.normalize) if loss else False, loss.outer if loss else 0,
+                self.net.ctx.rng_state)
+
+    def separate(self) -> None:
+        if self.rows is not None:
+            from .ops import hip
+            loss = self.head.loss
+            hip.xent_reduce(self.rows, loss.normalize, loss.outer, out=self.out)
+        ops.advance_rng(self.net.ctx.rng_state)
+
+
+def step_tail(net, heads):
+    if net.device.type != "cuda" or not features.enabled("step_tail") or len(net._loss_tops) != 1:
+        return None
+    head = heads[0] if len(heads) == 1 and net._loss_tops[0][1] == 1.0 else None
+    return StepTail(net, head)
 
 
 class _SlabGrad:
@@ -802,11 +889,23 @@
         elif fuse_fc:
             fuse_fc_updates(solver)
             fuse_splitk_updates(solver)
+        self.heads = fuse_loss_head(solver.net)
+        self.tail = step_tail(solver.net, self.heads) if self.overlap is None else None
         self.n_streams = streams if not solver.net.debug_info else 1
         self.branches = None
         self._use_branches = False
 
     def _body(self):
+        armed = self.heads + ([self.tail] if self.tail is not None else [])
+        for a in armed:
+            a.armed = True
+        try:
+            return self._armed_body()
+        finally:
+            for a in armed:
+                a.armed = False
+
+    def _armed_body(self):
         s = self.solver
         net = s.net
         net.clear_param_diffs(lazy=True)
@@ -822,6 +921,9 @@
         fp8_step(net)
         for cb in s.callbacks:
             getattr(cb, "on_gradients_ready", lambda: None)()
+        if self.tail is not None:
+            s.update_params(tail=self.tail)
+            return loss
         ops.advance_rng(net.ctx.rng_state)
         if self.overlap is not None:
             self.overlap.end()
diff --git a/sparknet_amd/layers/loss.py b/sparknet_amd/layers/loss.py
--- a/sparknet_amd/layers/loss.py
+++ b/sparknet_amd/layers/loss.py
@@ -125,7 +125,24 @@
         if len(tops) > 1:
             tops[1].reshape(b.shape, self.dtype)
 
-    def forward(self, bottoms, tops):
+    fused_head = None
+
+    def forward(self, bottoms, tops):
+        head = self.fused_head
+        self._head_done = head is not None and head.armed and bottoms[0].data.is_cuda
+        if self._head_done:
+            from ..ops import hip
+            x2 = bottoms[0].data.reshape(-1, bottoms[0].shape[1])
+            self.prob, rows, dx = hip.ip_softmax_xent(x2, bottoms[1].data, head.loss_weight, self.normalize,
+                                                      self.outer, *head.take())
+            bottoms[0].diff = dx.reshape(bottoms[0].data.shape)
+            tail = head.tail
+            if tail is not None and tail.armed:
+                tail.rows = rows
+                tops[0].data = tail.out[0].reshape(())
+            else:
+                tops[0].data = hip.xent_reduce(rows, self.normalize, self.outer)[0].reshape(())
+            return
         x2 = rows_view(bottoms[0], self.axis)
         loss, prob, norm = ops.softmax_loss_forward(x2, bottoms[1].data, self.ignore_label,
                                                     self.normalize, self.outer)
@@ -137,6 +154,8 @@
     def backward(self, tops, propagate_down, bottoms):
         if len(propagate_down) > 1 and propagate_down[1]:
             raise ValueError("SoftmaxWithLoss cannot backpropagate to label inputs")
+        if getattr(self, "_head_done", False):
+            return
         if propagate_down[0]:
             g = ops.softmax_loss_backward(self.prob, bottoms[1].data, tops[0].diff, self.norm,
                                           self.ignore_label, bottoms[0].dtype)
diff --git a/sparknet_amd/layers/vision.py b/sparknet_amd/layers/vision.py
--- a/sparknet_amd/layers/vision.py
+++ b/sparknet_amd/layers/vision.py
@@ -670,6 +670,15 @@
         bias = self.bias.data if self.bias is not None else None
         d = self.fused_dropout
         drop = (d.ctx.rng_state, d.stream, d.ratio) if d is not None and x2.is_cuda and d.phase == 0 else None
+        head = self.loss_head
+        if head is not None and head.armed and x2.is_cuda:
+            from ..ops.gemm import head_reduce
+            with head_reduce(head.begin(bias)):
+                self._forward(x2, bias, drop, tops)
+            return
+        self._forward(x2, bias, drop, tops)
+
+    def _forward(self, x2, bias, drop, tops):
         if self.fp8_slots is not None and x2.is_cuda:
             from ..ops import hip
             sc = self.ctx.fp8
@@ -688,6 +697,7 @@
     fp8_slots = None
     fused_update = None
     fused_dropout = None
+    loss_head = None
     gate_scale = 1.0
 
     def fp8_eligible(self, b) -> bool:
diff --git a/sparknet_amd/ops/__init__.py b/sparknet_amd/ops/__init__.py
--- a/sparknet_amd/ops/__init__.py
+++ b/sparknet_amd/ops/__init__.py
@@ -148,10 +148,14 @@
 
 
 def solver_update(kind, data, diff, history, compute, tables, hyper, l1: bool, clip: bool,
-                  grid_limit: int = 0) -> None:
+                  grid_limit: int = 0, tail=None) -> None:
     if data.is_cuda:
-        _hipmod().solver_update(kind, data, diff, history, compute, tables, hyper, l1, clip, grid_limit)
+        if tail is not None:
+            _hipmod().solver_update(kind, data, diff, history, compute, tables, hyper, l1, clip, grid_limit, tail)
+        else:
+            _hipmod().solver_update(kind, data, diff, history, compute, tables, hyper, l1, clip, grid_limit)
         return
+    assert tail is None
     h = hyper.tolist()
     ref.solver_update_ref(kind, data, diff, history, tables["lr"], tables["decay"], h, l1, clip)
     if compute is not None and compute is not data:
diff --git a/sparknet_amd/ops/gemm.py b/sparknet_amd/ops/gemm.py
--- a/sparknet_amd/ops/gemm.py
+++ b/sparknet_amd/ops/gemm.py
@@ -320,6 +320,10 @@
         sink.record(SplitSlabs(ws, ws.data_ptr(), splits, M, N - (1 if c.ones >= 0 else 0), ldw, c.groups, c.ones,
                                c.ldc, c.c_gstride))
         return
+    head = _HEAD_SINK
+    if head is not None and head.accepts(c):
+        head.record(ws, splits, ldw)
+        return
     mode = {EPI_BF16: 0, EPI_F32: 1, EPI_F32_ACC: 2}[c.epi]
     _lib.call("splitk_reduce", ws, splits, M * ldw, M, N, ldw, out, c.ldc, mode, c.bias, int(c.relu),
               c.groups, splits * M * ldw, c.c_gstride, c.gate, c.bias_grad, c.ones, int(c.bias_acc), M,
@@ -414,6 +418,24 @@
         global _DEFER_SINK
         _DEFER_SINK = self.prev
         self.sink.end()
+        return False
+
+
+_HEAD_SINK = None
+
+
+class head_reduce:
+    def __init__(self, sink):
+        self.sink = sink
+
+    def __enter__(self):
+        global _HEAD_SINK
+        self.prev, _HEAD_SINK = _HEAD_SINK, self.sink
+        return self.sink
+
+    def __exit__(self, *exc):
+        global _HEAD_SINK
+        _HEAD_SINK = self.prev
         return False
 
 
diff --git a/sparknet_amd/ops/hip.py b/sparknet_amd/ops/hip.py
--- a/sparknet_amd/ops/hip.py
+++ b/sparknet_amd/ops/hip.py
@@ -966,6 +966,27 @@
     return dx if dtype == BF16 else dx.to(dtype)
 
 
+def ip_softmax_xent(x2, labels, loss_weight, normalize, outer_num, slabs=None, bias=None):
+    M, Cn = x2.shape
+    assert x2.dtype == BF16 and x2.stride(1) == 1
+    dev = x2.device
+    prob = torch.empty((M, Cn), dtype=torch.float32, device=dev)
+    rows = torch.empty((2, M), dtype=torch.float32, device=dev)
+    dx = torch.empty((M, Cn), dtype=BF16, device=dev)
+    lab = _c(labels.reshape(-1).float())
+    ws, splits, ldw = slabs if slabs is not None else (None, 0, 0)
+    call("ip_softmax_xent", ws, splits, M * ldw, ldw, bias if slabs is not None else None, x2, x2.stride(0), lab,
+         prob, rows[0], rows[1], dx, M, Cn, float(loss_weight), int(normalize), int(outer_num))
+    return prob, rows, dx
+
+
+def xent_reduce(rows, normalize, outer_num, out=None):
+    if out is None:
+        out = torch.empty(2, dtype=torch.float32, device=rows.device)
+    call("xent_reduce", rows[0], rows[1], out[0:1], out[1:2], rows.shape[1], int(normalize), int(outer_num))
+    return out
+
+
 def softmax_forward(x2):
     x2 = as_bf16(x2)
     y = torch.empty_like(x2)
@@ -1021,9 +1042,17 @@
     }
 
 
-def solver_update(kind, data, diff, history, compute, tables, hyper, l1, clip, grid_limit=0):
+def solver_update(kind, data, diff, history, compute, tables, hyper, l1, clip, grid_limit=0, tail=None):
     h0 = history[0]
     h1 = history[1] if len(history) > 1 else history[0]
+    if tail is not None:
+        rows, out, normalize, outer_num, rng = tail
+        has = rows is not None
+        call("solver_update_tail", int(kind), data, diff, h0, h1, compute, tables["pos"], tables["mult"], tables["n"],
+             hyper, int(l1), int(clip), tables["part"], tables["part"].numel(), tables["total"], int(grid_limit),
+             tables.get("src"), rows[0] if has else None, rows[1] if has else None, out[0:1] if has else None,
+             out[1:2] if has else None, rows.shape[1] if has else 0, int(normalize), int(outer_num), rng)
+        return
     call("solver_update", int(kind), data, diff, h0, h1, compute, tables["pos"], tables["mult"], tables["n"],
          hyper, int(l1), int(clip), tables["part"], tables["part"].numel(), tables["total"], int(grid_limit),
          tables.get("src"))
diff --git a/sparknet_amd/utils/features.py b/sparknet_amd/utils/features.py
--- a/sparknet_amd/utils/features.py
+++ b/sparknet_amd/utils/features.py
@@ -11,6 +11,8 @@
     "fuse_bn_scale": True,
     "branch_depfree": True,
     "fuse_splitk": False,
+    "fuse_loss_head": True,
+    "step_tail": True,
     "conv_direct_c64": True,
     "conv_direct_k96": True,
     "conv_direct96": True,
```

Result: slower. 117,400 images/sec (-2.3%).
